# shaofeifei11/SSDR-AL

Measured on AMD Instinct MI355X. Metric: Mpoints/s subsample→KNN→RandLA-Net→FPS-GCN select, S3DIS 40960-pt tiles, higher is better.
Workload: dtype bf16x3: split-bf16 MFMA operands (hi*hi + lo*hi + hi*lo), fp32 accumulate, fp32 activations and non-matrix arithmetic

## Files before the change

include/ssdr_al.h:

```cpp
#ifndef SSDR_AL_H
#define SSDR_AL_H

#include <stddef.h>
#include <stdint.h>

#ifdef __cplusplus
extern "C" {
#endif

#define SSDR_OK               0
#define SSDR_ERR_INVALID      1
#define SSDR_ERR_NO_DEVICE    2
#define SSDR_ERR_HIP          3
#define SSDR_ERR_EMPTY        4
#define SSDR_ERR_UNSUPPORTED  5
#define SSDR_ERR_INTERNAL     6

const char* ssdr_version(void);
const char* ssdr_last_error(void);
int  ssdr_init(int device);
void ssdr_shutdown(void);
int  ssdr_stream_sync(void* stream);
int  ssdr_stream_create(void** out_stream);
int  ssdr_stream_create_priority(void** out_stream, int priority);
int  ssdr_stream_destroy(void* stream);
int  ssdr_main_stream(void** out_stream);
int  ssdr_stream_wait(void* waiter, void* waited);
int  ssdr_event_create(void** ev);
int  ssdr_event_record(void* ev, void* stream);
int  ssdr_stream_wait_event(void* stream, void* ev);
int  ssdr_event_destroy(void* ev);
int ssdr_prof_enable(int on);
const char* ssdr_prof_report(void);
float ssdr_last_gpu_ms(void);

int ssdr_knn(const float* points, size_t npts, size_t dim,
             const float* queries, size_t nqueries, size_t K, int64_t* indices);
int ssdr_knn_batch(const float* batch_data, size_t batch_size, size_t npts, size_t dim,
                   const float* queries, size_t nqueries, size_t K, int64_t* batch_indices);
int ssdr_knn_batch_i32(const float* batch_data, size_t batch_size, size_t npts, size_t dim,
                       const float* queries, size_t nqueries, size_t K, int32_t* batch_indices);
int ssdr_knn_batch_dev(const float* d_batch_data, size_t batch_size, size_t npts, size_t dim,
                       const float* d_queries, size_t nqueries, size_t K, int32_t* d_indices, void* stream);
int ssdr_knn_status(void* stream, int32_t* out4);
int ssdr_knn_status_poll(void* stream, int32_t* out4);

int ssdr_knn_pyramid_dev(const float* d_xyz, size_t batch_size, size_t npts,
                         size_t num_layers, const int32_t* ratios, size_t K,
                         int32_t* const* d_neigh_idx, int32_t* const* d_sub_idx,
                         int32_t* const* d_interp_idx, void* stream);
int ssdr_knn_pyramid(const float* xyz, size_t batch_size, size_t npts,
                     size_t num_layers, const int32_t* ratios, size_t K,
                     int32_t* const* neigh_idx, int32_t* const* sub_idx, int32_t* const* interp_idx);

#define SSDR_ORDER_REFERENCE 0
#define SSDR_ORDER_KEY       1
int ssdr_grid_subsample(const float* points, size_t n,
                        const float* features, size_t fdim,
                        const int32_t* classes, size_t ldim,
                        float sampleDl, int order, size_t* out_m);
int ssdr_grid_subsample_fetch(float* out_points, float* out_features, int32_t* out_classes);
int ssdr_grid_subsample_dev(const float* d_points, size_t n,
                            const float* d_features, size_t fdim,
                            const int32_t* d_classes, size_t ldim,
                            float sampleDl, int order,
                            float* d_out_points, float* d_out_features, int32_t* d_out_classes,
                            int64_t* d_out_m, void* stream);

int ssdr_grid_subsample_batch_dev(const float* d_points, const float* d_features, size_t fdim, const int32_t* d_classes, size_t ldim,
                                  const int64_t* cloud_offsets, size_t num_clouds, float sampleDl,
                                  float* d_out_points, float* d_out_features, int32_t* d_out_classes, int64_t* d_out_m, void* stream);
#define SSDR_SUBSAMPLE_AUTO 0
#define SSDR_SUBSAMPLE_SORT 1
int ssdr_grid_subsample_set_method(int method);
int ssdr_grid_subsample_status(void* stream, int32_t* out_status);

int ssdr_split3_dev(const float* d_xyz, size_t n, size_t max_size, size_t recurse_max_size, size_t merge_max, int32_t* d_part, int32_t* d_order, int64_t* part_offsets,
                    size_t max_parts, size_t* num_parts, void* stream);

int ssdr_tile_select_dev(const float* d_points, const float* d_colors, int color_dim, const int64_t* d_m, size_t n_max,
                         const float* center, size_t num_points, const int32_t* d_perm, const float* d_dup_u, float color_scale,
                         float* d_out_xyz, float* d_out_feat, int32_t* d_out_idx, void* stream);

int ssdr_tile_select_batch_dev(const float* d_points, const float* d_colors, int color_dim, const int64_t* d_m, const int64_t* cloud_offsets,
                               size_t num_clouds, const float* centers, size_t num_points, const int32_t* d_perm, const float* d_dup_u,
                               float color_scale, float* d_out_xyz, float* d_out_feat, int32_t* d_out_idx, const int32_t* d_labels,
                               int32_t* d_out_labels, void* stream);
int ssdr_tile_select_possibility_dev(const float* d_points, const float* d_colors, int color_dim, const int64_t* d_m, size_t n_max,
                                     const float* center, size_t num_points, const int32_t* d_perm, const float* d_dup_u, float color_scale,
                                     float* d_out_xyz, float* d_out_feat, int32_t* d_out_idx,
                                     double* d_possibility, double* d_out_min_possibility, int32_t* d_out_argmin, void* stream);

int ssdr_prune_dev(const float* d_xyz, size_t n, float voxel_size, const uint8_t* d_rgb, const uint8_t* d_labels, int n_labels,
                   const uint32_t* d_objects, int n_objects, float* d_out_xyz, uint8_t* d_out_rgb, uint32_t* d_out_labels,
                   uint32_t* d_out_objects, int64_t* d_out_m, void* stream);
int ssdr_prune_status(void* stream, int32_t* out_status);

int  ssdr_randla_create(int num_layers, const int32_t* d_out, int k_n, int num_classes, int in_dim, void** handle);
int  ssdr_randla_num_layers(void* handle);
int  ssdr_randla_layer_shape(void* handle, int layer, int* in, int* out, int* has_bias);
int  ssdr_randla_set_layer(void* handle, int layer, const float* W, const float* b);
#define SSDR_PREC_F32 0
#define SSDR_PREC_BF16X3 1
#define SSDR_PREC_BF16 2
int  ssdr_randla_set_precision(void* handle, int mode);
int  ssdr_randla_set_formulation(void* handle, int tiles32);
void ssdr_randla_destroy(void* handle);
int  ssdr_randla_infer_dev(void* handle, size_t batch_size, size_t npts, const float* d_features, const float* d_xyz,
                           const int32_t* ratios, int32_t* const* d_neigh_idx, int32_t* const* d_interp_idx,
                           float* d_probs, float* d_feat32, void* stream);
int  ssdr_randla_infer_rows_dev(void* handle, const size_t* level_rows, const float* d_features, const float* d_xyz,
                                int32_t* const* d_neigh_idx, int32_t* const* d_interp_idx, float* d_probs, float* d_feat32, void* stream);

#define SSDR_PREDICT_MAX_ROWS (1 << 23)
int ssdr_predict_layout(const int64_t* cloud_offsets, size_t num_clouds, size_t num_points, size_t num_layers, const int32_t* ratios,
                        int64_t* level_rows);
int ssdr_predict_tile_dev(const float* d_points, const float* d_colors, const int32_t* d_labels, const int64_t* cloud_offsets, size_t num_clouds,
                          const float* centers, size_t num_points, size_t num_layers, const int32_t* ratios, const int32_t* d_perm, const float* d_dup_u,
                          float color_scale, float* d_cm_xyz, int32_t* d_cm_idx, float* d_pk_xyz, float* d_pk_feat, int32_t* d_pk_src,
                          int32_t* d_pk_labels, void* stream);
int ssdr_knn_pyramid_ragged_dev(const float* d_cm_xyz, const int64_t* cloud_offsets, size_t num_clouds, size_t num_points, size_t num_layers,
                                const int32_t* ratios, size_t K, int32_t* d_cm_neigh, int32_t* d_cm_interp, void* stream);
int ssdr_predict_translate_dev(const int64_t* cloud_offsets, size_t num_clouds, size_t num_points, size_t num_layers, const int32_t* ratios, size_t K,
                               const int32_t* d_cm_neigh, const int32_t* d_cm_interp, int32_t* d_pk_neigh, int32_t* d_pk_interp, void* stream);
#define SSDR_READBACK_REFERENCE 0
#define SSDR_READBACK_POINT 1
int ssdr_predict_readback_dev(const int64_t* cloud_offsets, size_t num_clouds, size_t num_points, size_t num_layers, const int32_t* ratios,
                              const int32_t* d_cm_idx, const float* d_pk_probs, size_t num_classes, const float* d_pk_feat32, int mode,
                              float* d_probs, float* d_feat32, void* stream);

#define SSDR_UNC_LC 0
#define SSDR_UNC_ENTROPY 1
#define SSDR_UNC_SB 2
#define SSDR_REGION_MEAN 0
#define SSDR_REGION_SUM_WEIGHT 1
#define SSDR_REGION_WETSU 2
int ssdr_point_uncertainty_dev(const float* d_probs, size_t n, int num_classes, int mode, float* d_unc, int32_t* d_cls, void* stream);
int ssdr_region_stats_dev(const float* d_unc, const int32_t* d_cls, const int32_t* d_sp_off, const int32_t* d_sp_pts, size_t S,
                          int num_classes, int mode, double* d_region_unc, int32_t* d_dom, int32_t* d_dom_cnt, void* stream);
int ssdr_dominant_label_dev(const int32_t* d_labels, const int32_t* d_sp_off, const int32_t* d_sp_pts, size_t S, int num_labels,
                            int32_t* d_label, double* d_purity, void* stream);
int ssdr_clsbal_dev(const int32_t* d_region_class, size_t S, const uint8_t* d_skip, const int32_t* d_selected_class_list, size_t n_selected,
                    double* d_region_unc, void* stream);
int ssdr_class_hist_dev(const int32_t* d_region_class, size_t S, const uint8_t* d_skip, const int32_t* d_selected_class_list, size_t n_selected,
                        int32_t* d_hist64, void* stream);
int ssdr_clsbal_hist_dev(const int32_t* d_region_class, size_t S, const int32_t* d_hist64, size_t total, double* d_region_unc, void* stream);
int ssdr_rank_regions_dev(const double* d_region_unc, size_t S, int32_t* d_sorted_inds, void* stream);
int ssdr_segment_mean_features_dev(const float* d_feat, int feat_dim, const int32_t* d_cls, const int32_t* d_dom,
                                   const int32_t* d_sp_off, const int32_t* d_sp_pts, const int32_t* d_sel, size_t nsel,
                                   float* d_out, void* stream);
int ssdr_mask_regions_dev(const double* d_region_unc, const uint8_t* d_labelled, size_t S, size_t S_padded, double* d_out, void* stream);
int ssdr_gather_rows_dev(const void* d_in, const int32_t* d_idx, size_t n, size_t row_bytes, void* d_out, void* stream);
int ssdr_widen_f32_f64_dev(const float* d_x, size_t n, double* d_y0, double* d_y1, void* stream);
int ssdr_cloud_graph_dev(const float* d_xyz, const int32_t* d_sp_off, const int32_t* d_sp_pts, const int32_t* d_sel, size_t nsel,
                         size_t max_sp_size, int gcn_top, double* d_centres, double* d_cd_dir, double* d_adj, void* stream);
int ssdr_cloud_graph_batch_dev(const float* d_xyz, const int32_t* d_sp_off, const int32_t* d_sp_pts, const int32_t* d_sel,
                               const int32_t* d_coff, const int64_t* d_boff, size_t num_clouds, size_t n_total, size_t n_max,
                               int gcn_top, double* d_centres, double* d_cd_dir, double* d_adj, void* stream);
int ssdr_select_set_chamfer_mode(int mode);
int ssdr_propagate_batch_dev(const double* d_adj, const int32_t* d_coff, const int64_t* d_boff, size_t num_clouds, size_t n_max,
                             const int32_t* d_rows, const double* d_vin, int feat_dim, double* d_vout, double* d_comb, void* stream);
int ssdr_propagate_dev(const double* d_adj, size_t n, const int32_t* d_rows, const double* d_vin, int feat_dim, double* d_vout,
                       double* d_comb, void* stream);
int ssdr_create_adj_dev(const float* d_feat, size_t N, int F, const double* d_centres, const double* d_cd_dir, const int32_t* d_coff, const int64_t* d_boff,
                        size_t num_clouds, size_t n_max, const int32_t* d_rows, float* d_out_v, float* d_out_adj, void* stream);
#define SSDR_GCN_NHID 128
#define SSDR_GCN_NPARAM 4353
#define SSDR_GCN_FUSED_CAP 1024
#define SSDR_GCN_FORM_AUTO 0
#define SSDR_GCN_FORM_GENERAL 1
#define SSDR_GCN_FORM_FUSED 2
#define SSDR_GCN_ST_SINGLETON 32
#define SSDR_GCN_ST_NO_LABELLED 64
#define SSDR_GCN_ST_SUBSTITUTED 128
#define SSDR_GCN_ST_OVERSIZE 256
int ssdr_gcn_block_adj_dev(const float* d_feat, size_t cap_rows, int F, const double* d_centres, const double* d_cd_dir, const int32_t* d_coff, const int64_t* d_boff,
                           size_t num_clouds, size_t n_max, const int32_t* d_rows, const int32_t* d_counts, float* d_out_v, float* d_out_adj, float* d_out_adjT,
                           int32_t* d_rowcloud, int32_t* d_info, void* stream);
int ssdr_gcn_train_dev(const float* d_v, const float* d_adj, const float* d_adjT, const int32_t* d_coff, const int64_t* d_boff, size_t num_clouds, size_t n_max,
                       const int32_t* d_rows, const int32_t* d_rowcloud, const int32_t* d_counts, size_t cap_rows, const float* d_init, float* d_trained, int steps,
                       float p, float lr, float weight_decay, float lamda, uint64_t seed, int form, float* d_loss, int32_t* d_info, void* stream);
int ssdr_gcn_eval_dev(const float* d_v, const float* d_adj, const float* d_adjT, const int32_t* d_coff, const int64_t* d_boff, size_t num_clouds, size_t n_max,
                      const int32_t* d_rows, const int32_t* d_rowcloud, const int32_t* d_counts, size_t cap_rows, const float* d_params, double* d_out, int32_t* d_info,
                      void* stream);
int ssdr_gcn_sampling_dev(const float* d_feat, int feat_dim, const int32_t* d_cls, const int32_t* d_dom, const int32_t* d_lab_cls, const int32_t* d_lab_dom,
                          const float* d_xyz, const int32_t* d_sp_off, const int32_t* d_sp_pts, const int32_t* d_order, size_t S, const uint8_t* d_labelled, const int32_t* d_sp_base, size_t num_clouds,
                          const int32_t* d_lab_off, const int32_t* d_lab_sp, size_t n_lab, size_t batch_size, const float* d_init, int steps, float p, float lr, float weight_decay,
                          float lamda, uint64_t seed, int form, size_t cap_rows, size_t cap_nmax, size_t cap_sq, size_t cap_unl, size_t max_select, int32_t* d_result, void* stream);
int ssdr_gcn_sampling_rows(void* stream, const double** d_rows, size_t* cap_rows, const float** d_params, const float** d_loss, const int32_t** d_info);
int ssdr_gcn_fps_sampling_dev(const float* d_feat, int feat_dim, const int32_t* d_cls, const int32_t* d_dom, const int32_t* d_lab_cls, const int32_t* d_lab_dom,
                              const float* d_xyz, const int32_t* d_sp_off, const int32_t* d_sp_pts, const int32_t* d_order, size_t S, const uint8_t* d_labelled, const int32_t* d_sp_base, size_t num_clouds,
                              const int32_t* d_lab_off, const int32_t* d_lab_sp, size_t n_lab, size_t batch_size, int gcn_number, int gcn_top, int selector, int start,
                              size_t cap_rows, size_t cap_nmax, size_t cap_sq, size_t cap_unl, size_t max_select, int32_t* d_result, void* stream);
int ssdr_gcn_fps_sampling_rows(void* stream, const double** d_rows, size_t* cap_rows);
int ssdr_gcn_fps_sharded_local_dev(const float* d_feat, int feat_dim, const int32_t* d_cls, const int32_t* d_dom, const int32_t* d_lab_cls, const int32_t* d_lab_dom,
                                   const float* d_xyz, const int32_t* d_sp_off, const int32_t* d_sp_pts, const int32_t* d_lab_off, const int32_t* d_lab_sp, size_t n_lab, size_t num_clouds,
                                   const int32_t* d_gorder, size_t Sg, const uint8_t* d_glabelled, const int32_t* d_gbase, int rank, int world, size_t Smax, size_t Bmax,
                                   size_t batch_size, int gcn_number, int gcn_top, size_t cap_rows, size_t cap_nmax, size_t cap_sq, size_t nu_max, size_t nl_max,
                                   double* d_comb_out, int32_t* d_plan, void* stream);
int ssdr_fps_gathered_dev(const double* d_gathered, const int32_t* d_plan, int world, size_t nu_max, size_t cap_rows, int repeat, int start, size_t max_select, double* d_glob,
                          int32_t* d_out, void* stream);
int ssdr_kcenter_gathered_dev(const double* d_gathered, const int32_t* d_plan, int world, size_t nu_max, size_t nl_max, const int32_t* d_nlab_off, size_t n_lab_total,
                              size_t cap_rows, size_t max_select, double* d_glob, int32_t* d_already, int32_t* d_out, void* stream);
int ssdr_select_status(void* stream, int32_t* out_status);
int ssdr_fps_dev(const double* d_feat, size_t n, int feat_dim, int start, size_t count, int32_t* d_out, void* stream);
int ssdr_fps_superpoint_dev(const double* d_centres, const double* d_cd_dir, size_t n, int start, size_t count, int32_t* d_out, void* stream);
int ssdr_edcd_fps_batch_dev(const double* d_centres, double* d_cd_dir, const int32_t* d_coff, const int64_t* d_boff, const int32_t* d_ntop, size_t num_clouds,
                            size_t n_max, size_t max_select, int32_t* d_out, int32_t* d_status, void* stream);
int ssdr_edcd_sampling_dev(const float* d_xyz, const int32_t* d_sp_off, const int32_t* d_sp_pts, const int32_t* d_order, size_t S, const uint8_t* d_labelled,
                           const int32_t* d_sp_base, size_t num_clouds, size_t batch_size, size_t cap_rows, size_t cap_nmax, size_t cap_sq, size_t max_select,
                           int32_t* d_result, void* stream);
int ssdr_edcd_sampling_sharded_dev(const float* d_xyz, const int32_t* d_sp_off, const int32_t* d_sp_pts, size_t num_clouds, const int32_t* d_gorder, size_t Sg,
                                   const uint8_t* d_glabelled, const int32_t* d_gbase, int rank, int world, size_t Smax, size_t Bmax, size_t batch_size,
                                   size_t cap_rows, size_t cap_nmax, size_t cap_sq, size_t max_select, int32_t* d_result, void* stream);
int ssdr_topk_regions_dev(const int32_t* d_order, size_t n, const uint8_t* d_skip, size_t batch_size, size_t lo, size_t hi, int32_t* d_res, int32_t* d_out, void* stream);
#define SSDR_LABEL_DOMINANT 0
#define SSDR_LABEL_NAIL     1
int ssdr_oracle_label_dev(const int32_t* d_gt, const int32_t* d_pred_class, size_t n, const int32_t* d_sp_off, const int32_t* d_sp_pts, size_t S,
                          const int32_t* d_sp_cloud, size_t num_clouds, const int32_t* d_items, const int32_t* d_n_items, size_t max_items,
                          const int32_t* d_cloud_key, size_t max_region, int num_labels, int num_classes, int mode, double threshold, int64_t min_size,
                          int64_t* d_budget, float* d_mask, float* d_label, uint8_t* d_used, uint8_t* d_labeled, int32_t* d_class_out, size_t class_cap,
                          int32_t* d_proc_order, int64_t* d_out, void* stream);
int ssdr_oracle_label_items_dev(const int32_t* d_result, int layout, size_t max_select, const int32_t* d_order, size_t S, const uint8_t* d_skip,
                                const int32_t* d_sp_cloud, size_t num_clouds, int32_t* d_items, size_t max_items, int32_t* d_n_items, int32_t* d_cloud_key,
                                void* stream);
int ssdr_kcenter_dev(const double* d_feat, size_t n, int feat_dim, const int32_t* d_already_selected, size_t n_already, size_t count,
                     int32_t* d_out, void* stream);

int ssdr_chamfer3d_forward_dev(const float* d_xyz1, const float* d_xyz2, size_t batch, size_t n, size_t m,
                               float* d_dist1, float* d_dist2, int32_t* d_idx1, int32_t* d_idx2, void* stream);

int ssdr_vote_smooth_dev(float* d_test_probs, const int32_t* d_point_idx, const float* d_probs, size_t n, int num_classes, double smooth,
                         int32_t* d_owner_scratch, void* stream);
int ssdr_confusion_dev(const float* d_probs, int num_classes, const int32_t* d_proj_idx, const int32_t* d_labels, size_t n, int32_t* d_pred,
                       uint64_t* d_confusion, double* d_iou, void* stream);

int ssdr_dev_alloc(size_t bytes, void** d_ptr);
int ssdr_dev_free(void* d_ptr);
int ssdr_memcpy_h2d(void* d_dst, const void* src, size_t bytes);
int ssdr_memcpy_d2h(void* dst, const void* d_src, size_t bytes);
int ssdr_memcpy_h2d_on(void* d_dst, const void* src, size_t bytes, void* stream);
int ssdr_memcpy_d2h_on(void* dst, const void* d_src, size_t bytes, void* stream);

int ssdr_knn_batch_distance_pick(const float* batch_data, size_t batch_size, size_t npts, size_t dim, float* batch_queries,
                                 size_t nqueries, size_t K, int64_t* batch_indices, uint32_t seed);

int ssdr_knn_graph_dev(const float* d_xyz, size_t n, size_t k_nn1, size_t k_nn2, uint32_t* d_source, uint32_t* d_target,
                       float* d_distances, uint32_t* d_target2, void* stream);
int ssdr_geof_dev(const float* d_xyz, size_t n, const uint32_t* d_target, size_t k_nn, float* d_geof, void* stream);

#ifdef __cplusplus
}
#endif
#endif
```

ssdr-al_amd/csrc/randla.hpp:

```cpp
#pragma once
#include "ssdr_internal.hpp"

namespace ssdr {

struct DenseArgs {
    const float* x1; int k1;
    const float* x2; int k2;
    const int* idx2;
    int m_per_batch;
    int x2_rows_per_batch;
    const float* W; const float* b;
    float* y; int M, N; int act;
    int ldy;
    const float* xyz; size_t xyz_batch_stride; int xyz_rows_per_batch;
    const uint16_t* wt_hi; const uint16_t* wt_lo; int kp;
};

struct LfaArgs {
    const float* xyz; size_t xyz_batch_stride;
    const int* neigh;
    const float* fin;
    const float* w_l1; const float* b_l1;
    const float* w_l2; const float* b_l2;
    const float* w_fc;
    const float* w_fc_t;
    const float* g;
    float* out;
    int n;
    const uint16_t* fc_hi; const uint16_t* fc_lo;
    const uint16_t* l2_hi; const uint16_t* l2_lo; int kp2;
};

struct Lfa32Args {
    const float* xyz; size_t xyz_batch_stride;
    const int* neigh;
    const float* fin;
    const float* g;
    float* out;
    int n;
    const uint16_t* w1p; const float* b1;
    const uint16_t *w2_hi, *w2_lo; const float* b2;
    const uint16_t *fc_hi, *fc_lo;
};

constexpr int PREC_F32 = 0;
constexpr int PREC_BF16X3 = 1;
constexpr int PREC_BF16 = 2;

int launch_dense(const DenseArgs& a, hipStream_t s);
int launch_xyz_fill(const DenseArgs& a, hipStream_t s);
int launch_lfa(int D, const LfaArgs& a, bool second, int B, hipStream_t s);
struct TailArgs {
    const float* x; int M, C;
    const uint16_t *w1h, *w1l; int kp1; const float* b1;
    const uint16_t *w2h, *w2l; int kp2; const float* b2;
    const uint16_t *w3h, *w3l; int kp3; const float* b3;
    float* feat32; float* probs;
    const float* skip; const float* up; const int* idx; int m_per_batch, up_rows_per_batch;
    const uint16_t *wdh, *wdl; int kpd; const float* bd;
};
int launch_tail_bf16(const TailArgs& t, int prec, hipStream_t s);
int launch_dense_bf16(const DenseArgs& a, int prec, hipStream_t s);
int launch_dense_rows2(const DenseArgs& a, const DenseArgs& b, hipStream_t s);
int launch_dense_chain(const DenseArgs& l1, const DenseArgs& l2, int prec, hipStream_t s);
int launch_lfa_bf16(int D, const LfaArgs& a, bool second, int B, int prec, hipStream_t s);
int launch_lfa32(int D, const Lfa32Args& a, bool second, int B, int prec, hipStream_t s);
int launch_gather_max(const float* f, const int* idx, int n_in, int n_out, int idx_rows, int C, float* out, int B, hipStream_t s);
int launch_tail(const float* x, const float* W1, const float* b1, const float* W2, const float* b2, const float* W3, const float* b3,
                int M, int C, float* feat32, float* probs, hipStream_t s);
int launch_head(const float* x, const float* W, const float* b, int M, int C, float* probs, hipStream_t s);

}
```

ssdr-al_amd/csrc/randla_bf16.hip:

```cpp
#include "ssdr_internal.hpp"
#include "randla.hpp"
#include "randla_dev.hpp"
#include <cmath>

namespace ssdr {

__device__ __forceinline__ u32x4 ld128(const void* p) { return *reinterpret_cast<const u32x4*>(p); }
__device__ __forceinline__ void st128(void* p, u32x4 v) { *reinterpret_cast<u32x4*>(p) = v; }

template <int TERMS>
__device__ __forceinline__ f32x4 mma_split(const u32x4 (&a)[2], const u32x4 (&b)[2], f32x4 c) {
    c = mfma_bf16(a[0], b[0], c);
    if (TERMS == 2) { c = mfma_bf16(a[1], b[0], c); c = mfma_bf16(a[0], b[1], c); }
    return c;
}

template <int TM, int KC, int TERMS, bool VEC>
__global__ __launch_bounds__(256) SSDR_WAVES_PER_EU(TM == 128 ? 4 : 5) void dense_bf16_kernel(DenseArgs a) {
    constexpr int KS = KC + 8;
    constexpr int TPR = KC / 8;
    constexpr int RPP = 256 / TPR;
    constexpr int APASS = TM / RPP, BPASS = 64 / RPP;
    static_assert(TM % RPP == 0 && 64 % RPP == 0, "staging passes");
    constexpr int CT = TM == 128 ? 4 : 1;
    __shared__ __attribute__((aligned(16))) uint16_t As[TERMS][TM * KS];
    __shared__ __attribute__((aligned(16))) uint16_t Bs[TERMS][64 * KS];
    const int tid = threadIdx.x, lane = tid & 63, w = tid >> 6;
    int bxr = (int)blockIdx.x, byc = (int)blockIdx.y;
    if (a.idx2 && a.m_per_batch % TM == 0 && a.M % a.m_per_batch == 0 && ((a.M / a.m_per_batch) & 7) == 0) {
        const int gy = (int)gridDim.y, rpb = a.m_per_batch / TM;
        const int lin = byc * (int)gridDim.x + bxr, xcd = lin & 7, j = lin >> 3, rb = j / gy;
        byc = j % gy; bxr = (xcd + 8 * (rb / rpb)) * rpb + rb % rpb;
    }
    const int row0 = bxr * TM, col0 = byc * 64;
    const int K = a.k1 + a.k2;
    const int sr = tid / TPR, sk = (tid % TPR) * 8;
    const float* x1r[APASS]; const float* x2r[APASS];
#pragma unroll
    for (int h = 0; h < APASS; ++h) {
        const int grow = row0 + sr + RPP * h;
        x1r[h] = nullptr; x2r[h] = nullptr;
        if (grow < a.M) {
            x1r[h] = a.x1 + (size_t)grow * a.k1;
            if (a.k2) {
                size_t r2 = (size_t)grow;
                if (a.idx2) r2 = (size_t)(grow / a.m_per_batch) * a.x2_rows_per_batch + (size_t)a.idx2[grow];
                x2r[h] = a.x2 + r2 * a.k2;
            }
        }
    }
    float ra[APASS][8]; u32x4 rb[BPASS][TERMS];
    auto fetch = [&](int kc) {
#pragma unroll
        for (int h = 0; h < APASS; ++h) {
            if (VEC) {
#pragma unroll
                for (int q = 0; q < 2; ++q) {
                    const int gk = kc + sk + 4 * q;
                    float4 v = make_float4(0.f, 0.f, 0.f, 0.f);
                    if (x1r[h] && gk < K) v = (gk < a.k1) ? *reinterpret_cast<const float4*>(x1r[h] + gk) : *reinterpret_cast<const float4*>(x2r[h] + (gk - a.k1));
                    ra[h][4 * q] = v.x; ra[h][4 * q + 1] = v.y; ra[h][4 * q + 2] = v.z; ra[h][4 * q + 3] = v.w;
                }
            } else {
#pragma unroll
                for (int j = 0; j < 8; ++j) {
                    const int gk = kc + sk + j;
                    float v = 0.f;
                    if (x1r[h]) { if (gk < a.k1) v = x1r[h][gk]; else if (gk < K) v = x2r[h][gk - a.k1]; }
                    ra[h][j] = v;
                }
            }
        }
#pragma unroll
        for (int h = 0; h < BPASS; ++h) {
            const int gc = col0 + sr + RPP * h;
#pragma unroll
            for (int t = 0; t < TERMS; ++t) {
                u32x4 v = {0u, 0u, 0u, 0u};
                if (gc < a.N && kc + sk < a.kp) v = ld128((t ? a.wt_lo : a.wt_hi) + (size_t)gc * a.kp + kc + sk);
                rb[h][t] = v;
            }
        }
    };
    auto stash = [&]() {
#pragma unroll
        for (int h = 0; h < APASS; ++h) {
            u32x4 hi, lo;
#pragma unroll
            for (int q = 0; q < 4; ++q) {
                unsigned hq, lq;
                split_bf16(ra[h][2 * q], ra[h][2 * q + 1], hq, lq);
                hi[q] = hq; lo[q] = lq;
            }
            st128(&As[0][(sr + RPP * h) * KS + sk], hi);
            if (TERMS == 2) st128(&As[TERMS - 1][(sr + RPP * h) * KS + sk], lo);
        }
#pragma unroll
        for (int h = 0; h < BPASS; ++h)
#pragma unroll
            for (int t = 0; t < TERMS; ++t) st128(&Bs[t][(sr + RPP * h) * KS + sk], rb[h][t]);
    };
    f32x4 acc[2][CT];
#pragma unroll
    for (int r = 0; r < 2; ++r)
#pragma unroll
        for (int c = 0; c < CT; ++c) acc[r][c] = f32x4{0.f, 0.f, 0.f, 0.f};
    const int rbase = TM == 128 ? w * 32 : 0, cbase = TM == 128 ? 0 : w * 16;
    const int fr = lane & 15, fk = 8 * (lane >> 4);
    fetch(0);
    for (int kc = 0; kc < K; kc += KC) {
        stash();
        __syncthreads();
        if (kc + KC < K) fetch(kc + KC);
#pragma unroll
        for (int ks = 0; ks < KC / 32; ++ks) {
            u32x4 af[2][2], bf[CT][2];
#pragma unroll
            for (int r = 0; r < 2; ++r)
#pragma unroll
                for (int t = 0; t < TERMS; ++t) af[r][t] = ld128(&As[t][(rbase + r * 16 + fr) * KS + ks * 32 + fk]);
#pragma unroll
            for (int c = 0; c < CT; ++c)
#pragma unroll
                for (int t = 0; t < TERMS; ++t) bf[c][t] = ld128(&Bs[t][(cbase + c * 16 + fr) * KS + ks * 32 + fk]);
#pragma unroll
            for (int r = 0; r < 2; ++r)
#pragma unroll
                for (int c = 0; c < CT; ++c) acc[r][c] = mma_split<TERMS>(af[r], bf[c], acc[r][c]);
        }
        __syncthreads();
    }
#pragma unroll
    for (int c = 0; c < CT; ++c) {
        const int col = col0 + cbase + c * 16 + (lane & 15);
        if (col >= a.N) continue;
        const float bias = a.b ? a.b[col] : 0.f;
#pragma unroll
        for (int r = 0; r < 2; ++r)
#pragma unroll
            for (int q = 0; q < 4; ++q) {
                const int row = row0 + rbase + r * 16 + (lane >> 4) * 4 + q;
                if (row < a.M) { float v = acc[r][c][q] + bias; a.y[(size_t)row * (a.ldy ? a.ldy : a.N) + col] = a.act ? lrelu(v) : v; }
            }
    }
}


struct ChainArgs {
    const float* x1; const float* x2; int k2;
    const uint16_t* wa_hi; const uint16_t* wa_lo; int kpa; const float* ba;
    const uint16_t* wb_hi; const uint16_t* wb_lo; int kpb; const float* bb;
    float* y; int M;
};
template <int D, int K2P, int TM, int TERMS>
__global__ __launch_bounds__(256) void dense_chain_kernel(ChainArgs a) {
    constexpr int KS = K2P + 8;
    constexpr int TPR = K2P <= 32 ? 4 : 16;
    constexpr int RPP = 256 / TPR;
    constexpr int WC = TM == 128 ? 1 : 2;
    constexpr int CT1 = (D / 16 + WC - 1) / WC;
    constexpr int CT2 = 4 / WC;
    static_assert(D % 16 == 0 && D <= 64 && K2P % 32 == 0 && TPR * 8 >= K2P && (TM == 128 || TM == 64) && TM % RPP == 0, "shapes");
    __shared__ __attribute__((aligned(16))) uint16_t As[TERMS][TM * KS];
    __shared__ __attribute__((aligned(16))) uint16_t Bs[TERMS][64 * KS];
    const int tid = threadIdx.x, lane = tid & 63, w = tid >> 6;
    const int wr = TM == 128 ? w : (w >> 1), wc = TM == 128 ? 0 : (w & 1);
    const int row0 = (int)blockIdx.x * TM;
    const int sr = tid / TPR, sk = (tid % TPR) * 8;
    const int K = D + a.k2;
    if (sk < K2P) {
        float4 va[TM / RPP][2];
#pragma unroll
        for (int h = 0; h < TM / RPP; ++h) {
            const int grow = row0 + sr + RPP * h;
            va[h][0] = make_float4(0.f, 0.f, 0.f, 0.f); va[h][1] = va[h][0];
            if (grow < a.M) {
                const float* src = sk < D ? a.x1 + (size_t)grow * D + sk : (sk < K ? a.x2 + (size_t)grow * a.k2 + (sk - D) : nullptr);
                if (src) { va[h][0] = *reinterpret_cast<const float4*>(src); va[h][1] = *reinterpret_cast<const float4*>(src + 4); }
            }
        }
#pragma unroll
        for (int h = 0; h < TM / RPP; ++h) {
            const int r = sr + RPP * h;
            const float4 v0 = va[h][0], v1 = va[h][1];
            u32x4 hi, lo; unsigned hq, lq;
            split_bf16(v0.x, v0.y, hq, lq); hi[0] = hq; lo[0] = lq;
            split_bf16(v0.z, v0.w, hq, lq); hi[1] = hq; lo[1] = lq;
            split_bf16(v1.x, v1.y, hq, lq); hi[2] = hq; lo[2] = lq;
            split_bf16(v1.z, v1.w, hq, lq); hi[3] = hq; lo[3] = lq;
            st128(&As[0][r * KS + sk], hi);
            if (TERMS == 2) st128(&As[TERMS - 1][r * KS + sk], lo);
        }
    }
    u32x4 wreg[64 / RPP][TERMS];
    auto load_w = [&](const uint16_t* whi, const uint16_t* wlo, int kp, int col0, int ncols, int kvalid) {
#pragma unroll
        for (int h = 0; h < 64 / RPP; ++h) {
            const int r = sr + RPP * h;
#pragma unroll
            for (int t = 0; t < TERMS; ++t) {
                u32x4 v = {0u, 0u, 0u, 0u};
                if (sk < K2P && col0 + r < ncols && sk < kvalid) v = ld128((t ? wlo : whi) + (size_t)(col0 + r) * kp + sk);
                wreg[h][t] = v;
            }
        }
    };
    auto store_w = [&]() {
        if (sk < K2P) {
#pragma unroll
            for (int h = 0; h < 64 / RPP; ++h)
#pragma unroll
                for (int t = 0; t < TERMS; ++t) st128(&Bs[t][(sr + RPP * h) * KS + sk], wreg[h][t]);
        }
    };
    load_w(a.wa_hi, a.wa_lo, a.kpa, 0, D, D);
    store_w();
    __syncthreads();
    load_w(a.wb_hi, a.wb_lo, a.kpb, 0, 2 * D, K);
    const int fr = lane & 15, fk = 8 * (lane >> 4), rbase = wr * 32;
    {
        f32x4 acc[2][CT1];
#pragma unroll
        for (int r = 0; r < 2; ++r)
#pragma unroll
            for (int c = 0; c < CT1; ++c) acc[r][c] = f32x4{0.f, 0.f, 0.f, 0.f};
        const bool has1 = wc * CT1 * 16 < D;
        if (has1) {
#pragma unroll
            for (int ks = 0; ks < (D + 31) / 32; ++ks) {
                u32x4 af[2][2], bf[CT1][2];
#pragma unroll
                for (int r = 0; r < 2; ++r)
#pragma unroll
                    for (int t = 0; t < TERMS; ++t) af[r][t] = ld128(&As[t][(rbase + r * 16 + fr) * KS + ks * 32 + fk]);
#pragma unroll
                for (int c = 0; c < CT1; ++c)
#pragma unroll
                    for (int t = 0; t < TERMS; ++t) bf[c][t] = ld128(&Bs[t][((wc * CT1 + c) * 16 + fr) * KS + ks * 32 + fk]);
#pragma unroll
                for (int r = 0; r < 2; ++r)
#pragma unroll
                    for (int c = 0; c < CT1; ++c) acc[r][c] = mma_split<TERMS>(af[r], bf[c], acc[r][c]);
            }
        }
        if (WC > 1) __syncthreads();
        if (has1) {
#pragma unroll
            for (int c = 0; c < CT1; ++c) {
                const int col = (wc * CT1 + c) * 16 + (lane & 15);
                const float bias = a.ba ? a.ba[col] : 0.f;
#pragma unroll
                for (int r = 0; r < 2; ++r)
#pragma unroll
                    for (int q = 0; q < 4; ++q) {
                        const int row = rbase + r * 16 + (lane >> 4) * 4 + q;
                        const float v = lrelu(acc[r][c][q] + bias);
                        unsigned hq, lq; split_bf16(v, 0.f, hq, lq);
                        As[0][row * KS + col] = (uint16_t)(hq & 0xffffu);
                        if (TERMS == 2) As[TERMS - 1][row * KS + col] = (uint16_t)(lq & 0xffffu);
                    }
            }
        }
    }
    for (int ct = 0; ct < (2 * D + 63) / 64; ++ct) {
        __syncthreads();
        store_w();
        __syncthreads();
        if (ct + 1 < (2 * D + 63) / 64) load_w(a.wb_hi, a.wb_lo, a.kpb, (ct + 1) * 64, 2 * D, K);
        f32x4 acc[2][CT2];
#pragma unroll
        for (int r = 0; r < 2; ++r)
#pragma unroll
            for (int c = 0; c < CT2; ++c) acc[r][c] = f32x4{0.f, 0.f, 0.f, 0.f};
#pragma unroll
        for (int ks = 0; ks < K2P / 32; ++ks) {
            u32x4 af[2][2], bf[CT2][2];
#pragma unroll
            for (int r = 0; r < 2; ++r)
#pragma unroll
                for (int t = 0; t < TERMS; ++t) af[r][t] = ld128(&As[t][(rbase + r * 16 + fr) * KS + ks * 32 + fk]);
#pragma unroll
            for (int c = 0; c < CT2; ++c)
#pragma unroll
                for (int t = 0; t < TERMS; ++t) bf[c][t] = ld128(&Bs[t][((wc * CT2 + c) * 16 + fr) * KS + ks * 32 + fk]);
#pragma unroll
            for (int r = 0; r < 2; ++r)
#pragma unroll
                for (int c = 0; c < CT2; ++c) acc[r][c] = mma_split<TERMS>(af[r], bf[c], acc[r][c]);
        }
#pragma unroll
        for (int c = 0; c < CT2; ++c) {
            const int col = ct * 64 + (wc * CT2 + c) * 16 + (lane & 15);
            if (col >= 2 * D) continue;
            const float bias = a.bb ? a.bb[col] : 0.f;
#pragma unroll
            for (int r = 0; r < 2; ++r)
#pragma unroll
                for (int q = 0; q < 4; ++q) {
                    const int row = row0 + rbase + r * 16 + (lane >> 4) * 4 + q;
                    if (row < a.M) a.y[(size_t)row * (2 * D) + col] = lrelu(acc[r][c][q] + bias);
                }
        }
    }
}

template <int D> struct LfaBf16Cfg {
    static constexpr int H = D / 2;
    static constexpr int NW = D >= 256 ? 8 : 4;
    static constexpr int NT = NW * 64;
    static constexpr int NCG = D == 64 ? 2 : NW;
    static constexpr int NPG = NW / NCG;
    static constexpr int PTS = D == 64 ? 8 : 4;
    static constexpr int PW = PTS / NPG;
    static constexpr int ROWS = PTS * 16;
    static constexpr int LDX = H + 8;
    static constexpr int NCT1 = H / 16;
    static constexpr int NCH = NCT1 / NCG;
    static_assert(NCT1 % NCG == 0 && PTS % NPG == 0, "tile split");
    static constexpr size_t lds_bytes(int terms) { return (size_t)ROWS * ((size_t)terms * LDX * 2 + 10 * 4 + 4); }
};

#ifndef HIPEMU
typedef __amdgpu_buffer_rsrc_t rsrc_t;
__device__ __forceinline__ rsrc_t make_rsrc(const void* p, unsigned bytes) { return __builtin_amdgcn_make_buffer_rsrc(const_cast<void*>(p), 0, (int)bytes, 0x00020000); }
template <int IMM> __device__ __forceinline__ float buf_load(rsrc_t r, unsigned voff) { return __builtin_bit_cast(float, __builtin_amdgcn_raw_buffer_load_b32(r, (int)voff + IMM, 0, 0)); }
#else
struct rsrc_t { const char* p; };
static inline rsrc_t make_rsrc(const void* p, unsigned) { return rsrc_t{reinterpret_cast<const char*>(p)}; }
template <int IMM> static inline float buf_load(rsrc_t r, unsigned voff) { return *reinterpret_cast<const float*>(r.p + voff + IMM); }
#endif

template <int D, bool SECOND, int TERMS>
__global__ __launch_bounds__(LfaBf16Cfg<D>::NT) SSDR_WAVES_PER_EU((D == 256 && !SECOND) ? 4 : 1) void lfa_bf16_kernel(LfaArgs a) {
    using C = LfaBf16Cfg<D>;
    constexpr int H = C::H, PTS = C::PTS, ROWS = C::ROWS, LDX = C::LDX, NT = C::NT, NCG = C::NCG, PW = C::PW, NCH = C::NCH, NCT1 = C::NCT1;
    SSDR_DYN_SHARED(float, smem);
    uint16_t* X[2];
    X[0] = reinterpret_cast<uint16_t*>(smem);
    X[1] = X[0] + (TERMS == 2 ? (size_t)ROWS * LDX : 0);
    float* REL = reinterpret_cast<float*>(X[0] + (size_t)TERMS * ROWS * LDX);
    int* NBR = reinterpret_cast<int*>(REL + (size_t)ROWS * 10);
    const int tid = threadIdx.x, lane = tid & 63, w = tid >> 6;
    const int lc = lane & 15, lg = lane >> 4;
    const int cg = w % NCG, p0 = (w / NCG) * PW;
    int bx_, b; xcd_tile_map(bx_, b);
    const int pt0 = bx_ * PTS;
    const float* xyz = a.xyz + (size_t)b * a.xyz_batch_stride;
    const int* neigh = a.neigh + (size_t)b * a.n * 16;

    float w1[NCH][3], b1c[NCH]; float4 b1r[NCH];
#pragma unroll
    for (int j = 0; j < NCH; ++j) {
        const int ct = cg * NCH + j;
#pragma unroll
        for (int ks = 0; ks < 3; ++ks) {
            const int k = ks * 4 + lg;
            const float v = a.w_l1[(k < 10 ? k : 9) * H + ct * 16 + lc];
            w1[j][ks] = k < 10 ? v : 0.f;
        }
        b1c[j] = a.b_l1[ct * 16 + lc];
        b1r[j] = *reinterpret_cast<const float4*>(a.b_l1 + ct * 16 + 4 * lg);
    }

    for (int row = tid; row < ROWS; row += NT) {
        const int n = pt0 + (row >> 4);
        float r[10]; int j = 0;
#pragma unroll
        for (int q = 0; q < 10; ++q) r[q] = 0.f;
        if (n < a.n) {
            j = neigh[(size_t)n * 16 + (row & 15)];
            const float px = xyz[3 * (size_t)n], py = xyz[3 * (size_t)n + 1], pz = xyz[3 * (size_t)n + 2];
            const float qx = xyz[3 * (size_t)j], qy = xyz[3 * (size_t)j + 1], qz = xyz[3 * (size_t)j + 2];
            const float dx = px - qx, dy = py - qy, dz = pz - qz;
            r[0] = sqrtf(dx * dx + dy * dy + dz * dz);
            r[1] = dx; r[2] = dy; r[3] = dz; r[4] = px; r[5] = py; r[6] = pz; r[7] = qx; r[8] = qy; r[9] = qz;
        }
#pragma unroll
        for (int q = 0; q < 10; ++q) REL[row * 10 + q] = r[q];
        NBR[row] = j;
    }
    __syncthreads();

    auto store_row4 = [&](int p, int ct, const float (&v)[4]) {
        u32x2 hi, lo; unsigned h, l;
        split_bf16(v[0], v[1], h, l); hi[0] = h; lo[0] = l;
        split_bf16(v[2], v[3], h, l); hi[1] = h; lo[1] = l;
        const int e = (p * 16 + lc) * LDX + ct * 16 + 4 * lg;
        *reinterpret_cast<u32x2*>(&X[0][e]) = hi;
        if (TERMS == 2) *reinterpret_cast<u32x2*>(&X[1][e]) = lo;
    };

    float fx[PW][NCH][4];

#pragma unroll
    for (int p = 0; p < PW; ++p) {
        float rf[3];
#pragma unroll
        for (int ks = 0; ks < 3; ++ks) { const int k = ks * 4 + lg; rf[ks] = (k < 10) ? REL[((p0 + p) * 16 + lc) * 10 + k] : 0.f; }
#pragma unroll
        for (int j = 0; j < NCH; ++j) {
            f32x4 at = f32x4{b1r[j].x, b1r[j].y, b1r[j].z, b1r[j].w};
#pragma unroll
            for (int ks = 0; ks < 3; ++ks) at = mfma16(w1[j][ks], rf[ks], at);
            float v[4];
#pragma unroll
            for (int r = 0; r < 4; ++r) v[r] = lrelu(at[r]);
            store_row4(p0 + p, cg * NCH + j, v);
            if (!SECOND) {
                f32x4 ac = f32x4{b1c[j], b1c[j], b1c[j], b1c[j]};
#pragma unroll
                for (int ks = 0; ks < 3; ++ks) ac = mfma16(rf[ks], w1[j][ks], ac);
#pragma unroll
                for (int r = 0; r < 4; ++r) fx[p][j][r] = lrelu(ac[r]);
            }
        }
    }
    __syncthreads();

    if (SECOND) {
        f32x4 accT[PW][NCH], acc2[PW][NCH];
#pragma unroll
        for (int j = 0; j < NCH; ++j) {
            const int ct = cg * NCH + j;
            const float4 br = *reinterpret_cast<const float4*>(a.b_l2 + ct * 16 + 4 * lg);
            const float bc = a.b_l2[ct * 16 + lc];
#pragma unroll
            for (int p = 0; p < PW; ++p) { accT[p][j] = f32x4{br.x, br.y, br.z, br.w}; acc2[p][j] = f32x4{bc, bc, bc, bc}; }
        }
        for (int kb = 0; kb < H / 32; ++kb) {
            u32x4 xf[PW][2], wf[NCH][2];
#pragma unroll
            for (int j = 0; j < NCH; ++j)
#pragma unroll
                for (int t = 0; t < TERMS; ++t) wf[j][t] = ld128((t ? a.l2_lo : a.l2_hi) + (size_t)((cg * NCH + j) * 16 + lc) * a.kp2 + kb * 32 + 8 * lg);
#pragma unroll
            for (int p = 0; p < PW; ++p)
#pragma unroll
                for (int t = 0; t < TERMS; ++t) xf[p][t] = ld128(&X[t][((p0 + p) * 16 + lc) * LDX + kb * 32 + 8 * lg]);
#pragma unroll
            for (int p = 0; p < PW; ++p)
#pragma unroll
                for (int j = 0; j < NCH; ++j) { accT[p][j] = mma_split<TERMS>(wf[j], xf[p], accT[p][j]); acc2[p][j] = mma_split<TERMS>(xf[p], wf[j], acc2[p][j]); }
        }
        __syncthreads();
#pragma unroll
        for (int p = 0; p < PW; ++p)
#pragma unroll
            for (int j = 0; j < NCH; ++j) {
                float v[4];
#pragma unroll
                for (int r = 0; r < 4; ++r) { v[r] = lrelu(accT[p][j][r]); fx[p][j][r] = lrelu(acc2[p][j][r]); }
                store_row4(p0 + p, cg * NCH + j, v);
            }
        __syncthreads();
    }

    const rsrc_t rG = make_rsrc(a.g + (size_t)b * a.n * D, (unsigned)a.n * D * 4u);
    const rsrc_t rF = make_rsrc(a.fin + (size_t)b * a.n * H, (unsigned)a.n * H * 4u);
    f32x4 acc[PW][2 * NCH];
    float fn[PW][NCH][4];
#pragma unroll
    for (int p = 0; p < PW; ++p) {
        int nb[4];
#pragma unroll
        for (int r = 0; r < 4; ++r) nb[r] = NBR[(p0 + p) * 16 + lg * 4 + r];
#pragma unroll
        for (int r = 0; r < 4; ++r) {
            const unsigned og = (unsigned)nb[r] * (D * 4u) + lc * 4u + cg * NCH * 64u, of = (unsigned)nb[r] * (H * 4u) + lc * 4u + cg * NCH * 64u;
            acc[p][0][r] = buf_load<0>(rG, og); acc[p][NCH][r] = buf_load<H * 4>(rG, og); fn[p][0][r] = buf_load<0>(rF, of);
            if constexpr (NCH == 2) { acc[p][1][r] = buf_load<64>(rG, og); acc[p][NCH + 1][r] = buf_load<H * 4 + 64>(rG, og); fn[p][1][r] = buf_load<64>(rF, of); }
        }
    }
    static_assert(NCH <= 2, "gather immediates are written out for one or two tiles per half");
    for (int kb = 0; kb < H / 32; ++kb) {
        u32x4 af[PW][2], bf[2 * NCH][2];
#pragma unroll
        for (int c = 0; c < 2 * NCH; ++c) {
            const int col = (c < NCH ? cg * NCH + c : NCT1 + cg * NCH + (c - NCH)) * 16 + lc;
#pragma unroll
            for (int t = 0; t < TERMS; ++t) bf[c][t] = ld128((t ? a.fc_lo : a.fc_hi) + (size_t)col * D + H + kb * 32 + 8 * lg);
        }
#pragma unroll
        for (int p = 0; p < PW; ++p)
#pragma unroll
            for (int t = 0; t < TERMS; ++t) af[p][t] = ld128(&X[t][((p0 + p) * 16 + lc) * LDX + kb * 32 + 8 * lg]);
#pragma unroll
        for (int p = 0; p < PW; ++p)
#pragma unroll
            for (int c = 0; c < 2 * NCH; ++c) acc[p][c] = mma_split<TERMS>(af[p], bf[c], acc[p][c]);
    }

    float* out = a.out + (size_t)b * a.n * D;
#pragma unroll
    for (int p = 0; p < PW; ++p) {
        const int n = pt0 + p0 + p;
#pragma unroll
        for (int c = 0; c < 2 * NCH; ++c) {
            const int col = (c < NCH ? cg * NCH + c : NCT1 + cg * NCH + (c - NCH)) * 16 + lc;
            float m = fmaxf(fmaxf(acc[p][c][0], acc[p][c][1]), fmaxf(acc[p][c][2], acc[p][c][3]));
            m = rows_max(m);
            float s = 0.f, v = 0.f;
#pragma unroll
            for (int r = 0; r < 4; ++r) {
                const float e = fast_exp2(acc[p][c][r] - m);
                const float f = c < NCH ? fn[p][c][r] : fx[p][c - NCH][r];
                s += e; v = fmaf(f, e, v);
            }
            s = rows_sum(s); v = rows_sum(v);
            v = v * fast_rcp(s);
            if (lg == 0 && n < a.n) out[(size_t)n * D + col] = v;
        }
    }
}

struct TailPre {
    const float* skip; const float* up; const int* idx; int m_per_batch, up_rows_per_batch;
    const uint16_t *wh, *wl; int kp; const float* b;
};
template <int TERMS, int C, bool PRE>
__global__ __launch_bounds__(256) void tail_bf16_kernel(TailPre pre, const float* __restrict__ x, const uint16_t* __restrict__ w1h, const uint16_t* __restrict__ w1l, int kp1,
                                                        const float* __restrict__ b1, const uint16_t* __restrict__ w2h, const uint16_t* __restrict__ w2l, int kp2,
                                                        const float* __restrict__ b2, const uint16_t* __restrict__ w3h, const uint16_t* __restrict__ w3l, int kp3,
                                                        const float* __restrict__ b3, int M, float* __restrict__ feat32, float* __restrict__ probs) {
    const int lane = threadIdx.x & 63, lc = lane & 15, lg = lane >> 4;
    const int wave = blockIdx.x * 4 + (threadIdx.x >> 6), nwaves = gridDim.x * 4;
    auto ld64x2 = [](const uint16_t* p0, const uint16_t* p1) {
        const u32x2 a = *reinterpret_cast<const u32x2*>(p0), b = *reinterpret_cast<const u32x2*>(p1);
        return u32x4{a[0], a[1], b[0], b[1]};
    };
    constexpr int F_WD = 0, F_W1 = 4, F_W2 = 8, F_W3 = 12, NFRAG = 13;
    __shared__ u32x4 s_w[NFRAG * 2][64];
    float4 BD[2];
    {
        const int wv = threadIdx.x >> 6;
#pragma unroll
        for (int t = 0; t < TERMS; ++t) {
            const uint16_t* p1 = t ? w1l : w1h; const uint16_t* p2 = t ? w2l : w2h; const uint16_t* p3 = t ? w3l : w3h;
            if (PRE && wv == 0) {
                const uint16_t* pd = t ? pre.wl : pre.wh;
#pragma unroll
                for (int kb = 0; kb < 2; ++kb)
#pragma unroll
                    for (int ct = 0; ct < 2; ++ct) s_w[(F_WD + 2 * kb + ct) * 2 + t][lane] = ld128(pd + (size_t)(16 * ct + lc) * pre.kp + 32 * kb + 8 * lg);
            }
            if (wv == 1) {
#pragma unroll
                for (int ct = 0; ct < 4; ++ct)
                    s_w[(F_W1 + ct) * 2 + t][lane] = PRE ? ld64x2(p1 + (size_t)(16 * ct + lc) * kp1 + 4 * lg, p1 + (size_t)(16 * ct + lc) * kp1 + 16 + 4 * lg) : ld128(p1 + (size_t)(16 * ct + lc) * kp1 + 8 * lg);
            }
            if (wv == 2) {
#pragma unroll
                for (int kb = 0; kb < 2; ++kb)
#pragma unroll
                    for (int ct = 0; ct < 2; ++ct) s_w[(F_W2 + 2 * kb + ct) * 2 + t][lane] = ld64x2(p2 + (size_t)(16 * ct + lc) * kp2 + 32 * kb + 4 * lg, p2 + (size_t)(16 * ct + lc) * kp2 + 32 * kb + 16 + 4 * lg);
            }
            if (wv == 3) s_w[F_W3 * 2 + t][lane] = lc < C ? ld64x2(p3 + (size_t)lc * kp3 + 4 * lg, p3 + (size_t)lc * kp3 + 16 + 4 * lg) : u32x4{0u, 0u, 0u, 0u};
        }
        __syncthreads();
    }
    auto wfr = [&](int f, u32x4 (&w)[2]) { w[0] = s_w[f * 2][lane]; w[1] = s_w[f * 2 + (TERMS - 1)][lane]; };
    if (PRE) { BD[0] = *reinterpret_cast<const float4*>(pre.b + 4 * lg); BD[1] = *reinterpret_cast<const float4*>(pre.b + 16 + 4 * lg); }
    float4 B1[4], B2t[2], B3; float B2c[2];
#pragma unroll
    for (int ct = 0; ct < 4; ++ct) B1[ct] = *reinterpret_cast<const float4*>(b1 + 16 * ct + 4 * lg);
#pragma unroll
    for (int ct = 0; ct < 2; ++ct) { B2t[ct] = *reinterpret_cast<const float4*>(b2 + 16 * ct + 4 * lg); B2c[ct] = b2[16 * ct + lc]; }
    {
        float t[4];
#pragma unroll
        for (int r = 0; r < 4; ++r) t[r] = 4 * lg + r < C ? b3[4 * lg + r] : 0.f;
        B3 = make_float4(t[0], t[1], t[2], t[3]);
    }
    auto frag = [](const float (&v)[8], u32x4 (&f)[2]) {
#pragma unroll
        for (int q = 0; q < 4; ++q) { unsigned h, l; split_bf16(v[2 * q], v[2 * q + 1], h, l); f[0][q] = h; f[1][q] = l; }
    };
    const int ntiles = (M + 15) / 16;
    int tpb = 0, nbe = 0;
    if (PRE && pre.m_per_batch % 16 == 0 && M % pre.m_per_batch == 0 && (gridDim.x & 7) == 0) { tpb = pre.m_per_batch / 16; nbe = M / pre.m_per_batch; if (nbe & 7) tpb = 0; }
    const int lw = ((int)blockIdx.x >> 3) * 4 + ((int)threadIdx.x >> 6), lnw = nwaves >> 3, lnt = tpb ? (nbe >> 3) * tpb : 0;
    const int it_first = tpb ? lw : wave, it_end = tpb ? lnt : ntiles, it_step = tpb ? lnw : nwaves;
    auto tile_of = [&](int it) { return tpb ? (((int)blockIdx.x & 7) + 8 * (it / tpb)) * tpb + it % tpb : it; };
    auto row_of = [&](int it) { const int r = tile_of(it) * 16 + lc; return (it < it_end && r < M) ? r : -1; };
    auto load8r = [&](const float* p, int ok, float4 (&v)[2]) {
        v[0] = make_float4(0.f, 0.f, 0.f, 0.f); v[1] = v[0];
        if (ok) { v[0] = *reinterpret_cast<const float4*>(p + 8 * lg); v[1] = *reinterpret_cast<const float4*>(p + 8 * lg + 4); }
    };
    auto unpack8 = [](const float4 (&a)[2], float (&v)[8]) { v[0] = a[0].x; v[1] = a[0].y; v[2] = a[0].z; v[3] = a[0].w; v[4] = a[1].x; v[5] = a[1].y; v[6] = a[1].z; v[7] = a[1].w; };
    float4 n_sk[2], n_up[2];
    int idx_next = 0;
    auto issue_rows = [&](int it, int idx) {
        const int r = row_of(it);
        if (PRE) {
            const int rw = r < 0 ? 0 : r;
            load8r(pre.skip + (size_t)rw * 32, r >= 0, n_sk);
            load8r(pre.up + ((size_t)(rw / pre.m_per_batch) * pre.up_rows_per_batch + (size_t)idx) * 32, r >= 0, n_up);
        } else load8r(x + (size_t)(r < 0 ? 0 : r) * 32, r >= 0, n_sk);
    };
    auto load_idx = [&](int it) { const int r = row_of(it); return (PRE && r >= 0) ? pre.idx[r] : 0; };
    {
        const int i0 = load_idx(it_first);
        idx_next = load_idx(it_first + it_step);
        issue_rows(it_first, i0);
    }
    for (int it = it_first; it < it_end; it += it_step) {
        const int tile = tile_of(it);
        const int row = tile * 16 + lc;
        float c_sk[8], c_up[8];
        unpack8(n_sk, c_sk);
        if (PRE) unpack8(n_up, c_up);
        {
            const int idx2 = load_idx(it + 2 * it_step);
            issue_rows(it + it_step, idx_next);
            idx_next = idx2;
        }
        SSDR_SCHED_FENCE();
        u32x4 xf[2];
        if (PRE) {
            u32x4 sf[2], uf[2]; frag(c_sk, sf); frag(c_up, uf);
            f32x4 d0 = f32x4{BD[0].x, BD[0].y, BD[0].z, BD[0].w}, d1 = f32x4{BD[1].x, BD[1].y, BD[1].z, BD[1].w};
            { u32x4 w[2]; wfr(F_WD + 0, w); d0 = mma_split<TERMS>(w, sf, d0); wfr(F_WD + 2, w); d0 = mma_split<TERMS>(w, uf, d0);
              wfr(F_WD + 1, w); d1 = mma_split<TERMS>(w, sf, d1); wfr(F_WD + 3, w); d1 = mma_split<TERMS>(w, uf, d1); }
            const float v[8] = {lrelu(d0[0]), lrelu(d0[1]), lrelu(d0[2]), lrelu(d0[3]), lrelu(d1[0]), lrelu(d1[1]), lrelu(d1[2]), lrelu(d1[3])};
            frag(v, xf);
        } else frag(c_sk, xf);
        float h1[4][4];
#pragma unroll
        for (int ct = 0; ct < 4; ++ct) {
            f32x4 acc = f32x4{B1[ct].x, B1[ct].y, B1[ct].z, B1[ct].w};
            { u32x4 w[2]; wfr(F_W1 + ct, w); acc = mma_split<TERMS>(w, xf, acc); }
#pragma unroll
            for (int r = 0; r < 4; ++r) h1[ct][r] = lrelu(acc[r]);
        }
        f32x4 at[2] = {f32x4{B2t[0].x, B2t[0].y, B2t[0].z, B2t[0].w}, f32x4{B2t[1].x, B2t[1].y, B2t[1].z, B2t[1].w}};
        f32x4 ac[2] = {f32x4{B2c[0], B2c[0], B2c[0], B2c[0]}, f32x4{B2c[1], B2c[1], B2c[1], B2c[1]}};
#pragma unroll
        for (int kb = 0; kb < 2; ++kb) {
            const float v[8] = {h1[2 * kb][0], h1[2 * kb][1], h1[2 * kb][2], h1[2 * kb][3], h1[2 * kb + 1][0], h1[2 * kb + 1][1], h1[2 * kb + 1][2], h1[2 * kb + 1][3]};
            u32x4 hf[2]; frag(v, hf);
#pragma unroll
            for (int ct = 0; ct < 2; ++ct) { u32x4 w[2]; wfr(F_W2 + 2 * kb + ct, w); at[ct] = mma_split<TERMS>(w, hf, at[ct]); ac[ct] = mma_split<TERMS>(hf, w, ac[ct]); }
        }
#pragma unroll
        for (int ct = 0; ct < 2; ++ct)
#pragma unroll
            for (int r = 0; r < 4; ++r) { const int rr = tile * 16 + 4 * lg + r; if (rr < M) feat32[(size_t)rr * 32 + 16 * ct + lc] = lrelu(ac[ct][r]); }
        const float v2[8] = {lrelu(at[0][0]), lrelu(at[0][1]), lrelu(at[0][2]), lrelu(at[0][3]), lrelu(at[1][0]), lrelu(at[1][1]), lrelu(at[1][2]), lrelu(at[1][3])};
        u32x4 ff[2]; frag(v2, ff);
        f32x4 lg3 = f32x4{B3.x, B3.y, B3.z, B3.w};
        { u32x4 w[2]; wfr(F_W3, w); lg3 = mma_split<TERMS>(w, ff, lg3); }
        float z[4], m = -3.402823466e+38f;
#pragma unroll
        for (int r = 0; r < 4; ++r) { z[r] = 4 * lg + r < C ? lg3[r] : -3.402823466e+38f; m = fmaxf(m, z[r]); }
        m = rows_max(m);
        float e[4], sum = 0.f;
#pragma unroll
        for (int r = 0; r < 4; ++r) { e[r] = 4 * lg + r < C ? expf(z[r] - m) : 0.f; sum += e[r]; }
        sum = rows_sum(sum);
        if (row < M)
#pragma unroll
            for (int r = 0; r < 4; ++r) if (4 * lg + r < C) probs[(size_t)row * C + 4 * lg + r] = e[r] / sum;
    }
}

template <int TM, int KC>
static int launch_dense_bf16_t(const DenseArgs& a, int prec, bool vec, hipStream_t s) {
    dim3 grid((unsigned)((a.M + TM - 1) / TM), (unsigned)((a.N + 63) / 64));
    if (prec == PREC_BF16X3) {
        if (vec) hipLaunchKernelGGL((dense_bf16_kernel<TM, KC, 2, true>), grid, dim3(256), 0, s, a);
        else hipLaunchKernelGGL((dense_bf16_kernel<TM, KC, 2, false>), grid, dim3(256), 0, s, a);
    } else {
        if (vec) hipLaunchKernelGGL((dense_bf16_kernel<TM, KC, 1, true>), grid, dim3(256), 0, s, a);
        else hipLaunchKernelGGL((dense_bf16_kernel<TM, KC, 1, false>), grid, dim3(256), 0, s, a);
    }
    SSDR_HIP(hipGetLastError());
    return SSDR_OK;
}

int launch_dense_bf16(const DenseArgs& a, int prec, hipStream_t s) {
    if (a.M <= 0 || a.N <= 0) return SSDR_OK;
    if (a.N == 8 && a.k2 == 0 && a.k1 <= 16) return launch_dense(a, s);
    if (!a.wt_hi || (prec == PREC_BF16X3 && !a.wt_lo)) { set_error("dense (bf16): the layer has no bf16 weight pieces"); return SSDR_ERR_INVALID; }
    if (a.xyz) SSDR_TRY(launch_xyz_fill(a, s));
    const bool small = a.M <= 16384;
    const double tm = small ? 32.0 : 128.0, kc = small ? 64.0 : 32.0;
    const double exec = 2.0 * std::ceil(a.M / tm) * tm * std::ceil((a.k1 + a.k2) / kc) * kc * std::ceil(a.N / 64.0) * 64.0 * (prec == PREC_BF16X3 ? 3.0 : 1.0);
    ProfScope prof(small ? "dense_bf16_kernel<32,64>" : "dense_bf16_kernel<128,32>", s, 2.0 * (double)a.M * (double)(a.k1 + a.k2) * (double)a.N, exec);
    const bool vec = a.k1 % 4 == 0 && a.k2 % 4 == 0 && ((uintptr_t)a.x1 & 15) == 0 && ((uintptr_t)a.x2 & 15) == 0;
    if (small) return launch_dense_bf16_t<32, 64>(a, prec, vec, s);
    return launch_dense_bf16_t<128, 32>(a, prec, vec, s);
}

int launch_dense_chain(const DenseArgs& l1, const DenseArgs& l2, int prec, hipStream_t s) {
    const int d = l1.k1;
    const bool shapes = l1.k2 == 0 && l1.N == d && l1.act && l2.act && l2.k1 == d && l2.N == 2 * d && l2.x1 == l1.y && l2.M == l1.M && !l2.idx2 && !l1.ldy && !l2.ldy && !l1.xyz && !l2.xyz &&
                        l2.k2 % 8 == 0 && l2.k2 > 0 && l1.wt_hi && l2.wt_hi && (prec != PREC_BF16X3 || (l1.wt_lo && l2.wt_lo)) &&
                        (((uintptr_t)l1.x1 | (uintptr_t)l2.x2) & 15) == 0 && l1.kp % 8 == 0 && l2.kp % 8 == 0;
    if (!shapes || l1.M <= 0) return SSDR_ERR_UNSUPPORTED;
    int k2p = 0;
    if (d == 16 && d + l2.k2 <= 32) k2p = 32; else if (d == 64 && d + l2.k2 <= 96) k2p = 96; else return SSDR_ERR_UNSUPPORTED;
    ChainArgs a{l1.x1, l2.x2, l2.k2, l1.wt_hi, l1.wt_lo, l1.kp, l1.b, l2.wt_hi, l2.wt_lo, l2.kp, l2.b, l2.y, l1.M};
    const double np = prec == PREC_BF16X3 ? 3.0 : 1.0, m128 = std::ceil(l1.M / 128.0) * 128.0;
    ProfScope prof(d == 16 ? "dense_chain_kernel<16>" : "dense_chain_kernel<64>", s, 2.0 * (double)l1.M * ((double)d * d + (double)(d + l2.k2) * 2.0 * d),
                   2.0 * m128 * ((d == 16 ? 32.0 * 16 : 64.0 * 64) + (double)k2p * (d == 16 ? 64.0 : 128.0)) * np);
    const bool t64 = d == 64;
    const dim3 grid((unsigned)((l1.M + (t64 ? 63 : 127)) / (t64 ? 64 : 128)));
#define SSDR_CHAIN(D_, K_, TM_) do { if (prec == PREC_BF16X3) hipLaunchKernelGGL((dense_chain_kernel<D_, K_, TM_, 2>), grid, dim3(256), 0, s, a); else hipLaunchKernelGGL((dense_chain_kernel<D_, K_, TM_, 1>), grid, dim3(256), 0, s, a); } while (0)
    if (d == 16) { if (t64) SSDR_CHAIN(16, 32, 64); else SSDR_CHAIN(16, 32, 128); }
    else { if (t64) SSDR_CHAIN(64, 96, 64); else SSDR_CHAIN(64, 96, 128); }
#undef SSDR_CHAIN
    SSDR_HIP(hipGetLastError());
    return SSDR_OK;
}

int launch_tail_bf16(const TailArgs& t, int prec, hipStream_t s) {
    if (t.M <= 0) return SSDR_OK;
    if ((t.C != 13 && t.C != 8) || (!t.skip && ((uintptr_t)t.x & 15)) || (t.skip && (((uintptr_t)t.skip | (uintptr_t)t.up) & 15)) || !t.w1h || !t.w2h || !t.w3h || (prec == PREC_BF16X3 && (!t.w1l || !t.w2l || !t.w3l))) return SSDR_ERR_UNSUPPORTED;
    const double m16 = std::ceil(t.M / 16.0) * 16.0;
    ProfScope prof("tail_kernel", s, (double)t.M * 4.0 * (32 + 32 + t.C), 2.0 * m16 * ((t.skip ? 64.0 * 32 : 0.0) + 32.0 * 64 + 2.0 * 64 * 32 + 32.0 * 16) * (prec == PREC_BF16X3 ? 3.0 : 1.0));
    const dim3 g((unsigned)std::max(1, std::min((t.M + 63) / 64, ctx().num_cu * 4)));
    TailPre pre{t.skip, t.up, t.idx, t.m_per_batch, t.up_rows_per_batch, t.wdh, t.wdl, t.kpd, t.bd};
#define SSDR_TAIL(TERMS_, C_) do { if (t.skip) hipLaunchKernelGGL((tail_bf16_kernel<TERMS_, C_, true>), g, dim3(256), 0, s, pre, t.x, t.w1h, t.w1l, t.kp1, t.b1, t.w2h, t.w2l, t.kp2, t.b2, t.w3h, t.w3l, t.kp3, t.b3, t.M, t.feat32, t.probs); \
                               else hipLaunchKernelGGL((tail_bf16_kernel<TERMS_, C_, false>), g, dim3(256), 0, s, pre, t.x, t.w1h, t.w1l, t.kp1, t.b1, t.w2h, t.w2l, t.kp2, t.b2, t.w3h, t.w3l, t.kp3, t.b3, t.M, t.feat32, t.probs); } while (0)
    if (prec == PREC_BF16X3) { if (t.C == 13) SSDR_TAIL(2, 13); else SSDR_TAIL(2, 8); }
    else { if (t.C == 13) SSDR_TAIL(1, 13); else SSDR_TAIL(1, 8); }
#undef SSDR_TAIL
    SSDR_HIP(hipGetLastError());
    return SSDR_OK;
}

template <int D> static int launch_lfa_bf16_d(const LfaArgs& a, bool second, int B, int prec, hipStream_t s) {
    using C = LfaBf16Cfg<D>;
    dim3 grid((unsigned)((a.n + C::PTS - 1) / C::PTS), (unsigned)B);
    const int terms = prec == PREC_BF16X3 ? 2 : 1;
    const size_t lds = C::lds_bytes(terms);
    static std::once_flag attr_once;
    hipError_t ae = hipSuccess;
    std::call_once(attr_once, [&] {
        ae = hipFuncSetAttribute(reinterpret_cast<const void*>(&lfa_bf16_kernel<D, true, 2>), hipFuncAttributeMaxDynamicSharedMemorySize, (int)C::lds_bytes(2));
        if (ae == hipSuccess) ae = hipFuncSetAttribute(reinterpret_cast<const void*>(&lfa_bf16_kernel<D, false, 2>), hipFuncAttributeMaxDynamicSharedMemorySize, (int)C::lds_bytes(2));
        if (ae == hipSuccess) ae = hipFuncSetAttribute(reinterpret_cast<const void*>(&lfa_bf16_kernel<D, true, 1>), hipFuncAttributeMaxDynamicSharedMemorySize, (int)C::lds_bytes(1));
        if (ae == hipSuccess) ae = hipFuncSetAttribute(reinterpret_cast<const void*>(&lfa_bf16_kernel<D, false, 1>), hipFuncAttributeMaxDynamicSharedMemorySize, (int)C::lds_bytes(1));
    });
    SSDR_HIP(ae);
    const double rows = (double)B * (double)a.n * 16.0;
    const double np = terms == 2 ? 3.0 : 1.0;
    const double exec = rows * (2.0 * 12 * C::H * (second ? 1.0 : 2.0) + (second ? 2.0 * 2.0 * C::H * C::H * np : 0.0) + 2.0 * C::H * D * np);
    ProfScope prof("lfa_att_kernel", s, rows * (2.0 * 10 * C::H + (second ? 2.0 * C::H * C::H : 0.0) + 2.0 * D * D + 2.0 * D), exec);
    if (terms == 2) {
        if (second) hipLaunchKernelGGL((lfa_bf16_kernel<D, true, 2>), grid, dim3(C::NT), lds, s, a);
        else hipLaunchKernelGGL((lfa_bf16_kernel<D, false, 2>), grid, dim3(C::NT), lds, s, a);
    } else {
        if (second) hipLaunchKernelGGL((lfa_bf16_kernel<D, true, 1>), grid, dim3(C::NT), lds, s, a);
        else hipLaunchKernelGGL((lfa_bf16_kernel<D, false, 1>), grid, dim3(C::NT), lds, s, a);
    }
    SSDR_HIP(hipGetLastError());
    return SSDR_OK;
}

int launch_lfa_bf16(int D, const LfaArgs& a, bool second, int B, int prec, hipStream_t s) {
    if (a.n <= 0 || B <= 0) return SSDR_OK;
    if (!a.g || !a.fc_hi || (second && !a.l2_hi)) { set_error("lfa (bf16): missing G rows or bf16 weight pieces"); return SSDR_ERR_INVALID; }
    switch (D) {
        case 64: return launch_lfa_bf16_d<64>(a, second, B, prec, s);
        case 128: return launch_lfa_bf16_d<128>(a, second, B, prec, s);
        case 256: return launch_lfa_bf16_d<256>(a, second, B, prec, s);
        case 512: return launch_lfa_bf16_d<512>(a, second, B, prec, s);
        default: set_error("d_out=%d has no bf16 LFA kernel (64, 128, 256, 512)", D); return SSDR_ERR_UNSUPPORTED;
    }
}

}
```

ssdr-al_amd/csrc/randla_lfa32.hip:

```cpp
#include "ssdr_internal.hpp"
#include "randla.hpp"
#include "randla_dev.hpp"
#include <cmath>

namespace ssdr {

#ifndef HIPEMU
typedef __amdgpu_buffer_rsrc_t rsrc32_t;
__device__ __forceinline__ rsrc32_t make_rsrc32(const void* p, unsigned bytes) { return __builtin_amdgcn_make_buffer_rsrc(const_cast<void*>(p), 0, (int)bytes, 0x00020000); }
__device__ __forceinline__ float buf_load_s(rsrc32_t r, unsigned voff, unsigned soff) { return __builtin_bit_cast(float, __builtin_amdgcn_raw_buffer_load_b32(r, (int)voff, (int)soff, 0)); }
#else
struct rsrc32_t { const char* p; unsigned bytes; };
static inline rsrc32_t make_rsrc32(const void* p, unsigned bytes) { return rsrc32_t{reinterpret_cast<const char*>(p), bytes}; }
static inline float buf_load_s(rsrc32_t r, unsigned voff, unsigned soff) {
    const unsigned long long o = (unsigned long long)voff + soff;
    return o + 4 <= r.bytes ? *reinterpret_cast<const float*>(r.p + o) : 0.f;
}
#endif

__device__ __forceinline__ u32x4 ld128g(const void* p) { return *reinterpret_cast<const u32x4*>(p); }
__device__ __forceinline__ void st128s(void* p, u32x4 v) { *reinterpret_cast<u32x4*>(p) = v; }

template <int D> struct Lfa32Cfg {
    static constexpr int H = D / 2;
    static constexpr int KS = H / 16;
    static constexpr int HT = H / 32;
    static constexpr int CT = D / 32;
    static constexpr int CCF = D < 8192 / H ? D : 8192 / H;
    static constexpr int CC2 = H < 8192 / H ? H : 8192 / H;
    static constexpr int NF = D / CCF, N2 = H / CC2;
    static constexpr int RS = 2 * H + 16;
    static constexpr int nw(bool second) { return D >= 256 && !second ? 8 : 4; }
    static constexpr int tpw(bool second) { return D == 128 && second ? 4 : 1; }
    static constexpr int SPR = RS / 16;
    static constexpr size_t buf_bytes(int terms) { return ((size_t)terms * CCF * RS + 4095) / 4096 * 4096; }
};

template <int TERMS> __device__ __forceinline__ f32x16 mma32_split(const u32x4 (&a)[TERMS], const u32x4 (&b)[TERMS], f32x16 c) {
    c = mfma32_bf16(a[0], b[0], c);
    if constexpr (TERMS == 2) { c = mfma32_bf16(a[1], b[0], c); c = mfma32_bf16(a[0], b[1], c); }
    return c;
}

template <int TERMS> __device__ __forceinline__ void acc_to_frags(const f32x16& v, u32x4 (&f0)[TERMS], u32x4 (&f1)[TERMS]) {
#pragma unroll
    for (int jj = 0; jj < 4; ++jj) {
        unsigned h, l;
        split_bf16(lrelu(v[2 * jj]), lrelu(v[2 * jj + 1]), h, l); f0[0][jj] = h; if constexpr (TERMS == 2) f0[1][jj] = l;
        split_bf16(lrelu(v[8 + 2 * jj]), lrelu(v[8 + 2 * jj + 1]), h, l); f1[0][jj] = h; if constexpr (TERMS == 2) f1[1][jj] = l;
    }
}

__device__ __forceinline__ f32x16 bias_rows(const float* b, int ch0, int lh) {
    f32x16 v;
#pragma unroll
    for (int g = 0; g < 4; ++g) {
        const float4 t = *reinterpret_cast<const float4*>(b + ch0 + 8 * g + 4 * lh);
        v[4 * g] = t.x; v[4 * g + 1] = t.y; v[4 * g + 2] = t.z; v[4 * g + 3] = t.w;
    }
    return v;
}
__device__ __forceinline__ f32x16 bias_cols(const float* b, int ch0, int lr) {
    const float t = b[ch0 + lr];
    f32x16 v;
#pragma unroll
    for (int q = 0; q < 16; ++q) v[q] = t;
    return v;
}

template <int TERMS> __device__ __forceinline__ u32x4 rel_fragment_x(float px, float py, float pz, float qx, float qy, float qz, int lh) {
    const float dx = px - qx, dy = py - qy, dz = pz - qz;
    const float x[7] = {sqrtf(dx * dx + dy * dy + dz * dz), dx, dy, dz, px, py, pz};
    const unsigned p01 = pack_bf16(x[0], x[1]), p23 = pack_bf16(x[2], x[3]), p45 = pack_bf16(x[4], x[5]);
    u32x4 f;
    if constexpr (TERMS == 2) {
        const float r0 = x[0] - bf16_lo_f32(p01), r1 = x[1] - bf16_hi_f32(p01), r2 = x[2] - bf16_lo_f32(p23), r3 = x[3] - bf16_hi_f32(p23);
        const float r4 = x[4] - bf16_lo_f32(p45), r5 = x[5] - bf16_hi_f32(p45);
        const unsigned p6 = pack_bf16(x[6], r0);
        const float r6 = x[6] - bf16_lo_f32(p6);
        f[0] = lh ? pack_bf16(r1, r2) : p01; f[1] = lh ? pack_bf16(r3, r4) : p23; f[2] = lh ? pack_bf16(r5, r6) : p45; f[3] = lh ? 0u : p6;
    } else {
        f[0] = lh ? 0u : p01; f[1] = lh ? 0u : p23; f[2] = lh ? 0u : p45; f[3] = lh ? 0u : pack_bf16(x[6], 0.f);
    }
    return f;
}
template <int TERMS> __device__ __forceinline__ u32x4 rel_fragment(const float* xyz, int p, int j, int lh) {
    return rel_fragment_x<TERMS>(xyz[3 * (size_t)p], xyz[3 * (size_t)p + 1], xyz[3 * (size_t)p + 2], xyz[3 * (size_t)j], xyz[3 * (size_t)j + 1], xyz[3 * (size_t)j + 2], lh);
}

__device__ __forceinline__ float softmax_wsum(const f32x16& s, const float (&f)[16]) {
    float m = fmaxf(fmaxf(fmaxf(s[0], s[1]), fmaxf(s[2], s[3])), fmaxf(fmaxf(s[4], s[5]), fmaxf(s[6], s[7])));
    m = fmaxf(m, fmaxf(fmaxf(fmaxf(s[8], s[9]), fmaxf(s[10], s[11])), fmaxf(fmaxf(s[12], s[13]), fmaxf(s[14], s[15]))));
    float den = 0.f, num = 0.f;
#pragma unroll
    for (int q = 0; q < 16; ++q) { const float e = fast_exp2(s[q] - m); den += e; num = fmaf(f[q], e, num); }
    return num * fast_rcp(den);
}

template <int D, bool SECOND, int TERMS>
__global__ __launch_bounds__(Lfa32Cfg<D>::nw(SECOND) * 64) SSDR_WAVES_PER_EU((D >= 256 && !SECOND) ? 2 : 1) void lfa32_kernel(Lfa32Args a) {
    using C = Lfa32Cfg<D>;
    constexpr int NW = C::nw(SECOND), NT = NW * 64;
    constexpr int H = C::H, KS = C::KS, HT = C::HT, CT = C::CT, CCF = C::CCF, CC2 = C::CC2, NF = C::NF, N2 = SECOND ? C::N2 : 0, RS = C::RS;
    constexpr int NCH = N2 + NF;
    constexpr int TPW = C::tpw(SECOND);
    static_assert(TPW == 1 || NCH <= 2, "several pairs per wave only where the staged weights stay");
    constexpr size_t BUFB = C::buf_bytes(TERMS);
    constexpr bool OFFREG = H <= 64;
    constexpr bool W1REG = H <= 64;
    __shared__ __attribute__((aligned(16))) char ldsA[BUFB];
    __shared__ __attribute__((aligned(16))) char ldsB[NCH > 1 ? BUFB : 16];
    const int tid = threadIdx.x, lane = tid & 63, w = tid >> 6;
    const int lr = lane & 31, lh = lane >> 5;
    int bx, b; xcd_tile_map(bx, b);
    const int n = a.n;
    const float* xyz = a.xyz + (size_t)b * a.xyz_batch_stride;
    const int* neigh = a.neigh + (size_t)b * n * 16;

    constexpr int MAXP = (TERMS * CCF * (H / 8) + NT - 1) / NT;
    u32x4 stg[MAXP];
    auto stage_load = [&](int i) {
        const bool is2 = SECOND && i < N2;
        const int rows = is2 ? CC2 : CCF, per = rows * (H / 8);
        const size_t base = is2 ? (size_t)i * CC2 * H : (size_t)(i - N2) * CCF * H;
        const uint16_t* hi = (is2 ? a.w2_hi : a.fc_hi) + base; const uint16_t* lo = (is2 ? a.w2_lo : a.fc_lo) + base;
#pragma unroll
        for (int p = 0; p < MAXP; ++p) {
            const int e = tid + NT * p;
            if (e < TERMS * per) { const int t = e >= per ? 1 : 0; stg[p] = ld128g((t ? lo : hi) + (size_t)(e - t * per) * 8); }
        }
    };
    auto stage_store = [&](int i, char* buf) {
        const bool is2 = SECOND && i < N2;
        const int rows = is2 ? CC2 : CCF, per = rows * (H / 8);
#pragma unroll
        for (int p = 0; p < MAXP; ++p) {
            const int e = tid + NT * p;
            if (e < TERMS * per) { const int t = e >= per ? 1 : 0, r = e - t * per; st128s(buf + (size_t)t * rows * RS + (size_t)(r / (H / 8)) * RS + (r % (H / 8)) * 16, stg[p]); }
        }
    };
    stage_load(0);
    u32x4 w1r[W1REG ? HT : 1][TERMS];
    auto w1_frag = [&](int t, int term) { return ld128g(a.w1p + ((size_t)(32 * t + lr) * 2 + term) * 16 + 8 * lh); };
    if constexpr (W1REG) {
#pragma unroll
        for (int t = 0; t < HT; ++t)
#pragma unroll
            for (int term = 0; term < TERMS; ++term) w1r[t][term] = w1_frag(t, term);
    }
    auto w1_get = [&](int t, u32x4 (&f)[TERMS]) {
#pragma unroll
        for (int term = 0; term < TERMS; ++term) { if constexpr (W1REG) f[term] = w1r[t][term]; else f[term] = w1_frag(t, term); }
    };
    const rsrc32_t rG = make_rsrc32(a.g + (size_t)b * n * D, (unsigned)n * D * 4u);
    const rsrc32_t rF = make_rsrc32(a.fin + (size_t)b * n * H, (unsigned)n * H * 4u);

    for (int it = 0; it < TPW; ++it) {
    const int rt = (bx * NW + w) * TPW + it;
    const bool active = 2 * rt < n;
    if (it > 0 && !active) break;

    u32x4 relf = {0u, 0u, 0u, 0u};
    unsigned goff[16], foff[OFFREG ? 16 : 1];
    const int pc = min(2 * rt + lh, n - 1);
    {
        const int pr = min(2 * rt + ((lr >> 2) & 1), n - 1);
        const int j = neigh[(size_t)pr * 16 + (lr & 3) + 4 * (lr >> 3)];
        relf = rel_fragment<TERMS>(xyz, pr, j, lh);
        const int4* nb4 = reinterpret_cast<const int4*>(neigh + (size_t)pc * 16);
#pragma unroll
        for (int g4 = 0; g4 < 4; ++g4) {
            const int4 v = nb4[g4];
            const int nb[4] = {v.x, v.y, v.z, v.w};
#pragma unroll
            for (int r = 0; r < 4; ++r) {
                goff[4 * g4 + r] = (unsigned)nb[r] * (unsigned)(D * 4) + (unsigned)lr * 4u;
                if constexpr (OFFREG) foff[4 * g4 + r] = (unsigned)nb[r] * (unsigned)(H * 4) + (unsigned)lr * 4u;
            }
        }
    }
    auto f_off = [&](int q) -> unsigned { if constexpr (OFFREG) return foff[q]; else return (goff[q] + (unsigned)lr * 4u) >> 1; };

    u32x4 Tf[KS][TERMS];
#pragma unroll
    for (int t = 0; t < HT; ++t) {
        u32x4 wf[TERMS]; w1_get(t, wf);
        f32x16 acc = bias_rows(a.b1, 32 * t, lh);
        acc = mfma32_bf16(wf[0], relf, acc);
        if constexpr (TERMS == 2) acc = mfma32_bf16(wf[1], relf, acc);
        acc_to_frags<TERMS>(acc, Tf[2 * t], Tf[2 * t + 1]);
    }
    auto x1_tile = [&](int t, float (&x)[16]) {
        u32x4 wf[TERMS]; w1_get(t, wf);
        f32x16 acc = bias_cols(a.b1, 32 * t, lr);
        acc = mfma32_bf16(relf, wf[0], acc);
        if constexpr (TERMS == 2) acc = mfma32_bf16(relf, wf[1], acc);
#pragma unroll
        for (int q = 0; q < 16; ++q) x[q] = lrelu(acc[q]);
    };

    if (it == 0) stage_store(0, ldsA);
    float x2[SECOND ? HT : 1][16];
    u32x4 T2f[SECOND ? KS : 1][TERMS];
    auto score_frag = [&](int s) -> const u32x4 (&)[TERMS] { if constexpr (SECOND) return T2f[s]; else return Tf[s]; };

    float gn[16];
#pragma unroll
    for (int q = 0; q < 16; ++q) gn[q] = buf_load_s(rG, goff[q], 0u);

    auto wfrag = [&](const char* img, int rows, int tile, int s, u32x4 (&f)[TERMS]) {
#pragma unroll
        for (int term = 0; term < TERMS; ++term) f[term] = ld128g(img + (size_t)term * rows * RS + (size_t)(32 * tile + lr) * RS + (16 * s + 8 * lh) * 2);
    };

#pragma unroll
    for (int i = 0; i < NCH; ++i) {
        char* buf = (i & 1) ? ldsB : ldsA;
        if (it == 0) {
            __syncthreads();
            if (i + 1 < NCH) stage_load(i + 1);
        }
        if (SECOND && i < N2) {
            if (active) {
#pragma unroll
                for (int tt = 0; tt < CC2 / 32; ++tt) {
                    const int t2 = i * (CC2 / 32) + tt;
                    f32x16 accT = bias_rows(a.b2, 32 * t2, lh), accX = bias_cols(a.b2, 32 * t2, lr);
                    u32x4 wa[TERMS], wb[TERMS];
                    wfrag(buf, CC2, tt, 0, wa);
#pragma unroll
                    for (int s = 0; s < KS; s += 2) {
                        wfrag(buf, CC2, tt, s + 1, wb);
                        SSDR_SCHED_FENCE();
                        accT = mma32_split<TERMS>(wa, Tf[s], accT);
                        accX = mma32_split<TERMS>(Tf[s], wa, accX);
                        SSDR_SCHED_FENCE();
                        if (s + 2 < KS) wfrag(buf, CC2, tt, s + 2, wa);
                        SSDR_SCHED_FENCE();
                        accT = mma32_split<TERMS>(wb, Tf[s + 1], accT);
                        accX = mma32_split<TERMS>(Tf[s + 1], wb, accX);
                        SSDR_SCHED_FENCE();
                    }
                    if constexpr (SECOND) {
#pragma unroll
                        for (int q = 0; q < 16; ++q) x2[t2][q] = lrelu(accX[q]);
                        acc_to_frags<TERMS>(accT, T2f[2 * t2], T2f[2 * t2 + 1]);
                    }
                }
            }
        } else {
            if (active) {
#pragma unroll
                for (int uu = 0; uu < CCF / 32; ++uu) {
                    const int u = (i - N2) * (CCF / 32) + uu;
                    u32x4 wa[TERMS], wb[TERMS];
                    wfrag(buf, CCF, uu, 0, wa);
                    f32x16 acc;
#pragma unroll
                    for (int q = 0; q < 16; ++q) acc[q] = gn[q];
                    if (u + 1 < CT) {
#pragma unroll
                        for (int q = 0; q < 16; ++q) gn[q] = buf_load_s(rG, goff[q], (unsigned)(u + 1) * 128u);
                    }
                    float fv[16];
                    if (u < HT) {
#pragma unroll
                        for (int q = 0; q < 16; ++q) fv[q] = buf_load_s(rF, f_off(q), (unsigned)u * 128u);
                    }
                    static_assert(KS % 2 == 0, "k steps in pairs");
                    SSDR_SCHED_FENCE();
#pragma unroll
                    for (int s = 0; s < KS; s += 2) {
                        wfrag(buf, CCF, uu, s + 1, wb);
                        SSDR_SCHED_FENCE();
                        acc = mma32_split<TERMS>(score_frag(s), wa, acc);
                        SSDR_SCHED_FENCE();
                        if (s + 2 < KS) wfrag(buf, CCF, uu, s + 2, wa);
                        SSDR_SCHED_FENCE();
                        acc = mma32_split<TERMS>(score_frag(s + 1), wb, acc);
                        SSDR_SCHED_FENCE();
                    }
                    if (u >= HT) {
                        if constexpr (SECOND) {
#pragma unroll
                            for (int q = 0; q < 16; ++q) fv[q] = x2[u - HT][q];
                        } else x1_tile(u - HT, fv);
                    }
                    const float v = softmax_wsum(acc, fv);
                    if (2 * rt + lh < n) a.out[((size_t)b * n + (size_t)(2 * rt + lh)) * D + 32 * u + lr] = v;
                }
            }
        }
        if (it == 0 && i + 1 < NCH) stage_store(i + 1, (i & 1) ? ldsA : ldsB);
    }
    }
}

template <int D> struct Lfa32ResCfg {
    static constexpr int H = D / 2, RS = 2 * H + 16;
    static constexpr int NW = 4;
    static constexpr int RPW = 8;
    static constexpr int FRS = H * 4 + 16;
    static constexpr size_t w_bytes(int terms, bool second) { return (size_t)terms * ((second ? H : 0) + 2 * D) * RS; }
    static constexpr size_t lds_bytes(int terms, bool second) { return w_bytes(terms, second) + (size_t)NW * 32 * FRS; }
};

template <int D, bool SECOND, int TERMS>
__global__ __launch_bounds__(Lfa32ResCfg<D>::NW * 64) void lfa32_res_kernel(Lfa32Args a) {
    using C = Lfa32ResCfg<D>;
    constexpr int H = C::H, KS = H / 16, HT = H / 32, CT = D / 32, RS = C::RS, RPW = C::RPW, NW = C::NW, FRS = C::FRS;
    SSDR_DYN_SHARED(float, smem);
    char* lds = reinterpret_cast<char*>(smem);
    char* const img2 = lds;
    char* const imgp = lds + (SECOND ? (size_t)TERMS * H * RS : 0);
    char* const imgn = imgp + (size_t)TERMS * D * RS;
    const int tid = threadIdx.x, lane = tid & 63, w = tid >> 6;
    char* const fimg = lds + C::w_bytes(TERMS, SECOND) + (size_t)w * 32 * FRS;
    const int lr = lane & 31, lh = lane >> 5;
    int bx, b; xcd_tile_map(bx, b);
    const int n = a.n;
    const float* xyz = a.xyz + (size_t)b * a.xyz_batch_stride;
    const int* neigh = a.neigh + (size_t)b * n * 16;
    const float* finb = a.fin + (size_t)b * n * H;
    {
        constexpr int P8 = H / 8, N2P = SECOND ? TERMS * H * P8 : 0, NFP = TERMS * 2 * D * P8;
        for (int e = tid; e < N2P + NFP; e += NW * 64) {
            const bool is2 = e < N2P;
            const int r = is2 ? e : e - N2P, rows = is2 ? H : 2 * D, per = rows * P8, t = r >= per ? 1 : 0, q = r - t * per;
            const uint16_t* src = (is2 ? (t ? a.w2_lo : a.w2_hi) : (t ? a.fc_lo : a.fc_hi)) + (size_t)q * 8;
            const int row = q / P8;
            char* dst = is2 ? img2 + (size_t)t * H * RS + (size_t)row * RS : (row < D ? imgp + (size_t)t * D * RS + (size_t)row * RS : imgn + (size_t)t * D * RS + (size_t)(row - D) * RS);
            st128s(dst + (q % P8) * 16, ld128g(src));
        }
    }
    u32x4 w1r[HT][TERMS];
#pragma unroll
    for (int t = 0; t < HT; ++t)
#pragma unroll
        for (int term = 0; term < TERMS; ++term) w1r[t][term] = ld128g(a.w1p + ((size_t)(32 * t + lr) * 2 + term) * 16 + 8 * lh);
    const int nbrrow = (lr & 3) + 4 * (lr >> 3), prow = (lr >> 2) & 1;
    __syncthreads();

    const int rt0 = ((int)bx * NW + w) * RPW;
    for (int it = 0; it < RPW; ++it) {
        const int rt = rt0 + it;
        if (2 * rt >= n) break;
        const int pr = min(2 * rt + prow, n - 1);
        const int j = neigh[(size_t)pr * 16 + nbrrow];
        const float* fj = finb + (size_t)j * H + 8 * lh;
        float4 fa[KS][2];
#pragma unroll
        for (int s2 = 0; s2 < KS; ++s2) { fa[s2][0] = *reinterpret_cast<const float4*>(fj + 16 * s2); fa[s2][1] = *reinterpret_cast<const float4*>(fj + 16 * s2 + 4); }
        const u32x4 relf = rel_fragment<TERMS>(xyz, pr, j, lh);
        u32x4 fnf[KS][TERMS];
        wave_sync();
#pragma unroll
        for (int s2 = 0; s2 < KS; ++s2) {
            float4* dst = reinterpret_cast<float4*>(fimg + (size_t)lr * FRS + (16 * s2 + 8 * lh) * 4);
            dst[0] = fa[s2][0]; dst[1] = fa[s2][1];
            const float f[8] = {fa[s2][0].x, fa[s2][0].y, fa[s2][0].z, fa[s2][0].w, fa[s2][1].x, fa[s2][1].y, fa[s2][1].z, fa[s2][1].w};
#pragma unroll
            for (int k2 = 0; k2 < 4; ++k2) { unsigned hh, ll; split_bf16(f[2 * k2], f[2 * k2 + 1], hh, ll); fnf[s2][0][k2] = hh; if constexpr (TERMS == 2) fnf[s2][1][k2] = ll; }
        }
        wave_sync();
        u32x4 Tf[KS][TERMS];
#pragma unroll
        for (int t = 0; t < HT; ++t) {
            f32x16 acc = bias_rows(a.b1, 32 * t, lh);
            acc = mfma32_bf16(w1r[t][0], relf, acc);
            if constexpr (TERMS == 2) acc = mfma32_bf16(w1r[t][1], relf, acc);
            acc_to_frags<TERMS>(acc, Tf[2 * t], Tf[2 * t + 1]);
        }
        float x2[SECOND ? HT : 1][16];
        if constexpr (SECOND) {
            u32x4 T2f[KS][TERMS];
#pragma unroll
            for (int t2 = 0; t2 < HT; ++t2) {
                f32x16 accT = bias_rows(a.b2, 32 * t2, lh), accX = bias_cols(a.b2, 32 * t2, lr);
                u32x4 wa[TERMS], wb[TERMS];
                auto w2f = [&](int s2, u32x4 (&f)[TERMS]) {
#pragma unroll
                    for (int term = 0; term < TERMS; ++term) f[term] = ld128g(img2 + (size_t)term * H * RS + (size_t)(32 * t2 + lr) * RS + (16 * s2 + 8 * lh) * 2);
                };
                w2f(0, wa);
#pragma unroll
                for (int s2 = 0; s2 < KS; s2 += 2) {
                    w2f(s2 + 1, wb);
                    accT = mma32_split<TERMS>(wa, Tf[s2], accT);
                    accX = mma32_split<TERMS>(Tf[s2], wa, accX);
                    if (s2 + 2 < KS) w2f(s2 + 2, wa);
                    accT = mma32_split<TERMS>(wb, Tf[s2 + 1], accT);
                    accX = mma32_split<TERMS>(Tf[s2 + 1], wb, accX);
                }
#pragma unroll
                for (int q = 0; q < 16; ++q) x2[t2][q] = lrelu(accX[q]);
                acc_to_frags<TERMS>(accT, T2f[2 * t2], T2f[2 * t2 + 1]);
            }
#pragma unroll
            for (int s2 = 0; s2 < KS; ++s2)
#pragma unroll
                for (int term = 0; term < TERMS; ++term) Tf[s2][term] = T2f[s2][term];
        }
#pragma unroll
        for (int u = 0; u < CT; ++u) {
            f32x16 acc;
#pragma unroll
            for (int q = 0; q < 16; ++q) acc[q] = 0.f;
            float fv[16];
            if (u < HT) {
#pragma unroll
                for (int q = 0; q < 16; ++q) fv[q] = *reinterpret_cast<const float*>(fimg + (size_t)((q & 3) + 8 * (q >> 2) + 4 * lh) * FRS + (32 * u + lr) * 4);
            }
            u32x4 wa[2][TERMS], wb[2][TERMS];
            auto wsf = [&](int s2, u32x4 (&f)[2][TERMS]) {
#pragma unroll
                for (int term = 0; term < TERMS; ++term) {
                    f[0][term] = ld128g(imgn + (size_t)term * D * RS + (size_t)(32 * u + lr) * RS + (16 * s2 + 8 * lh) * 2);
                    f[1][term] = ld128g(imgp + (size_t)term * D * RS + (size_t)(32 * u + lr) * RS + (16 * s2 + 8 * lh) * 2);
                }
            };
            wsf(0, wa);
#pragma unroll
            for (int s2 = 0; s2 < KS; s2 += 2) {
                wsf(s2 + 1, wb);
                acc = mma32_split<TERMS>(fnf[s2], wa[0], acc);
                acc = mma32_split<TERMS>(Tf[s2], wa[1], acc);
                if (s2 + 2 < KS) wsf(s2 + 2, wa);
                acc = mma32_split<TERMS>(fnf[s2 + 1], wb[0], acc);
                acc = mma32_split<TERMS>(Tf[s2 + 1], wb[1], acc);
            }
            if (u < HT) {
            } else if constexpr (SECOND) {
#pragma unroll
                for (int q = 0; q < 16; ++q) fv[q] = x2[u - HT][q];
            } else {
                f32x16 ax = bias_cols(a.b1, 32 * (u - HT), lr);
                ax = mfma32_bf16(relf, w1r[u - HT][0], ax);
                if constexpr (TERMS == 2) ax = mfma32_bf16(relf, w1r[u - HT][1], ax);
#pragma unroll
                for (int q = 0; q < 16; ++q) fv[q] = lrelu(ax[q]);
            }
            const float v = softmax_wsum(acc, fv);
            if (2 * rt + lh < n) a.out[((size_t)b * n + (size_t)(2 * rt + lh)) * D + 32 * u + lr] = v;
        }
    }
}

constexpr int L0_TPW = 8;
constexpr int L0_IMG = 64 * 32 + 32, L0_ZERO = 1024, L0_WAVE = L0_IMG + L0_ZERO;

template <bool SECOND, int TERMS>
__global__ __launch_bounds__(256) void lfa32_l0_kernel(Lfa32Args a) {
    __shared__ __attribute__((aligned(16))) char l0lds[4 * L0_WAVE];
    const int tid = threadIdx.x, lane = tid & 63, w = tid >> 6;
    const int lr = lane & 31, lh = lane >> 5, cc = lr & 15, sg = lr >> 4;
    int bx, b; xcd_tile_map(bx, b);
    const int n = a.n;
    const int* neigh = a.neigh + (size_t)b * n * 16;
    const float* tabb = a.fin + (size_t)b * n * 16;
    char* const img = l0lds + w * L0_WAVE;
    for (int i = lane; i < L0_ZERO / 4; i += 64) reinterpret_cast<float*>(img + L0_IMG)[i] = 0.f;
    auto tab = [&](const uint16_t* t, int f) { return ld128g(t + ((size_t)f * 64 + lane) * 8); };
    u32x4 locT[TERMS], locX[TERMS], w2T[SECOND ? TERMS : 1], w2X[SECOND ? TERMS : 1], fcB[TERMS], fcN[TERMS];
#pragma unroll
    for (int t = 0; t < TERMS; ++t) {
        locT[t] = tab(a.w1p, t); locX[t] = tab(a.w1p, 2 + t);
        fcB[t] = tab(t ? a.fc_lo : a.fc_hi, 0); fcN[t] = tab(t ? a.fc_lo : a.fc_hi, 1);
        if constexpr (SECOND) { w2T[t] = tab(t ? a.w2_lo : a.w2_hi, 0); w2X[t] = tab(t ? a.w2_lo : a.w2_hi, 1); }
    }
    u32x4 onesA = {0u, 0u, 0u, 0u}, biasB = {0u, 0u, 0u, 0u};
    float b2r[8];
    if constexpr (SECOND) {
        if (lh == 0) { onesA[0] = 0x3f803f80u; if (cc >= 8) { const float bv = a.b2[cc - 8]; unsigned h, l; split_bf16(bv, 0.f, h, l); biasB[0] = (h & 0xffffu) | (TERMS == 2 ? (l << 16) : 0u); } }
#pragma unroll
        for (int q = 0; q < 8; ++q) b2r[q] = a.b2[q];
    }
    const float slope = cc < 8 ? 1.f : 0.2f;
    float* out = a.out + (size_t)b * n * 16;
    const int g0 = ((int)bx * 4 + w) * L0_TPW;
    const int nbrrow = (lr & 3) + 4 * (lr >> 3), prow = 2 * lh + ((lr >> 2) & 1), pcol = 2 * sg + lh;
    char* const wrow = img + lane * 32 + lh * 32;
    const char* const rbase = cc < 8 ? img + (32 * (pcol >> 1) + 4 * (pcol & 1)) * 32 + (pcol >> 1) * 32 + cc * 4 : img + L0_IMG;
    for (int it = 0; it < L0_TPW; ++it) {
        const int t = g0 + it;
        if (4 * t >= n) break;
        const int pr = min(4 * t + prow, n - 1);
        const int j = neigh[(size_t)pr * 16 + nbrrow];
        const float4 pp = *reinterpret_cast<const float4*>(tabb + (size_t)pr * 16);
        const float4* rowj = reinterpret_cast<const float4*>(tabb + (size_t)j * 16);
        const float4 qq = rowj[0], fa0 = rowj[1], fa1 = rowj[2];
        wave_sync();
        reinterpret_cast<float4*>(wrow)[0] = fa0; reinterpret_cast<float4*>(wrow)[1] = fa1;
        u32x4 rel[TERMS], fnA[TERMS];
        {
            const float dx = pp.x - qq.x, dy = pp.y - qq.y, dz = pp.z - qq.z;
            const float v[8] = {sqrtf(dx * dx + dy * dy + dz * dz), dx, dy, dz, pp.x, pp.y, pp.z, 1.f};
            const float f[8] = {fa0.x, fa0.y, fa0.z, fa0.w, fa1.x, fa1.y, fa1.z, fa1.w};
#pragma unroll
            for (int k2 = 0; k2 < 4; ++k2) {
                unsigned h, l;
                split_bf16(v[2 * k2], v[2 * k2 + 1], h, l); rel[0][k2] = h; if constexpr (TERMS == 2) rel[1][k2] = l;
                split_bf16(f[2 * k2], f[2 * k2 + 1], h, l); fnA[0][k2] = h; if constexpr (TERMS == 2) fnA[1][k2] = l;
            }
        }
        wave_sync();
        f32x16 accX;
#pragma unroll
        for (int q = 0; q < 16; ++q) accX[q] = *reinterpret_cast<const float*>(rbase + ((q & 3) + 8 * (q >> 2)) * 32);
        f32x16 accS, accT;
#pragma unroll
        for (int q = 0; q < 16; ++q) { accS[q] = 0.f; accT[q] = 0.f; }
        accS = mma32_split<TERMS>(fnA, fcN, accS);
        accT = mma32_split<TERMS>(locT, rel, accT);
        u32x4 Tf[TERMS];
        auto to_frag = [&](const f32x16& v, u32x4 (&f)[TERMS]) {
#pragma unroll
            for (int jj = 0; jj < 4; ++jj) { unsigned h, l; split_bf16(lrelu(v[2 * jj]), lrelu(v[2 * jj + 1]), h, l); f[0][jj] = h; if constexpr (TERMS == 2) f[1][jj] = l; }
        };
        to_frag(accT, Tf);
        if constexpr (SECOND) {
            f32x16 acc2;
#pragma unroll
            for (int q = 0; q < 16; ++q) acc2[q] = q < 8 ? b2r[q] : 0.f;
            acc2 = mma32_split<TERMS>(w2T, Tf, acc2);
            accX = mfma32_bf16(onesA, biasB, accX);
            accX = mma32_split<TERMS>(Tf, w2X, accX);
            to_frag(acc2, Tf);
        } else {
            accX = mma32_split<TERMS>(rel, locX, accX);
        }
        float fv[16];
#pragma unroll
        for (int q = 0; q < 16; ++q) fv[q] = fmaxf(accX[q], accX[q] * slope);
        accS = mma32_split<TERMS>(Tf, fcB, accS);
        const float v = softmax_wsum(accS, fv);
        const int pcu = 4 * t + pcol;
        if (pcu < n) out[(size_t)pcu * 16 + cc] = v;
    }
}

static int launch_lfa32_l0(const Lfa32Args& a, bool second, int B, int prec, hipStream_t s) {
    dim3 grid((unsigned)((a.n + 16 * L0_TPW - 1) / (16 * L0_TPW)), (unsigned)B);
    const int terms = prec == PREC_BF16X3 ? 2 : 1;
    const double rows = (double)B * (double)a.n * 16.0, np = terms == 2 ? 3.0 : 1.0;
    const double exec = (double)B * std::ceil(a.n / 4.0) * 2.0 * 32 * 32 * 16 * (np * (second ? 5.0 : 4.0) + (second ? 1.0 : 0.0));
    ProfScope prof("lfa32_l0_kernel", s, rows * (2.0 * 10 * 8 + (second ? 2.0 * 8 * 8 : 0.0) + 2.0 * 16 * 16 + 2.0 * 16), exec);
    if (terms == 2) {
        if (second) hipLaunchKernelGGL((lfa32_l0_kernel<true, 2>), grid, dim3(256), 0, s, a);
        else hipLaunchKernelGGL((lfa32_l0_kernel<false, 2>), grid, dim3(256), 0, s, a);
    } else {
        if (second) hipLaunchKernelGGL((lfa32_l0_kernel<true, 1>), grid, dim3(256), 0, s, a);
        else hipLaunchKernelGGL((lfa32_l0_kernel<false, 1>), grid, dim3(256), 0, s, a);
    }
    SSDR_HIP(hipGetLastError());
    return SSDR_OK;
}

template <int D> static int launch_lfa32_d(const Lfa32Args& a, bool second, int B, int prec, hipStream_t s) {
    using C = Lfa32Cfg<D>;
    const int nw = C::nw(second);
    dim3 grid((unsigned)((a.n + 2 * nw * C::tpw(second) - 1) / (2 * nw * C::tpw(second))), (unsigned)B);
    const int terms = prec == PREC_BF16X3 ? 2 : 1;
    const double rows = (double)B * (double)a.n * 16.0;
    const double np = terms == 2 ? 3.0 : 1.0;
    const double exec = rows * (2.0 * 2.0 * 16 * C::H * terms + (second ? 2.0 * 2.0 * C::H * C::H * np : 0.0) + 2.0 * C::H * D * np);
    ProfScope prof(D == 128 ? "lfa32_kernel<128>" : D == 256 ? "lfa32_kernel<256>" : "lfa32_kernel<512>", s, rows * (2.0 * 10 * C::H + (second ? 2.0 * C::H * C::H : 0.0) + 2.0 * D * D + 2.0 * D), exec);
    if (terms == 2) {
        if (second) hipLaunchKernelGGL((lfa32_kernel<D, true, 2>), grid, dim3(nw * 64), 0, s, a);
        else hipLaunchKernelGGL((lfa32_kernel<D, false, 2>), grid, dim3(nw * 64), 0, s, a);
    } else {
        if (second) hipLaunchKernelGGL((lfa32_kernel<D, true, 1>), grid, dim3(nw * 64), 0, s, a);
        else hipLaunchKernelGGL((lfa32_kernel<D, false, 1>), grid, dim3(nw * 64), 0, s, a);
    }
    SSDR_HIP(hipGetLastError());
    return SSDR_OK;
}

template <int D> static int launch_lfa32_res(const Lfa32Args& a, bool second, int B, int prec, hipStream_t s) {
    using C = Lfa32ResCfg<D>;
    dim3 grid((unsigned)((a.n + 2 * C::NW * C::RPW - 1) / (2 * C::NW * C::RPW)), (unsigned)B);
    const int terms = prec == PREC_BF16X3 ? 2 : 1;
    const size_t lds = C::lds_bytes(terms, second);
    static std::once_flag attr_once;
    hipError_t ae = hipSuccess;
    std::call_once(attr_once, [&] {
        ae = hipFuncSetAttribute(reinterpret_cast<const void*>(&lfa32_res_kernel<D, true, 2>), hipFuncAttributeMaxDynamicSharedMemorySize, (int)C::lds_bytes(2, true));
        if (ae == hipSuccess) ae = hipFuncSetAttribute(reinterpret_cast<const void*>(&lfa32_res_kernel<D, false, 2>), hipFuncAttributeMaxDynamicSharedMemorySize, (int)C::lds_bytes(2, false));
        if (ae == hipSuccess) ae = hipFuncSetAttribute(reinterpret_cast<const void*>(&lfa32_res_kernel<D, true, 1>), hipFuncAttributeMaxDynamicSharedMemorySize, (int)C::lds_bytes(1, true));
        if (ae == hipSuccess) ae = hipFuncSetAttribute(reinterpret_cast<const void*>(&lfa32_res_kernel<D, false, 1>), hipFuncAttributeMaxDynamicSharedMemorySize, (int)C::lds_bytes(1, false));
    });
    SSDR_HIP(ae);
    const double rows = (double)B * (double)a.n * 16.0, np = terms == 2 ? 3.0 : 1.0;
    const double exec = rows * (2.0 * 2.0 * 16 * C::H * terms + (second ? 2.0 * 2.0 * C::H * C::H * np : 0.0) + 2.0 * D * D * np);
    ProfScope prof("lfa32_res_kernel<64>", s, rows * (2.0 * 10 * C::H + (second ? 2.0 * C::H * C::H : 0.0) + 2.0 * D * D + 2.0 * D), exec);
    const dim3 blk(C::NW * 64);
    if (terms == 2) {
        if (second) hipLaunchKernelGGL((lfa32_res_kernel<D, true, 2>), grid, blk, lds, s, a);
        else hipLaunchKernelGGL((lfa32_res_kernel<D, false, 2>), grid, blk, lds, s, a);
    } else {
        if (second) hipLaunchKernelGGL((lfa32_res_kernel<D, true, 1>), grid, blk, lds, s, a);
        else hipLaunchKernelGGL((lfa32_res_kernel<D, false, 1>), grid, blk, lds, s, a);
    }
    SSDR_HIP(hipGetLastError());
    return SSDR_OK;
}

int launch_lfa32(int D, const Lfa32Args& a, bool second, int B, int prec, hipStream_t s) {
    if (a.n <= 0 || B <= 0) return SSDR_OK;
    if ((!a.g && D > 64) || !a.fc_hi || !a.w1p || (second && !a.w2_hi)) { set_error("lfa32: missing G rows or permuted weight pieces"); return SSDR_ERR_INVALID; }
    switch (D) {
        case 16: return launch_lfa32_l0(a, second, B, prec, s);
        case 64: return launch_lfa32_res<64>(a, second, B, prec, s);
        case 128: return launch_lfa32_d<128>(a, second, B, prec, s);
        case 256: return launch_lfa32_d<256>(a, second, B, prec, s);
        case 512: return launch_lfa32_d<512>(a, second, B, prec, s);
        default: return SSDR_ERR_UNSUPPORTED;
    }
}

}
```

ssdr-al_amd/csrc/randla_model.hip:

```cpp
#include "ssdr_internal.hpp"
#include "randla.hpp"
#include <cstring>

namespace ssdr {
namespace {

struct Layer {
    int in = 0, out = 0; bool has_b = true; DevBuf W, b, Wt; bool set = false;
    DevBuf Wh, Wl; int kp = 0;
    DevBuf Ph, Pl, P1;
};

struct Model {
    int L = 5, K = 16, C = 13, in_dim = 6;
    int prec = PREC_F32;
    int tiles32 = 1;
    int d_out[8] = {16, 64, 128, 256, 512, 0, 0, 0};
    std::vector<Layer> layers;
    std::vector<DevBuf> ws;
};

int n_layers(const Model& m) { return 1 + 8 * m.L + 1 + m.L + 3; }

void shapes(Model& m) {
    m.layers.clear(); m.layers.resize(n_layers(m));
    auto set = [&](int i, int in, int out, bool b) { m.layers[i].in = in; m.layers[i].out = out; m.layers[i].has_b = b; };
    set(0, m.in_dim, 8, true);
    int d_in = 8;
    std::vector<int> enc_ch; enc_ch.push_back(2 * m.d_out[0]);
    for (int i = 0; i < m.L; ++i) {
        const int d = m.d_out[i], h = d / 2, base = 1 + 8 * i;
        set(base + 0, d_in, h, true); set(base + 1, 10, h, true); set(base + 2, d, d, false); set(base + 3, d, h, true);
        set(base + 4, h, h, true); set(base + 5, d, d, false); set(base + 6, d, d, true); set(base + 7, d + d_in, 2 * d, true);
        d_in = 2 * d; enc_ch.push_back(2 * d);
    }
    int idx = 1 + 8 * m.L;
    set(idx++, d_in, d_in, true);
    int feat = d_in;
    for (int j = 0; j < m.L; ++j) { const int skip = enc_ch[enc_ch.size() - j - 2]; set(idx++, skip + feat, skip, true); feat = skip; }
    set(idx++, feat, 64, true); set(idx++, 64, 32, true); set(idx++, 32, m.C, true);
}

DenseArgs dense(const float* x1, int k1, const Layer& ly, float* y, int M, int act) {
    DenseArgs a{}; a.x1 = x1; a.k1 = k1; a.x2 = nullptr; a.k2 = 0; a.idx2 = nullptr; a.m_per_batch = 1; a.x2_rows_per_batch = 0;
    a.W = ly.W.as<float>(); a.b = ly.has_b ? ly.b.as<float>() : nullptr; a.y = y; a.M = M; a.N = ly.out; a.act = act;
    a.wt_hi = ly.Wh.as<uint16_t>(); a.wt_lo = ly.Wl.as<uint16_t>(); a.kp = ly.kp;
    return a;
}

uint16_t bf16_rn(float f) { uint32_t u; memcpy(&u, &f, 4); return (uint16_t)((u + 0x7fffu + ((u >> 16) & 1u)) >> 16); }
float bf16_f32(uint16_t h) { uint32_t u = (uint32_t)h << 16; float f; memcpy(&f, &u, 4); return f; }

int kperm_src(int pos) { const int h = pos >> 3, j = pos & 7; return 8 * (j >> 2) + 4 * h + (j & 3); }

int permuted_pieces(Layer& ly, const float* W, int k0, int K, double scale, bool with_natural = false) {
    std::vector<uint16_t> hi((size_t)ly.out * K * (with_natural ? 2 : 1)), lo(hi.size());
    for (int x = 0; x < ly.out; ++x)
        for (int kb = 0; kb < K; kb += 16)
            for (int pos = 0; pos < 16; ++pos) {
                const float v = (float)((double)W[(size_t)(k0 + kb + kperm_src(pos)) * ly.out + x] * scale);
                const uint16_t h = bf16_rn(v);
                hi[(size_t)x * K + kb + pos] = h; lo[(size_t)x * K + kb + pos] = bf16_rn(v - bf16_f32(h));
            }
    if (with_natural)
        for (int x = 0; x < ly.out; ++x)
            for (int k = 0; k < K; ++k) {
                const float v = (float)((double)W[(size_t)k * ly.out + x] * scale);
                const uint16_t h = bf16_rn(v);
                hi[(size_t)(ly.out + x) * K + k] = h; lo[(size_t)(ly.out + x) * K + k] = bf16_rn(v - bf16_f32(h));
            }
    SSDR_TRY(ly.Ph.reserve(2 * hi.size())); SSDR_TRY(ly.Pl.reserve(2 * lo.size()));
    SSDR_HIP(hipMemcpy(ly.Ph.p, hi.data(), 2 * hi.size(), hipMemcpyHostToDevice));
    SSDR_HIP(hipMemcpy(ly.Pl.p, lo.data(), 2 * lo.size(), hipMemcpyHostToDevice));
    return SSDR_OK;
}

int locse_fragments(Layer& ly, const float* W) {
    std::vector<uint16_t> f((size_t)ly.out * 32, 0);
    for (int c = 0; c < ly.out; ++c) {
        double w7[7];
        w7[0] = W[c];
        for (int a = 0; a < 3; ++a) { w7[1 + a] = (double)W[(size_t)(1 + a) * ly.out + c] - (double)W[(size_t)(7 + a) * ly.out + c]; w7[4 + a] = (double)W[(size_t)(4 + a) * ly.out + c] + (double)W[(size_t)(7 + a) * ly.out + c]; }
        for (int i = 0; i < 7; ++i) {
            const float v = (float)w7[i];
            const uint16_t h = bf16_rn(v), l = bf16_rn(v - bf16_f32(h));
            const int s0 = i, s1 = i == 0 ? 7 : 7 + i;
            f[(size_t)c * 32 + s0] = h; f[(size_t)c * 32 + s1] = h;
            f[(size_t)c * 32 + 16 + s0] = l; f[(size_t)c * 32 + 16 + s1] = l;
        }
    }
    SSDR_TRY(ly.P1.reserve(2 * f.size()));
    SSDR_HIP(hipMemcpy(ly.P1.p, f.data(), 2 * f.size(), hipMemcpyHostToDevice));
    return SSDR_OK;
}

template <class F> void level0_fragment(std::vector<uint16_t>& hi, std::vector<uint16_t>& lo, bool transposed, bool pos_only, F&& weight ) {
    for (int l = 0; l < 64; ++l) {
        const int r = l & 31, hh = l >> 5;
        int pair, ch; bool used;
        if (transposed) { pair = (r >> 2) & 1; ch = (r & 3) + 4 * (r >> 3); used = r < 16; }
        else { pair = r >> 4; ch = r & 15; used = !pos_only || ch >= 8; if (pos_only) ch -= 8; }
        for (int j = 0; j < 8; ++j) {
            uint16_t h = 0, lw = 0;
            if (used && pair == hh) { const float v = weight(j, ch); h = bf16_rn(v); lw = bf16_rn(v - bf16_f32(h)); }
            hi.push_back(h); lo.push_back(lw);
        }
    }
}
int upload16(DevBuf& d, const std::vector<uint16_t>& v) {
    SSDR_TRY(d.reserve(2 * v.size()));
    SSDR_HIP(hipMemcpy(d.p, v.data(), 2 * v.size(), hipMemcpyHostToDevice));
    return SSDR_OK;
}
int level0_tables(Layer& ly, int role, const float* W, const float* b) {
    std::vector<uint16_t> hi, lo;
    if (role == 1) {
        auto w8 = [&](int j, int c) -> float {
            if (j == 0) return W[c];
            if (j < 4) return (float)((double)W[(size_t)j * 8 + c] - (double)W[(size_t)(6 + j) * 8 + c]);
            if (j < 7) return (float)((double)W[(size_t)j * 8 + c] + (double)W[(size_t)(3 + j) * 8 + c]);
            return b[c];
        };
        std::vector<uint16_t> th, tl, xh, xl;
        level0_fragment(th, tl, true, false, w8); level0_fragment(xh, xl, false, true, w8);
        std::vector<uint16_t> all; all.insert(all.end(), th.begin(), th.end()); all.insert(all.end(), tl.begin(), tl.end());
        all.insert(all.end(), xh.begin(), xh.end()); all.insert(all.end(), xl.begin(), xl.end());
        return upload16(ly.P1, all);
    }
    if (role == 4) {
        auto w = [&](int j, int c) -> float { return W[(size_t)j * 8 + c]; };
        std::vector<uint16_t> xh, xl;
        level0_fragment(hi, lo, true, false, w); level0_fragment(xh, xl, false, true, w);
        hi.insert(hi.end(), xh.begin(), xh.end()); lo.insert(lo.end(), xl.begin(), xl.end());
    } else {
        for (int half = 1; half >= 0; --half) {
            auto w = [&](int j, int c) -> float { return (float)((double)W[(size_t)(8 * half + j) * 16 + c] * 1.4426950408889634); };
            level0_fragment(hi, lo, false, false, w);
        }
    }
    SSDR_TRY(upload16(ly.Ph, hi));
    return upload16(ly.Pl, lo);
}

int run_dense(const Model& m, const DenseArgs& a, hipStream_t s) { return m.prec == PREC_F32 ? launch_dense(a, s) : launch_dense_bf16(a, m.prec, s); }

}
}

using namespace ssdr;

extern "C" {

int ssdr_randla_create(int num_layers, const int32_t* d_out, int k_n, int num_classes, int in_dim, void** handle) {
    if (!handle || !d_out || num_layers < 1 || num_layers > 8) { set_error("randla_create: bad arguments"); return SSDR_ERR_INVALID; }
    if (k_n != 16) { set_error("randla: k_n=%d is not supported (16)", k_n); return SSDR_ERR_UNSUPPORTED; }
    if (num_classes < 1 || num_classes > 32) { set_error("randla: num_classes must be in [1,32]"); return SSDR_ERR_UNSUPPORTED; }
    if (in_dim < 1) { set_error("randla: in_dim=%d: the input features need at least one channel", in_dim); return SSDR_ERR_UNSUPPORTED; }
    for (int i = 0; i < num_layers; ++i)
        if (d_out[i] != 16 && d_out[i] != 64 && d_out[i] != 128 && d_out[i] != 256 && d_out[i] != 512) { set_error("randla: d_out[%d]=%d is not supported", i, d_out[i]); return SSDR_ERR_UNSUPPORTED; }
    Model* m = new Model();
    m->L = num_layers; m->K = k_n; m->C = num_classes; m->in_dim = in_dim;
    for (int i = 0; i < num_layers; ++i) m->d_out[i] = d_out[i];
    shapes(*m);
    *handle = m;
    return SSDR_OK;
}

int ssdr_randla_num_layers(void* handle) { return handle ? n_layers(*static_cast<Model*>(handle)) : 0; }

int ssdr_randla_layer_shape(void* handle, int layer, int* in, int* out, int* has_bias) {
    Model* m = static_cast<Model*>(handle);
    if (!m || layer < 0 || layer >= n_layers(*m)) { set_error("randla_layer_shape: bad layer"); return SSDR_ERR_INVALID; }
    if (in) *in = m->layers[layer].in;
    if (out) *out = m->layers[layer].out;
    if (has_bias) *has_bias = m->layers[layer].has_b;
    return SSDR_OK;
}

int ssdr_randla_set_layer(void* handle, int layer, const float* W, const float* b) {
    Model* m = static_cast<Model*>(handle);
    if (!m || layer < 0 || layer >= n_layers(*m) || !W) { set_error("randla_set_layer: bad arguments"); return SSDR_ERR_INVALID; }
    SSDR_TRY(ensure_init());
    Layer& ly = m->layers[layer];
    if (ly.has_b && !b) { set_error("randla_set_layer: layer %d needs a bias", layer); return SSDR_ERR_INVALID; }
    SSDR_TRY(ly.W.reserve(sizeof(float) * (size_t)ly.in * ly.out));
    SSDR_HIP(hipMemcpy(ly.W.p, W, sizeof(float) * (size_t)ly.in * ly.out, hipMemcpyHostToDevice));
    if (ly.has_b) { SSDR_TRY(ly.b.reserve(sizeof(float) * ly.out)); SSDR_HIP(hipMemcpy(ly.b.p, b, sizeof(float) * ly.out, hipMemcpyHostToDevice)); }
    if (!ly.has_b && ly.in == ly.out) {
        std::vector<float> t((size_t)ly.in * ly.out);
        for (int k = 0; k < ly.in; ++k) for (int c = 0; c < ly.out; ++c) t[(size_t)c * ly.in + k] = W[(size_t)k * ly.out + c];
        SSDR_TRY(ly.Wt.reserve(sizeof(float) * t.size()));
        SSDR_HIP(hipMemcpy(ly.Wt.p, t.data(), sizeof(float) * t.size(), hipMemcpyHostToDevice));
    }
    {
        ly.kp = (ly.in + 63) / 64 * 64;
        std::vector<uint16_t> hi((size_t)ly.out * ly.kp, 0), lo((size_t)ly.out * ly.kp, 0);
        const double scale = (!ly.has_b && ly.in == ly.out) ? 1.4426950408889634 : 1.0;
        for (int k = 0; k < ly.in; ++k)
            for (int c = 0; c < ly.out; ++c) {
                const float v = (float)((double)W[(size_t)k * ly.out + c] * scale);
                const uint16_t h = bf16_rn(v);
                hi[(size_t)c * ly.kp + k] = h; lo[(size_t)c * ly.kp + k] = bf16_rn(v - bf16_f32(h));
            }
        SSDR_TRY(ly.Wh.reserve(2 * hi.size())); SSDR_TRY(ly.Wl.reserve(2 * lo.size()));
        SSDR_HIP(hipMemcpy(ly.Wh.p, hi.data(), 2 * hi.size(), hipMemcpyHostToDevice));
        SSDR_HIP(hipMemcpy(ly.Wl.p, lo.data(), 2 * lo.size(), hipMemcpyHostToDevice));
    }
    if (layer >= 1 && layer < 1 + 8 * m->L) {
        const int r = (layer - 1) % 8;
        if (m->d_out[(layer - 1) / 8] == 16 && (r == 1 || r == 2 || r == 4 || r == 5)) SSDR_TRY(level0_tables(ly, r == 5 ? 2 : r, W, b));
        else if (r == 1 && ly.in == 10) SSDR_TRY(locse_fragments(ly, W));
        else if (r == 4 && ly.in % 16 == 0) SSDR_TRY(permuted_pieces(ly, W, 0, ly.in, 1.0));
        else if ((r == 2 || r == 5) && ly.in % 32 == 0) SSDR_TRY(permuted_pieces(ly, W, ly.in / 2, ly.in / 2, 1.4426950408889634, true));
    }
    ly.set = true;
    return SSDR_OK;
}

int ssdr_randla_set_precision(void* handle, int mode) {
    Model* m = static_cast<Model*>(handle);
    if (!m || (mode != PREC_F32 && mode != PREC_BF16X3 && mode != PREC_BF16)) { set_error("randla_set_precision: mode must be 0 (f32), 1 (split bf16) or 2 (bf16)"); return SSDR_ERR_INVALID; }
    m->prec = mode;
    return SSDR_OK;
}

int ssdr_randla_set_formulation(void* handle, int tiles32) {
    Model* m = static_cast<Model*>(handle);
    if (!m) { set_error("randla_set_formulation: bad handle"); return SSDR_ERR_INVALID; }
    m->tiles32 = tiles32 ? 1 : 0;
    return SSDR_OK;
}

void ssdr_randla_destroy(void* handle) {
    Model* m = static_cast<Model*>(handle);
    if (!m) return;
    for (auto& l : m->layers) { l.W.release(); l.b.release(); l.Wt.release(); l.Wh.release(); l.Wl.release(); l.Ph.release(); l.Pl.release(); l.P1.release(); }
    for (auto& w : m->ws) w.release();
    delete m;
}

}

namespace ssdr {
namespace {

int infer_levels(Model* m, size_t B, size_t n0, const std::vector<int>& N, const float* d_features, const float* d_xyz,
                 int32_t* const* d_neigh_idx, int32_t* const* d_interp_idx, float* d_probs, float* d_feat32, hipStream_t s) {
    const int L = m->L, Bi = (int)B;

    size_t need = 0;
    auto idxs = [&](int level, int which) { return level * 6 + which; };
    if (m->ws.size() < (size_t)(6 * L + 7)) m->ws.resize(6 * L + 7);
    auto buf = [&](int slot, size_t floats) -> float* { if (m->ws[slot].reserve(floats * 4) != SSDR_OK) return nullptr; (void)need; return m->ws[slot].as<float>(); };

    float* f0 = buf(6 * L + 0, B * N[0] * 8); if (!f0) return SSDR_ERR_HIP;
    const DenseArgs a_fc0 = dense(d_features, m->in_dim, m->layers[0], f0, Bi * N[0], 1);
    if (L < 1) { set_error("randla_infer: no encoder level"); return SSDR_ERR_INVALID; }
    const float* f = f0; int d_in = 8;
    std::vector<const float*> enc; std::vector<int> enc_ch, enc_n;
    for (int i = 0; i < L; ++i) {
        const int d = m->d_out[i], h = d / 2, base = 1 + 8 * i, n = N[i];
        const size_t rows = B * (size_t)n;
        float* f_pc = buf(idxs(i, 0), rows * h); float* agg = buf(idxs(i, 1), rows * d); float* aggm = buf(idxs(i, 2), rows * d);
        float* out = buf(idxs(i, 3), rows * 2 * d); float* samp = buf(idxs(i, 4), B * (size_t)N[i + 1] * 2 * d);
        if (!f_pc || !agg || !aggm || !out || !samp) return SSDR_ERR_HIP;
        const bool use32 = m->prec != PREC_F32 && m->tiles32 != 0;
        float* tab0 = nullptr;
        if (use32 && d == 16) { tab0 = buf(6 * L + 5, rows * 16); if (!tab0) return SSDR_ERR_HIP; }
        {
            DenseArgs a1 = dense(f, d_in, m->layers[base + 0], tab0 ? tab0 + 4 : f_pc, (int)rows, 1);
            if (tab0) { a1.ldy = 16; a1.xyz = d_xyz; a1.xyz_batch_stride = n0 * 3; a1.xyz_rows_per_batch = n; }
            if (i == 0) {
                const int fused = launch_dense_rows2(a_fc0, a1, s);
                if (fused == SSDR_ERR_UNSUPPORTED) { SSDR_TRY(run_dense(*m, a_fc0, s)); SSDR_TRY(run_dense(*m, a1, s)); }
                else SSDR_TRY(fused);
            } else SSDR_TRY(run_dense(*m, a1, s));
        }
        LfaArgs la{}; la.xyz = d_xyz; la.xyz_batch_stride = n0 * 3; la.neigh = d_neigh_idx[i]; la.n = n;
        la.w_l1 = m->layers[base + 1].W.as<float>(); la.b_l1 = m->layers[base + 1].b.as<float>();
        la.w_l2 = m->layers[base + 4].W.as<float>(); la.b_l2 = m->layers[base + 4].b.as<float>();
        la.fin = f_pc; la.w_fc = m->layers[base + 2].W.as<float>(); la.w_fc_t = m->layers[base + 2].Wt.as<float>(); la.out = agg;
        la.fc_hi = m->layers[base + 2].Wh.as<uint16_t>(); la.fc_lo = m->layers[base + 2].Wl.as<uint16_t>();
        la.l2_hi = m->layers[base + 4].Wh.as<uint16_t>(); la.l2_lo = m->layers[base + 4].Wl.as<uint16_t>(); la.kp2 = m->layers[base + 4].kp;
        const bool lfa16 = m->prec != PREC_F32 && d >= 64;
        float* gbuf = nullptr;
        if (d >= 64 && !(use32 && d <= 64)) {
            gbuf = buf(idxs(i, 5), rows * d); if (!gbuf) return SSDR_ERR_HIP;
            DenseArgs ga{}; ga.x1 = f_pc; ga.k1 = h; ga.W = la.w_fc; ga.b = nullptr; ga.y = gbuf; ga.M = (int)rows; ga.N = d; ga.act = 0; ga.m_per_batch = 1;
            ga.wt_hi = la.fc_hi; ga.wt_lo = la.fc_lo; ga.kp = m->layers[base + 2].kp;
            SSDR_TRY(run_dense(*m, ga, s));
        }
        la.g = gbuf;
        Lfa32Args l32{}; l32.xyz = d_xyz; l32.xyz_batch_stride = n0 * 3; l32.neigh = d_neigh_idx[i]; l32.n = n; l32.g = gbuf; l32.out = agg;
        l32.w1p = m->layers[base + 1].P1.as<uint16_t>(); l32.b1 = la.b_l1;
        l32.w2_hi = m->layers[base + 4].Ph.as<uint16_t>(); l32.w2_lo = m->layers[base + 4].Pl.as<uint16_t>(); l32.b2 = la.b_l2;
        auto run_lfa = [&](bool second, const float* fin, const Layer& fc) -> int {
            if (use32) {
                l32.fin = fin; l32.fc_hi = fc.Ph.as<uint16_t>(); l32.fc_lo = fc.Pl.as<uint16_t>();
                const int rc = launch_lfa32(d, l32, second, Bi, m->prec, s);
                if (rc != SSDR_ERR_UNSUPPORTED) return rc;
                if (tab0 || !gbuf) { set_error("randla: the 32 x 32-tile attention kernel refused d = %d and the level's buffers were laid out for it", d); return SSDR_ERR_INTERNAL; }
            }
            return lfa16 ? launch_lfa_bf16(d, la, second, Bi, m->prec, s) : launch_lfa(d, la, second, Bi, s);
        };
        SSDR_TRY(run_lfa(false, tab0 ? tab0 : f_pc, m->layers[base + 2]));
        {
            DenseArgs a3 = dense(agg, d, m->layers[base + 3], tab0 ? tab0 + 4 : aggm, (int)rows, 1);
            if (tab0) a3.ldy = 16;
            SSDR_TRY(run_dense(*m, a3, s));
        }
        la.fin = aggm; la.w_fc = m->layers[base + 5].W.as<float>(); la.w_fc_t = m->layers[base + 5].Wt.as<float>(); la.out = agg;
        la.fc_hi = m->layers[base + 5].Wh.as<uint16_t>(); la.fc_lo = m->layers[base + 5].Wl.as<uint16_t>();
        if (gbuf) {
            DenseArgs ga{}; ga.x1 = aggm; ga.k1 = h; ga.W = la.w_fc; ga.b = nullptr; ga.y = gbuf; ga.M = (int)rows; ga.N = d; ga.act = 0; ga.m_per_batch = 1;
            ga.wt_hi = la.fc_hi; ga.wt_lo = la.fc_lo; ga.kp = m->layers[base + 5].kp;
            SSDR_TRY(run_dense(*m, ga, s));
        }
        SSDR_TRY(run_lfa(true, tab0 ? tab0 : aggm, m->layers[base + 5]));
        DenseArgs a6 = dense(agg, d, m->layers[base + 6], aggm, (int)rows, 1);
        DenseArgs r = dense(aggm, d, m->layers[base + 7], out, (int)rows, 1);
        r.x2 = f; r.k2 = d_in;
        int chained = m->prec != PREC_F32 ? launch_dense_chain(a6, r, m->prec, s) : SSDR_ERR_UNSUPPORTED;
        if (chained == SSDR_ERR_UNSUPPORTED) { SSDR_TRY(run_dense(*m, a6, s)); SSDR_TRY(run_dense(*m, r, s)); }
        else SSDR_TRY(chained);
        SSDR_TRY(launch_gather_max(out, d_neigh_idx[i], n, N[i + 1], n, 2 * d, samp, Bi, s));
        if (i == 0) { enc.push_back(out); enc_ch.push_back(2 * d); enc_n.push_back(n); }
        enc.push_back(samp); enc_ch.push_back(2 * d); enc_n.push_back(N[i + 1]);
        f = samp; d_in = 2 * d;
    }
    int li = 1 + 8 * L;
    float* dec = buf(6 * L + 1, B * (size_t)N[L] * d_in); if (!dec) return SSDR_ERR_HIP;
    SSDR_TRY(run_dense(*m, dense(enc.back(), d_in, m->layers[li++], dec, Bi * N[L], 1), s));
    const float* feat = dec; int feat_c = d_in, feat_n = N[L];
    const Layer& l1 = m->layers[li + L]; const Layer& l2 = m->layers[li + L + 1]; const Layer& fc = m->layers[li + L + 2];
    const bool tail16 = m->prec != PREC_F32 && l1.in == 32 && l1.out == 64 && l2.out == 32 && l1.has_b && l2.has_b && fc.has_b && (m->C == 13 || m->C == 8);
    TailArgs t{};
    for (int j = 0; j < L; ++j) {
        const int e = (int)enc.size() - j - 2;
        const int skip_c = enc_ch[e], n = enc_n[e];
        const Layer& ld = m->layers[li];
        if (j == L - 1 && tail16 && skip_c == 32 && feat_c == 32 && ld.has_b) {
            t.skip = enc[e]; t.up = feat; t.idx = d_interp_idx[L - 1 - j]; t.m_per_batch = n; t.up_rows_per_batch = feat_n;
            t.wdh = ld.Wh.as<uint16_t>(); t.wdl = ld.Wl.as<uint16_t>(); t.kpd = ld.kp; t.bd = ld.b.as<float>();
            ++li; feat = nullptr; feat_c = skip_c; feat_n = n;
            break;
        }
        float* y = buf(6 * L + 2 + (j & 1), B * (size_t)n * skip_c); if (!y) return SSDR_ERR_HIP;
        DenseArgs a = dense(enc[e], skip_c, m->layers[li++], y, Bi * n, 1);
        a.x2 = feat; a.k2 = feat_c; a.idx2 = d_interp_idx[L - 1 - j]; a.m_per_batch = n; a.x2_rows_per_batch = feat_n;
        SSDR_TRY(run_dense(*m, a, s));
        feat = y; feat_c = skip_c; feat_n = n;
    }
    int fused = SSDR_ERR_UNSUPPORTED;
    if (tail16 && feat_c == 32) {
        t.x = feat; t.M = Bi * N[0]; t.C = m->C;
        t.w1h = l1.Wh.as<uint16_t>(); t.w1l = l1.Wl.as<uint16_t>(); t.kp1 = l1.kp; t.b1 = l1.b.as<float>();
        t.w2h = l2.Wh.as<uint16_t>(); t.w2l = l2.Wl.as<uint16_t>(); t.kp2 = l2.kp; t.b2 = l2.b.as<float>();
        t.w3h = fc.Wh.as<uint16_t>(); t.w3l = fc.Wl.as<uint16_t>(); t.kp3 = fc.kp; t.b3 = fc.b.as<float>();
        t.feat32 = d_feat32; t.probs = d_probs;
        fused = launch_tail_bf16(t, m->prec, s);
        if (fused == SSDR_ERR_UNSUPPORTED && t.skip) { set_error("randla: the fused decoder + tail kernel refused its arguments"); return SSDR_ERR_INTERNAL; }
    }
    if (fused == SSDR_ERR_UNSUPPORTED && feat_c == 32 && l1.out == 64 && l2.out == 32 && l1.has_b && l2.has_b)
        fused = launch_tail(feat, l1.W.as<float>(), l1.b.as<float>(), l2.W.as<float>(), l2.b.as<float>(), fc.W.as<float>(), fc.b.as<float>(),
                            Bi * N[0], m->C, d_feat32, d_probs, s);
    if (fused == SSDR_ERR_UNSUPPORTED) {
        float* f1 = buf(6 * L + 4, B * (size_t)N[0] * 64); if (!f1) return SSDR_ERR_HIP;
        SSDR_TRY(run_dense(*m, dense(feat, feat_c, l1, f1, Bi * N[0], 1), s));
        SSDR_TRY(run_dense(*m, dense(f1, 64, l2, d_feat32, Bi * N[0], 1), s));
        SSDR_TRY(launch_head(d_feat32, fc.W.as<float>(), fc.b.as<float>(), Bi * N[0], m->C, d_probs, s));
    } else SSDR_TRY(fused);
    return SSDR_OK;
}

}
}

extern "C" {

int ssdr_randla_infer_dev(void* handle, size_t B, size_t n0, const float* d_features, const float* d_xyz,
                          const int32_t* ratios, int32_t* const* d_neigh_idx, int32_t* const* d_interp_idx,
                          float* d_probs, float* d_feat32, void* stream) {
    Model* m = static_cast<Model*>(handle);
    if (!m || !d_features || !d_xyz || !ratios || !d_neigh_idx || !d_interp_idx || !d_probs || !d_feat32 || B == 0 || n0 == 0) { set_error("randla_infer: bad arguments"); return SSDR_ERR_INVALID; }
    for (auto& l : m->layers) if (!l.set) { set_error("randla_infer: not every layer has weights"); return SSDR_ERR_INVALID; }
    SSDR_TRY(ensure_init());
    hipStream_t s = pick_stream(stream);
    const int L = m->L;
    std::vector<int> N(L + 1); N[0] = (int)n0;
    for (int i = 0; i < L; ++i) { if (ratios[i] <= 0) { set_error("ratio must be positive"); return SSDR_ERR_INVALID; } N[i + 1] = N[i] / ratios[i]; }
    if (N[L] <= 0) { set_error("randla_infer: tile too small for the pyramid"); return SSDR_ERR_INVALID; }
    return infer_levels(m, B, n0, N, d_features, d_xyz, d_neigh_idx, d_interp_idx, d_probs, d_feat32, s);
}

int ssdr_randla_infer_rows_dev(void* handle, const size_t* level_rows, const float* d_features, const float* d_xyz,
                               int32_t* const* d_neigh_idx, int32_t* const* d_interp_idx, float* d_probs, float* d_feat32, void* stream) {
    Model* m = static_cast<Model*>(handle);
    if (!m || !level_rows || !d_features || !d_xyz || !d_neigh_idx || !d_interp_idx || !d_probs || !d_feat32) { set_error("randla_infer_rows: bad arguments"); return SSDR_ERR_INVALID; }
    for (auto& l : m->layers) if (!l.set) { set_error("randla_infer_rows: not every layer has weights"); return SSDR_ERR_INVALID; }
    const int L = m->L;
    if (level_rows[0] > SSDR_PREDICT_MAX_ROWS) { set_error("randla_infer_rows: %zu level-0 rows (cap %d = 2^23: int32 element offsets)", level_rows[0], SSDR_PREDICT_MAX_ROWS); return SSDR_ERR_UNSUPPORTED; }
    std::vector<int> N(L + 1);
    for (int i = 0; i <= L; ++i) {
        if (level_rows[i] == 0 || (i > 0 && level_rows[i] > level_rows[i - 1])) {
            set_error("randla_infer_rows: level table must be positive and non-increasing (level %d: %zu rows, level above: %zu)", i, level_rows[i], i > 0 ? level_rows[i - 1] : 0);
            return SSDR_ERR_INVALID;
        }
        N[i] = (int)level_rows[i];
    }
    SSDR_TRY(ensure_init());
    return infer_levels(m, 1, level_rows[0], N, d_features, d_xyz, d_neigh_idx, d_interp_idx, d_probs, d_feat32, pick_stream(stream));
}

}
```

ssdr-al_amd/ssdr_al/_lib.py:

```python
import ctypes as C
import os

import numpy as np

_PKG = os.path.dirname(os.path.dirname(os.path.abspath(__file__)))
DEFAULT_PATH = os.path.join(_PKG, "libssdr_al.so")

SSDR_OK = 0
ORDER_REFERENCE, ORDER_KEY = 0, 1

_lib = None
_forced_path = None
_libs = {}


class SsdrError(RuntimeError):
    def __init__(self, status, msg):
        super().__init__("libssdr_al status %d: %s" % (status, msg))
        self.status = status


def lib_path():
    return _forced_path or os.environ.get("SSDR_AL_LIBRARY", DEFAULT_PATH)


def use(path):
    global _lib, _forced_path
    _forced_path = path
    _lib = None


def lib():
    global _lib
    if _lib is None:
        path = lib_path()
        if path in _libs:
            _lib = _libs[path]
            return _lib
        if not os.path.exists(path):
            raise SsdrError(-1, "%s not found: build it with `python -c 'import __graft_entry__ as g; g.build()'` "
                                "(hipcc --offload-arch=gfx950); there is no CPU fallback" % path)
        L = C.CDLL(path)
        vp, sz, f32, i32 = C.c_void_p, C.c_size_t, C.c_float, C.c_int
        L.ssdr_version.restype = C.c_char_p
        L.ssdr_last_error.restype = C.c_char_p
        L.ssdr_last_gpu_ms.restype = C.c_float
        L.ssdr_init.argtypes = [i32]
        L.ssdr_stream_sync.argtypes = [vp]
        L.ssdr_stream_create.argtypes = [C.POINTER(vp)]
        L.ssdr_stream_create_priority.argtypes = [C.POINTER(vp), i32]
        L.ssdr_stream_destroy.argtypes = [vp]
        L.ssdr_stream_wait.argtypes = [vp, vp]
        L.ssdr_knn.argtypes = [vp, sz, sz, vp, sz, sz, vp]
        L.ssdr_knn_batch.argtypes = [vp, sz, sz, sz, vp, sz, sz, vp]
        L.ssdr_knn_batch_i32.argtypes = [vp, sz, sz, sz, vp, sz, sz, vp]
        L.ssdr_knn_batch_dev.argtypes = [vp, sz, sz, sz, vp, sz, sz, vp, vp]
        L.ssdr_knn_status.argtypes = [vp, vp]
        L.ssdr_knn_pyramid.argtypes = [vp, sz, sz, sz, vp, sz, vp, vp, vp]
        L.ssdr_knn_pyramid_dev.argtypes = [vp, sz, sz, sz, vp, sz, vp, vp, vp, vp]
        L.ssdr_grid_subsample.argtypes = [vp, sz, vp, sz, vp, sz, f32, i32, C.POINTER(sz)]
        L.ssdr_grid_subsample_fetch.argtypes = [vp, vp, vp]
        L.ssdr_grid_subsample_dev.argtypes = [vp, sz, vp, sz, vp, sz, f32, i32, vp, vp, vp, vp, vp]
        L.ssdr_randla_create.argtypes = [i32, vp, i32, i32, i32, C.POINTER(vp)]
        L.ssdr_randla_num_layers.argtypes = [vp]
        L.ssdr_randla_layer_shape.argtypes = [vp, i32, C.POINTER(i32), C.POINTER(i32), C.POINTER(i32)]
        L.ssdr_randla_set_layer.argtypes = [vp, i32, vp, vp]
        L.ssdr_randla_set_precision.argtypes = [vp, i32]
        L.ssdr_select_status.argtypes = [vp, C.POINTER(i32)]
        L.ssdr_randla_set_formulation.argtypes = [vp, i32]
        L.ssdr_randla_destroy.argtypes = [vp]
        L.ssdr_randla_destroy.restype = None
        L.ssdr_randla_infer_dev.argtypes = [vp, sz, sz, vp, vp, vp, vp, vp, vp, vp, vp]
        f64 = C.c_double
        L.ssdr_point_uncertainty_dev.argtypes = [vp, sz, i32, i32, vp, vp, vp]
        L.ssdr_region_stats_dev.argtypes = [vp, vp, vp, vp, sz, i32, i32, vp, vp, vp, vp]
        L.ssdr_dominant_label_dev.argtypes = [vp, vp, vp, sz, i32, vp, vp, vp]
        L.ssdr_clsbal_dev.argtypes = [vp, sz, vp, vp, sz, vp, vp]
        L.ssdr_class_hist_dev.argtypes = [vp, sz, vp, vp, sz, vp, vp]
        L.ssdr_clsbal_hist_dev.argtypes = [vp, sz, vp, sz, vp, vp]
        L.ssdr_rank_regions_dev.argtypes = [vp, sz, vp, vp]
        L.ssdr_segment_mean_features_dev.argtypes = [vp, i32, vp, vp, vp, vp, vp, sz, vp, vp]
        L.ssdr_widen_f32_f64_dev.argtypes = [vp, sz, vp, vp, vp]
        L.ssdr_knn_batch_distance_pick.argtypes = [vp, sz, sz, sz, vp, sz, sz, vp, C.c_uint32]
        L.ssdr_knn_graph_dev.argtypes = [vp, sz, sz, sz, vp, vp, vp, vp, vp]
        L.ssdr_geof_dev.argtypes = [vp, sz, vp, sz, vp, vp]
        L.ssdr_cloud_graph_dev.argtypes = [vp, vp, vp, vp, sz, sz, i32, vp, vp, vp, vp]
        L.ssdr_propagate_dev.argtypes = [vp, sz, vp, vp, i32, vp, vp, vp]
        L.ssdr_cloud_graph_batch_dev.argtypes = [vp, vp, vp, vp, vp, vp, sz, sz, sz, i32, vp, vp, vp, vp]
        L.ssdr_propagate_batch_dev.argtypes = [vp, vp, vp, sz, sz, vp, vp, i32, vp, vp, vp]
        L.ssdr_fps_dev.argtypes = [vp, sz, i32, i32, sz, vp, vp]
        L.ssdr_create_adj_dev.argtypes = [vp, sz, i32, vp, vp, vp, vp, sz, sz, vp, vp, vp, vp]
        L.ssdr_gcn_fps_sampling_dev.argtypes = [vp, i32, vp, vp, vp, vp, vp, vp, vp, vp, sz, vp, vp, sz, vp, vp, sz, sz, i32, i32, i32, i32, sz, sz, sz, sz, sz, vp, vp]
        L.ssdr_fps_superpoint_dev.argtypes = [vp, vp, sz, i32, sz, vp, vp]
        L.ssdr_edcd_fps_batch_dev.argtypes = [vp, vp, vp, vp, vp, sz, sz, sz, vp, vp, vp]
        L.ssdr_edcd_sampling_dev.argtypes = [vp, vp, vp, vp, sz, vp, vp, sz, sz, sz, sz, sz, sz, vp, vp]
        L.ssdr_edcd_sampling_sharded_dev.argtypes = [vp, vp, vp, sz, vp, sz, vp, vp, i32, i32, sz, sz, sz, sz, sz, sz, sz, vp, vp]
        L.ssdr_topk_regions_dev.argtypes = [vp, sz, vp, sz, sz, sz, vp, vp, vp]
        L.ssdr_oracle_label_dev.argtypes = [vp, vp, sz, vp, vp, sz, vp, sz, vp, vp, sz, vp, sz, i32, i32, i32, f64, C.c_int64, vp, vp, vp, vp, vp, vp, sz, vp, vp, vp]
        L.ssdr_oracle_label_items_dev.argtypes = [vp, i32, sz, vp, sz, vp, vp, sz, vp, sz, vp, vp, vp]
        L.ssdr_gcn_fps_sharded_local_dev.argtypes = [vp, i32, vp, vp, vp, vp, vp, vp, vp, vp, vp, sz, sz, vp, sz, vp, vp, i32, i32, sz, sz, sz, i32, i32, sz, sz, sz, sz, sz, vp, vp, vp]
        L.ssdr_event_create.argtypes = [C.POINTER(vp)]; L.ssdr_event_record.argtypes = [vp, vp]; L.ssdr_stream_wait_event.argtypes = [vp, vp]; L.ssdr_event_destroy.argtypes = [vp]
        L.ssdr_select_set_chamfer_mode.argtypes = [i32]
        L.ssdr_gcn_fps_sampling_rows.argtypes = [vp, C.POINTER(vp), C.POINTER(sz)]
        u64 = C.c_uint64
        L.ssdr_gcn_block_adj_dev.argtypes = [vp, sz, i32, vp, vp, vp, vp, sz, sz, vp, vp, vp, vp, vp, vp, vp, vp]
        L.ssdr_gcn_train_dev.argtypes = [vp, vp, vp, vp, vp, sz, sz, vp, vp, vp, sz, vp, vp, i32, f32, f32, f32, f32, u64, i32, vp, vp, vp]
        L.ssdr_gcn_eval_dev.argtypes = [vp, vp, vp, vp, vp, sz, sz, vp, vp, vp, sz, vp, vp, vp, vp]
        L.ssdr_gcn_sampling_dev.argtypes = [vp, i32, vp, vp, vp, vp, vp, vp, vp, vp, sz, vp, vp, sz, vp, vp, sz, sz, vp, i32, f32, f32, f32, f32, u64, i32, sz, sz, sz, sz, sz, vp, vp]
        L.ssdr_gcn_sampling_rows.argtypes = [vp, C.POINTER(vp), C.POINTER(sz), C.POINTER(vp), C.POINTER(vp), C.POINTER(vp)]
        L.ssdr_kcenter_gathered_dev.argtypes = [vp, vp, i32, sz, sz, vp, sz, sz, sz, vp, vp, vp, vp]
        L.ssdr_fps_gathered_dev.argtypes = [vp, vp, i32, sz, sz, i32, i32, sz, vp, vp, vp]
        L.ssdr_kcenter_dev.argtypes = [vp, sz, i32, vp, sz, sz, vp, vp]
        L.ssdr_tile_select_dev.argtypes = [vp, vp, i32, vp, sz, vp, sz, vp, vp, f32, vp, vp, vp, vp]
        L.ssdr_grid_subsample_batch_dev.argtypes = [vp, vp, sz, vp, sz, vp, sz, f32, vp, vp, vp, vp, vp]
        L.ssdr_tile_select_batch_dev.argtypes = [vp, vp, i32, vp, vp, sz, vp, sz, vp, vp, f32, vp, vp, vp, vp, vp, vp]
        L.ssdr_tile_select_possibility_dev.argtypes = [vp, vp, i32, vp, sz, vp, sz, vp, vp, f32, vp, vp, vp, vp, vp, vp, vp]
        L.ssdr_split3_dev.argtypes = [vp, sz, sz, sz, sz, vp, vp, vp, sz, C.POINTER(sz), vp]
        L.ssdr_chamfer3d_forward_dev.argtypes = [vp, vp, sz, sz, sz, vp, vp, vp, vp, vp]
        L.ssdr_vote_smooth_dev.argtypes = [vp, vp, vp, sz, i32, f64, vp, vp]
        L.ssdr_confusion_dev.argtypes = [vp, i32, vp, vp, sz, vp, vp, vp, vp]
        L.ssdr_main_stream.argtypes = [C.POINTER(vp)]
        L.ssdr_mask_regions_dev.argtypes = [vp, vp, sz, sz, vp, vp]
        L.ssdr_gather_rows_dev.argtypes = [vp, vp, sz, sz, vp, vp]
        L.ssdr_prune_dev.argtypes = [vp, sz, f32, vp, vp, i32, vp, i32, vp, vp, vp, vp, vp, vp]
        L.ssdr_prune_status.argtypes = [vp, vp]
        L.ssdr_prof_enable.argtypes = [i32]
        L.ssdr_prof_report.restype = C.c_char_p
        L.ssdr_dev_alloc.argtypes = [sz, C.POINTER(vp)]
        L.ssdr_dev_free.argtypes = [vp]
        L.ssdr_memcpy_h2d.argtypes = [vp, vp, sz]
        L.ssdr_memcpy_d2h.argtypes = [vp, vp, sz]
        L.ssdr_memcpy_h2d_on.argtypes = [vp, vp, sz, vp]
        L.ssdr_memcpy_d2h_on.argtypes = [vp, vp, sz, vp]
        L.ssdr_knn_status_poll.argtypes = [vp, vp]
        L.ssdr_grid_subsample_status.argtypes = [vp, vp]
        L.ssdr_grid_subsample_set_method.argtypes = [i32]
        L.ssdr_randla_infer_rows_dev.argtypes = [vp, vp, vp, vp, vp, vp, vp, vp, vp]
        L.ssdr_predict_layout.argtypes = [vp, sz, sz, sz, vp, vp]
        L.ssdr_predict_tile_dev.argtypes = [vp, vp, vp, vp, sz, vp, sz, sz, vp, vp, vp, f32, vp, vp, vp, vp, vp, vp, vp]
        L.ssdr_knn_pyramid_ragged_dev.argtypes = [vp, vp, sz, sz, sz, vp, sz, vp, vp, vp]
        L.ssdr_predict_translate_dev.argtypes = [vp, sz, sz, sz, vp, sz, vp, vp, vp, vp, vp]
        L.ssdr_predict_readback_dev.argtypes = [vp, sz, sz, sz, vp, vp, vp, sz, vp, i32, vp, vp, vp]
        _lib = _libs[path] = L
    return _lib


def check(status):
    if status != SSDR_OK:
        raise SsdrError(status, lib().ssdr_last_error().decode())


def ptr(a):
    return None if a is None else a.ctypes.data_as(C.c_void_p)


def last_gpu_ms():
    return float(lib().ssdr_last_gpu_ms())


_pool = {}


def _size_class(nbytes):
    c = 256
    while c < nbytes:
        c *= 2
    return c


class DevArray:

    def __init__(self, shape, dtype):
        self.shape = tuple(int(s) for s in shape)
        self.dtype = np.dtype(dtype)
        self.nbytes = int(np.prod(self.shape)) * self.dtype.itemsize
        self._cls = _size_class(max(self.nbytes, 1))
        self._owner_lib = lib()
        free = _pool.get((id(self._owner_lib), self._cls))
        if free:
            self.ptr = free.pop()
        else:
            p = C.c_void_p()
            check(lib().ssdr_dev_alloc(self._cls, C.byref(p)))
            self.ptr = p.value

    @classmethod
    def from_host(cls, a, stream=None):
        a = np.ascontiguousarray(a)
        d = cls(a.shape, a.dtype)
        if stream is None:
            check(lib().ssdr_memcpy_h2d(d.ptr, ptr(a), d.nbytes))
        else:
            check(lib().ssdr_memcpy_h2d_on(d.ptr, ptr(a), d.nbytes, stream))
        return d

    @property
    def __cuda_array_interface__(self):
        return {"shape": self.shape, "typestr": self.dtype.str, "data": (int(self.ptr), False), "version": 2, "strides": None}

    def host_view(self):
        buf = (C.c_char * self.nbytes).from_address(int(self.ptr))
        return np.frombuffer(buf, self.dtype).reshape(self.shape)

    def to_host(self, stream=None):
        out = np.empty(self.shape, self.dtype)
        if stream is None:
            check(lib().ssdr_memcpy_d2h(ptr(out), self.ptr, self.nbytes))
        else:
            check(lib().ssdr_memcpy_d2h_on(ptr(out), self.ptr, self.nbytes, stream))
        return out

    def __del__(self):
        try:
            if self.ptr:
                free = _pool.setdefault((id(self._owner_lib), self._cls), [])
                if len(free) < 64 and self._cls <= (1 << 26):
                    free.append(self.ptr)
                else:
                    self._owner_lib.ssdr_dev_free(self.ptr)
                self.ptr = None
        except Exception:
            pass


def sync(stream=None):
    check(lib().ssdr_stream_sync(stream))
```

ssdr-al_amd/ssdr_al/randlanet.py:

```python
import ctypes as C

import numpy as np

from . import _lib
from .helper_tool import ConfigS3DIS

BN_EPS = 1e-6


def _fold(ent):
    w = np.asarray(ent["W"], np.float64)
    if ent.get("transposed"):
        w = w.T
    b = np.zeros(w.shape[1]) if ent.get("b") is None else np.asarray(ent["b"], np.float64)
    if ent.get("bn") is not None:
        g, beta, mu, var = [np.asarray(a, np.float64) for a in ent["bn"]]
        s = g / np.sqrt(var + BN_EPS)
        w = w * s[None, :]
        b = (b - mu) * s + beta
    return w, b


class Network:

    def __init__(self, config=ConfigS3DIS, in_dim=6):
        self.config = config
        self.in_dim = in_dim
        self._h = C.c_void_p()
        d = np.asarray(config.d_out, np.int32)
        _lib.check(_lib.lib().ssdr_randla_create(config.num_layers, _lib.ptr(d), config.k_n, config.num_classes, in_dim,
                                                 C.byref(self._h)))
        self._lib = _lib.lib()
        self.precision = "f32"

    def __del__(self):
        try:
            if self._h:
                self._lib.ssdr_randla_destroy(self._h)
                self._h = None
        except Exception:
            pass

    PRECISIONS = {"f32": 0, "bf16x3": 1, "bf16": 2}

    def set_precision(self, mode):
        _lib.check(_lib.lib().ssdr_randla_set_precision(self._h, self.PRECISIONS[mode]))
        self.precision = mode
        return self

    def set_formulation(self, tiles32=True):
        _lib.check(_lib.lib().ssdr_randla_set_formulation(self._h, 1 if tiles32 else 0))
        return self

    def layer_table(self, weights):
        L = self.config.num_layers
        out = [_fold(weights["fc0"])]
        for i in range(L):
            p = "Encoder_layer_%d" % i
            out.append(_fold(weights[p + "mlp1"]))
            out.append(_fold(weights[p + "LFAmlp1"]))
            out.append((np.asarray(weights[p + "LFAatt_pooling_1fc"]["W"], np.float64), None))
            out.append(_fold(weights[p + "LFAatt_pooling_1mlp"]))
            out.append(_fold(weights[p + "LFAmlp2"]))
            out.append((np.asarray(weights[p + "LFAatt_pooling_2fc"]["W"], np.float64), None))
            out.append(_fold(weights[p + "LFAatt_pooling_2mlp"]))
            w2, b2 = _fold(weights[p + "mlp2"])
            ws, bs = _fold(weights[p + "shortcut"])
            out.append((np.concatenate([w2, ws], 0), b2 + bs))
        out.append(_fold(weights["decoder_0"]))
        for j in range(L):
            out.append(_fold(weights["Decoder_layer_%d" % j]))
        out += [_fold(weights["fc1"]), _fold(weights["fc2"]), _fold(weights["fc"])]
        return out

    def load(self, weights):
        table = self.layer_table(weights)
        L = _lib.lib()
        assert L.ssdr_randla_num_layers(self._h) == len(table)
        for i, (w, b) in enumerate(table):
            cin, cout, hb = C.c_int(), C.c_int(), C.c_int()
            _lib.check(L.ssdr_randla_layer_shape(self._h, i, C.byref(cin), C.byref(cout), C.byref(hb)))
            assert w.shape == (cin.value, cout.value), "layer %d: %s vs (%d,%d)" % (i, w.shape, cin.value, cout.value)
            w32 = np.ascontiguousarray(w, np.float32)
            b32 = None if b is None else np.ascontiguousarray(b, np.float32)
            _lib.check(L.ssdr_randla_set_layer(self._h, i, _lib.ptr(w32), _lib.ptr(b32)))
        return self

    def infer_dev(self, B, N, d_features, d_xyz, d_neigh, d_interp, d_probs, d_feat, stream=None):
        L = self.config.num_layers
        arr = C.c_void_p * L
        r = np.asarray(self.config.sub_sampling_ratio, np.int32)
        _lib.check(_lib.lib().ssdr_randla_infer_dev(self._h, B, N, d_features, d_xyz, _lib.ptr(r), arr(*d_neigh), arr(*d_interp),
                                                    d_probs, d_feat, stream))

    def infer(self, features, xyz):
        cfg = self.config
        features = np.ascontiguousarray(features, np.float32)
        xyz = np.ascontiguousarray(xyz, np.float32)
        B, N = xyz.shape[0], xyz.shape[1]
        L, K = cfg.num_layers, cfg.k_n
        sizes = [N]
        for r in cfg.sub_sampling_ratio:
            sizes.append(sizes[-1] // r)
        d_xyz = _lib.DevArray.from_host(xyz)
        d_feat_in = _lib.DevArray.from_host(features)
        neigh = [_lib.DevArray((B, sizes[i], K), np.int32) for i in range(L)]
        interp = [_lib.DevArray((B, sizes[i], 1), np.int32) for i in range(L)]
        arr = C.c_void_p * L
        r = np.asarray(cfg.sub_sampling_ratio, np.int32)
        _lib.check(_lib.lib().ssdr_knn_pyramid_dev(d_xyz.ptr, B, N, L, _lib.ptr(r), K, arr(*[a.ptr for a in neigh]), None,
                                                   arr(*[a.ptr for a in interp]), None))
        probs = _lib.DevArray((B * N, cfg.num_classes), np.float32)
        feat = _lib.DevArray((B * N, 32), np.float32)
        self.infer_dev(B, N, d_feat_in.ptr, d_xyz.ptr, [a.ptr for a in neigh], [a.ptr for a in interp], probs.ptr, feat.ptr)
        _lib.sync()
        return probs.to_host(), feat.to_host()
```

Baseline: 203.2.

## Fuse layer-0 attention-pool MLP and dense chain into LFA32 kernel

Adds a fused variant of the first-encoder-layer LFA32 kernel. The first pass also applies the 16→8 attention-pooling MLP and writes a second tile table, and the second pass runs the mlp2+shortcut dense chain on the pooled result in LDS and writes the block output directly. This removes two dense-kernel launches and the round-trips of the agg/aggm intermediates through global memory for layer 0. The cost is much more LDS and register use in the l0 kernel, which may lower occupancy. A new fusion mode (off/auto/always) defaults to auto, which enables the path for more than 16384 rows.

Result: no change. 204.5, median of 6 (+0.6%).

```diff
diff --git a/include/ssdr_al.h b/include/ssdr_al.h
--- a/include/ssdr_al.h
+++ b/include/ssdr_al.h
@@ -105,6 +105,7 @@
 #define SSDR_PREC_BF16 2
 int  ssdr_randla_set_precision(void* handle, int mode);
 int  ssdr_randla_set_formulation(void* handle, int tiles32);
+int  ssdr_randla_set_fusion(void* handle, int mode);
 void ssdr_randla_destroy(void* handle);
 int  ssdr_randla_infer_dev(void* handle, size_t batch_size, size_t npts, const float* d_features, const float* d_xyz,
                            const int32_t* ratios, int32_t* const* d_neigh_idx, int32_t* const* d_interp_idx,
diff --git a/ssdr-al_amd/csrc/randla.hpp b/ssdr-al_amd/csrc/randla.hpp
--- a/ssdr-al_amd/csrc/randla.hpp
+++ b/ssdr-al_amd/csrc/randla.hpp
@@ -43,6 +43,14 @@
     const uint16_t *fc_hi, *fc_lo;
 };
 
+struct L0FuseArgs {
+    const float* w; const float* b; float* tab2;
+    const float* x2;
+    const uint16_t *wa_hi, *wa_lo; int kpa; const float* ba;
+    const uint16_t *wb_hi, *wb_lo; int kpb; const float* bb;
+    float* y;
+};
+
 constexpr int PREC_F32 = 0;
 constexpr int PREC_BF16X3 = 1;
 constexpr int PREC_BF16 = 2;
@@ -65,6 +73,8 @@
 int launch_dense_chain(const DenseArgs& l1, const DenseArgs& l2, int prec, hipStream_t s);
 int launch_lfa_bf16(int D, const LfaArgs& a, bool second, int B, int prec, hipStream_t s);
 int launch_lfa32(int D, const Lfa32Args& a, bool second, int B, int prec, hipStream_t s);
+bool dense_chain_accepts(const DenseArgs& l1, const DenseArgs& l2, int prec);
+int launch_lfa32_l0_fused(const Lfa32Args& a, const L0FuseArgs& f, bool second, int B, int prec, hipStream_t s);
 int launch_gather_max(const float* f, const int* idx, int n_in, int n_out, int idx_rows, int C, float* out, int B, hipStream_t s);
 int launch_tail(const float* x, const float* W1, const float* b1, const float* W2, const float* b2, const float* W3, const float* b3,
                 int M, int C, float* feat32, float* probs, hipStream_t s);
diff --git a/ssdr-al_amd/csrc/randla_bf16.hip b/ssdr-al_amd/csrc/randla_bf16.hip
--- a/ssdr-al_amd/csrc/randla_bf16.hip
+++ b/ssdr-al_amd/csrc/randla_bf16.hip
@@ -1,19 +1,10 @@
 #include "ssdr_internal.hpp"
 #include "randla.hpp"
 #include "randla_dev.hpp"
+#include "randla_chain.hpp"
 #include <cmath>
 
 namespace ssdr {
-
-__device__ __forceinline__ u32x4 ld128(const void* p) { return *reinterpret_cast<const u32x4*>(p); }
-__device__ __forceinline__ void st128(void* p, u32x4 v) { *reinterpret_cast<u32x4*>(p) = v; }
-
-template <int TERMS>
-__device__ __forceinline__ f32x4 mma_split(const u32x4 (&a)[2], const u32x4 (&b)[2], f32x4 c) {
-    c = mfma_bf16(a[0], b[0], c);
-    if (TERMS == 2) { c = mfma_bf16(a[1], b[0], c); c = mfma_bf16(a[0], b[1], c); }
-    return c;
-}
 
 template <int TM, int KC, int TERMS, bool VEC>
 __global__ __launch_bounds__(256) SSDR_WAVES_PER_EU(TM == 128 ? 4 : 5) void dense_bf16_kernel(DenseArgs a) {
@@ -217,7 +208,8 @@
     store_w();
     __syncthreads();
     load_w(a.wb_hi, a.wb_lo, a.kpb, 0, 2 * D, K);
-    const int fr = lane & 15, fk = 8 * (lane >> 4), rbase = wr * 32;
+    const int rbase = wr * 32;
+    uint16_t* const Aw[2] = {&As[0][rbase * KS], &As[TERMS - 1][rbase * KS]};
     {
         f32x4 acc[2][CT1];
 #pragma unroll
@@ -225,82 +217,20 @@
 #pragma unroll
             for (int c = 0; c < CT1; ++c) acc[r][c] = f32x4{0.f, 0.f, 0.f, 0.f};
         const bool has1 = wc * CT1 * 16 < D;
-        if (has1) {
-#pragma unroll
-            for (int ks = 0; ks < (D + 31) / 32; ++ks) {
-                u32x4 af[2][2], bf[CT1][2];
-#pragma unroll
-                for (int r = 0; r < 2; ++r)
-#pragma unroll
-                    for (int t = 0; t < TERMS; ++t) af[r][t] = ld128(&As[t][(rbase + r * 16 + fr) * KS + ks * 32 + fk]);
-#pragma unroll
-                for (int c = 0; c < CT1; ++c)
-#pragma unroll
-                    for (int t = 0; t < TERMS; ++t) bf[c][t] = ld128(&Bs[t][((wc * CT1 + c) * 16 + fr) * KS + ks * 32 + fk]);
-#pragma unroll
-                for (int r = 0; r < 2; ++r)
-#pragma unroll
-                    for (int c = 0; c < CT1; ++c) acc[r][c] = mma_split<TERMS>(af[r], bf[c], acc[r][c]);
-            }
-        }
+        const uint16_t* const B1[2] = {&Bs[0][wc * CT1 * 16 * KS], &Bs[TERMS - 1][wc * CT1 * 16 * KS]};
+        if (has1) chain_first_mma<D, KS, TERMS, CT1>(Aw, B1, lane, acc);
         if (WC > 1) __syncthreads();
-        if (has1) {
-#pragma unroll
-            for (int c = 0; c < CT1; ++c) {
-                const int col = (wc * CT1 + c) * 16 + (lane & 15);
-                const float bias = a.ba ? a.ba[col] : 0.f;
-#pragma unroll
-                for (int r = 0; r < 2; ++r)
-#pragma unroll
-                    for (int q = 0; q < 4; ++q) {
-                        const int row = rbase + r * 16 + (lane >> 4) * 4 + q;
-                        const float v = lrelu(acc[r][c][q] + bias);
-                        unsigned hq, lq; split_bf16(v, 0.f, hq, lq);
-                        As[0][row * KS + col] = (uint16_t)(hq & 0xffffu);
-                        if (TERMS == 2) As[TERMS - 1][row * KS + col] = (uint16_t)(lq & 0xffffu);
-                    }
-            }
-        }
-    }
+        if (has1) chain_first_store<KS, TERMS, CT1>(Aw, a.ba, wc * CT1 * 16, lane, acc);
+    }
+    const uint16_t* const B2[2] = {&Bs[0][wc * CT2 * 16 * KS], &Bs[TERMS - 1][wc * CT2 * 16 * KS]};
     for (int ct = 0; ct < (2 * D + 63) / 64; ++ct) {
         __syncthreads();
         store_w();
         __syncthreads();
         if (ct + 1 < (2 * D + 63) / 64) load_w(a.wb_hi, a.wb_lo, a.kpb, (ct + 1) * 64, 2 * D, K);
         f32x4 acc[2][CT2];
-#pragma unroll
-        for (int r = 0; r < 2; ++r)
-#pragma unroll
-            for (int c = 0; c < CT2; ++c) acc[r][c] = f32x4{0.f, 0.f, 0.f, 0.f};
-#pragma unroll
-        for (int ks = 0; ks < K2P / 32; ++ks) {
-            u32x4 af[2][2], bf[CT2][2];
-#pragma unroll
-            for (int r = 0; r < 2; ++r)
-#pragma unroll
-                for (int t = 0; t < TERMS; ++t) af[r][t] = ld128(&As[t][(rbase + r * 16 + fr) * KS + ks * 32 + fk]);
-#pragma unroll
-            for (int c = 0; c < CT2; ++c)
-#pragma unroll
-                for (int t = 0; t < TERMS; ++t) bf[c][t] = ld128(&Bs[t][((wc * CT2 + c) * 16 + fr) * KS + ks * 32 + fk]);
-#pragma unroll
-            for (int r = 0; r < 2; ++r)
-#pragma unroll
-                for (int c = 0; c < CT2; ++c) acc[r][c] = mma_split<TERMS>(af[r], bf[c], acc[r][c]);
-        }
-#pragma unroll
-        for (int c = 0; c < CT2; ++c) {
-            const int col = ct * 64 + (wc * CT2 + c) * 16 + (lane & 15);
-            if (col >= 2 * D) continue;
-            const float bias = a.bb ? a.bb[col] : 0.f;
-#pragma unroll
-            for (int r = 0; r < 2; ++r)
-#pragma unroll
-                for (int q = 0; q < 4; ++q) {
-                    const int row = row0 + rbase + r * 16 + (lane >> 4) * 4 + q;
-                    if (row < a.M) a.y[(size_t)row * (2 * D) + col] = lrelu(acc[r][c][q] + bias);
-                }
-        }
+        chain_second_mma<K2P, KS, TERMS, CT2>(Aw, B2, lane, acc);
+        chain_second_store<CT2>(acc, a.bb, ct * 64 + wc * CT2 * 16, 2 * D, a.y + (size_t)(row0 + rbase) * (2 * D), 2 * D, a.M - (row0 + rbase), lane);
     }
 }
 
@@ -691,14 +621,21 @@
     return launch_dense_bf16_t<128, 32>(a, prec, vec, s);
 }
 
-int launch_dense_chain(const DenseArgs& l1, const DenseArgs& l2, int prec, hipStream_t s) {
+static int chain_k2p(const DenseArgs& l1, const DenseArgs& l2, int prec) {
     const int d = l1.k1;
     const bool shapes = l1.k2 == 0 && l1.N == d && l1.act && l2.act && l2.k1 == d && l2.N == 2 * d && l2.x1 == l1.y && l2.M == l1.M && !l2.idx2 && !l1.ldy && !l2.ldy && !l1.xyz && !l2.xyz &&
                         l2.k2 % 8 == 0 && l2.k2 > 0 && l1.wt_hi && l2.wt_hi && (prec != PREC_BF16X3 || (l1.wt_lo && l2.wt_lo)) &&
                         (((uintptr_t)l1.x1 | (uintptr_t)l2.x2) & 15) == 0 && l1.kp % 8 == 0 && l2.kp % 8 == 0;
-    if (!shapes || l1.M <= 0) return SSDR_ERR_UNSUPPORTED;
-    int k2p = 0;
-    if (d == 16 && d + l2.k2 <= 32) k2p = 32; else if (d == 64 && d + l2.k2 <= 96) k2p = 96; else return SSDR_ERR_UNSUPPORTED;
+    if (!shapes || l1.M <= 0) return 0;
+    if (d == 16 && d + l2.k2 <= 32) return 32;
+    if (d == 64 && d + l2.k2 <= 96) return 96;
+    return 0;
+}
+bool dense_chain_accepts(const DenseArgs& l1, const DenseArgs& l2, int prec) { return chain_k2p(l1, l2, prec) != 0; }
+
+int launch_dense_chain(const DenseArgs& l1, const DenseArgs& l2, int prec, hipStream_t s) {
+    const int d = l1.k1, k2p = chain_k2p(l1, l2, prec);
+    if (!k2p) return SSDR_ERR_UNSUPPORTED;
     ChainArgs a{l1.x1, l2.x2, l2.k2, l1.wt_hi, l1.wt_lo, l1.kp, l1.b, l2.wt_hi, l2.wt_lo, l2.kp, l2.b, l2.y, l1.M};
     const double np = prec == PREC_BF16X3 ? 3.0 : 1.0, m128 = std::ceil(l1.M / 128.0) * 128.0;
     ProfScope prof(d == 16 ? "dense_chain_kernel<16>" : "dense_chain_kernel<64>", s, 2.0 * (double)l1.M * ((double)d * d + (double)(d + l2.k2) * 2.0 * d),
diff --git a/ssdr-al_amd/csrc/randla_chain.hpp b/ssdr-al_amd/csrc/randla_chain.hpp
--- /dev/null
+++ b/ssdr-al_amd/csrc/randla_chain.hpp
@@ -0,0 +1,99 @@
+#pragma once
+#include "randla_dev.hpp"
+
+namespace ssdr {
+
+__device__ __forceinline__ u32x4 ld128(const void* p) { return *reinterpret_cast<const u32x4*>(p); }
+__device__ __forceinline__ void st128(void* p, u32x4 v) { *reinterpret_cast<u32x4*>(p) = v; }
+
+template <int TERMS>
+__device__ __forceinline__ f32x4 mma_split(const u32x4 (&a)[2], const u32x4 (&b)[2], f32x4 c) {
+    c = mfma_bf16(a[0], b[0], c);
+    if (TERMS == 2) { c = mfma_bf16(a[1], b[0], c); c = mfma_bf16(a[0], b[1], c); }
+    return c;
+}
+
+
+template <int K1, int KS, int TERMS, int CT1>
+__device__ __forceinline__ void chain_first_mma(uint16_t* const (&A)[2], const uint16_t* const (&B)[2], int lane, f32x4 (&acc)[2][CT1]) {
+    const int fr = lane & 15, fk = 8 * (lane >> 4);
+#pragma unroll
+    for (int ks = 0; ks < (K1 + 31) / 32; ++ks) {
+        u32x4 af[2][2], bf[CT1][2];
+#pragma unroll
+        for (int r = 0; r < 2; ++r)
+#pragma unroll
+            for (int t = 0; t < TERMS; ++t) af[r][t] = ld128(&A[t][(r * 16 + fr) * KS + ks * 32 + fk]);
+#pragma unroll
+        for (int c = 0; c < CT1; ++c)
+#pragma unroll
+            for (int t = 0; t < TERMS; ++t) bf[c][t] = ld128(&B[t][(c * 16 + fr) * KS + ks * 32 + fk]);
+#pragma unroll
+        for (int r = 0; r < 2; ++r)
+#pragma unroll
+            for (int c = 0; c < CT1; ++c) acc[r][c] = mma_split<TERMS>(af[r], bf[c], acc[r][c]);
+    }
+}
+
+template <int KS, int TERMS, int CT1>
+__device__ __forceinline__ void chain_first_store(uint16_t* const (&A)[2], const float* ba, int col0, int lane, const f32x4 (&acc)[2][CT1]) {
+#pragma unroll
+    for (int c = 0; c < CT1; ++c) {
+        const int col = col0 + c * 16 + (lane & 15);
+        const float bias = ba ? ba[col] : 0.f;
+#pragma unroll
+        for (int r = 0; r < 2; ++r)
+#pragma unroll
+            for (int q = 0; q < 4; ++q) {
+                const int row = r * 16 + (lane >> 4) * 4 + q;
+                const float v = lrelu(acc[r][c][q] + bias);
+                unsigned hq, lq; split_bf16(v, 0.f, hq, lq);
+                A[0][row * KS + col] = (uint16_t)(hq & 0xffffu);
+                if (TERMS == 2) A[TERMS - 1][row * KS + col] = (uint16_t)(lq & 0xffffu);
+            }
+    }
+}
+
+template <int K2P, int KS, int TERMS, int CT2>
+__device__ __forceinline__ void chain_second_mma(uint16_t* const (&A)[2], const uint16_t* const (&B)[2], int lane, f32x4 (&acc)[2][CT2]) {
+    const int fr = lane & 15, fk = 8 * (lane >> 4);
+#pragma unroll
+    for (int r = 0; r < 2; ++r)
+#pragma unroll
+        for (int c = 0; c < CT2; ++c) acc[r][c] = f32x4{0.f, 0.f, 0.f, 0.f};
+#pragma unroll
+    for (int ks = 0; ks < K2P / 32; ++ks) {
+        u32x4 af[2][2], bf[CT2][2];
+#pragma unroll
+        for (int r = 0; r < 2; ++r)
+#pragma unroll
+            for (int t = 0; t < TERMS; ++t) af[r][t] = ld128(&A[t][(r * 16 + fr) * KS + ks * 32 + fk]);
+#pragma unroll
+        for (int c = 0; c < CT2; ++c)
+#pragma unroll
+            for (int t = 0; t < TERMS; ++t) bf[c][t] = ld128(&B[t][(c * 16 + fr) * KS + ks * 32 + fk]);
+#pragma unroll
+        for (int r = 0; r < 2; ++r)
+#pragma unroll
+            for (int c = 0; c < CT2; ++c) acc[r][c] = mma_split<TERMS>(af[r], bf[c], acc[r][c]);
+    }
+}
+
+template <int CT2>
+__device__ __forceinline__ void chain_second_store(const f32x4 (&acc)[2][CT2], const float* bb, int col0, int ncols, float* y, int ldy, int rows, int lane) {
+#pragma unroll
+    for (int c = 0; c < CT2; ++c) {
+        const int col = col0 + c * 16 + (lane & 15);
+        if (col >= ncols) continue;
+        const float bias = bb ? bb[col] : 0.f;
+#pragma unroll
+        for (int r = 0; r < 2; ++r)
+#pragma unroll
+            for (int q = 0; q < 4; ++q) {
+                const int row = r * 16 + (lane >> 4) * 4 + q;
+                if (row < rows) y[(size_t)row * ldy + col] = lrelu(acc[r][c][q] + bias);
+            }
+    }
+}
+
+}
diff --git a/ssdr-al_amd/csrc/randla_lfa32.hip b/ssdr-al_amd/csrc/randla_lfa32.hip
--- a/ssdr-al_amd/csrc/randla_lfa32.hip
+++ b/ssdr-al_amd/csrc/randla_lfa32.hip
@@ -1,6 +1,7 @@
 #include "ssdr_internal.hpp"
 #include "randla.hpp"
 #include "randla_dev.hpp"
+#include "randla_chain.hpp"
 #include <cmath>
 
 namespace ssdr {
@@ -448,10 +449,20 @@
 
 constexpr int L0_TPW = 8;
 constexpr int L0_IMG = 64 * 32 + 32, L0_ZERO = 1024, L0_WAVE = L0_IMG + L0_ZERO;
-
-template <bool SECOND, int TERMS>
-__global__ __launch_bounds__(256) void lfa32_l0_kernel(Lfa32Args a) {
+constexpr int L0_PRS = 20;
+constexpr int L0_CKS = 32 + 8;
+constexpr int L0_YS = 32 + 4;
+
+template <bool SECOND, int TERMS, bool FUSED>
+__global__ __launch_bounds__(256) void lfa32_l0_kernel(Lfa32Args a, L0FuseArgs fz) {
     __shared__ __attribute__((aligned(16))) char l0lds[4 * L0_WAVE];
+    constexpr bool F1 = FUSED && !SECOND, F2 = FUSED && SECOND;
+    __shared__ __attribute__((aligned(16))) float l0pool[F1 ? 4 * 32 * L0_PRS : 4];
+    __shared__ float l0w[F1 ? 16 * 8 + 8 : 1];
+    constexpr int L0_AW = TERMS * 32 * L0_CKS * 2 > 32 * L0_YS * 4 ? TERMS * 32 * L0_CKS * 2 : 32 * L0_YS * 4;
+    __shared__ __attribute__((aligned(16))) char l0A[F2 ? 4 * L0_AW : 16];
+    __shared__ __attribute__((aligned(16))) uint16_t l0Wa[TERMS][F2 ? 16 * L0_CKS : 8], l0Wb[TERMS][F2 ? 32 * L0_CKS : 8];
+    __shared__ float l0bias[F2 ? 16 + 32 : 1];
     const int tid = threadIdx.x, lane = tid & 63, w = tid >> 6;
     const int lr = lane & 31, lh = lane >> 5, cc = lr & 15, sg = lr >> 4;
     int bx, b; xcd_tile_map(bx, b);
@@ -481,6 +492,48 @@
     const int nbrrow = (lr & 3) + 4 * (lr >> 3), prow = 2 * lh + ((lr >> 2) & 1), pcol = 2 * sg + lh;
     char* const wrow = img + lane * 32 + lh * 32;
     const char* const rbase = cc < 8 ? img + (32 * (pcol >> 1) + 4 * (pcol & 1)) * 32 + (pcol >> 1) * 32 + cc * 4 : img + L0_IMG;
+    const int p0 = 4 * g0;
+    float* const pool = l0pool + (F1 ? w * 32 * L0_PRS : 0);
+    uint16_t* const Aimg = reinterpret_cast<uint16_t*>(l0A + (F2 ? w * L0_AW : 0));
+    uint16_t* const Aw[2] = {Aimg, Aimg + (F2 ? (TERMS - 1) * 32 * L0_CKS : 0)};
+    constexpr int NSTG = F2 ? (TERMS * 48 * 4 + 255) / 256 : 1;
+    u32x4 stg[NSTG]; float wst = 0.f; float4 x2v = make_float4(0.f, 0.f, 0.f, 0.f);
+    if constexpr (F1) { if (tid < 16 * 8) wst = fz.w[tid]; else if (tid < 16 * 8 + 8 && fz.b) wst = fz.b[tid - 16 * 8]; }
+    if constexpr (F2) {
+#pragma unroll
+        for (int p = 0; p < NSTG; ++p) {
+            const int e = tid + 256 * p, t = e / (48 * 4), q = e - t * (48 * 4), row = q >> 2, sk = (q & 3) * 8;
+            stg[p] = u32x4{0u, 0u, 0u, 0u};
+            if (e < TERMS * 48 * 4) {
+                if (row < 16) { if (sk < 16) stg[p] = ld128((t ? fz.wa_lo : fz.wa_hi) + (size_t)row * fz.kpa + sk); }
+                else if (sk < 24) stg[p] = ld128((t ? fz.wb_lo : fz.wb_hi) + (size_t)(row - 16) * fz.kpb + sk);
+            }
+        }
+        if (tid < 16) wst = fz.ba ? fz.ba[tid] : 0.f; else if (tid < 48) wst = fz.bb ? fz.bb[tid - 16] : 0.f;
+        if (p0 + (lane >> 1) < n) x2v = *reinterpret_cast<const float4*>(fz.x2 + ((size_t)b * n + (size_t)(p0 + (lane >> 1))) * 8 + 4 * (lane & 1));
+    }
+    auto stage_store = [&]() {
+        if constexpr (F1) { if (tid < 16 * 8 + 8) l0w[tid] = wst; }
+        if constexpr (F2) {
+#pragma unroll
+            for (int p = 0; p < NSTG; ++p) {
+                const int e = tid + 256 * p, t = e / (48 * 4), q = e - t * (48 * 4), row = q >> 2, sk = (q & 3) * 8;
+                if (e < TERMS * 48 * 4) { if (row < 16) st128(&l0Wa[t][row * L0_CKS + sk], stg[p]); else st128(&l0Wb[t][(row - 16) * L0_CKS + sk], stg[p]); }
+            }
+            if (tid < 48) l0bias[tid] = wst;
+            u32x2 hi, lo; unsigned hq, lq;
+            split_bf16(x2v.x, x2v.y, hq, lq); hi[0] = hq; lo[0] = lq;
+            split_bf16(x2v.z, x2v.w, hq, lq); hi[1] = hq; lo[1] = lq;
+            *reinterpret_cast<u32x2*>(&Aw[0][(lane >> 1) * L0_CKS + 16 + 4 * (lane & 1)]) = hi;
+            if (TERMS == 2) *reinterpret_cast<u32x2*>(&Aw[TERMS - 1][(lane >> 1) * L0_CKS + 16 + 4 * (lane & 1)]) = lo;
+            if (lane < 32) {
+                const u32x4 z = {0u, 0u, 0u, 0u};
+#pragma unroll
+                for (int t = 0; t < TERMS; ++t) st128(&Aw[t][lane * L0_CKS + 24], z);
+            }
+        }
+        if constexpr (FUSED) __syncthreads();
+    };
     for (int it = 0; it < L0_TPW; ++it) {
         const int t = g0 + it;
         if (4 * t >= n) break;
@@ -534,26 +587,93 @@
         for (int q = 0; q < 16; ++q) fv[q] = fmaxf(accX[q], accX[q] * slope);
         accS = mma32_split<TERMS>(Tf, fcB, accS);
         const float v = softmax_wsum(accS, fv);
-        const int pcu = 4 * t + pcol;
-        if (pcu < n) out[(size_t)pcu * 16 + cc] = v;
-    }
-}
-
-static int launch_lfa32_l0(const Lfa32Args& a, bool second, int B, int prec, hipStream_t s) {
+        if constexpr (F1) pool[(4 * it + pcol) * L0_PRS + cc] = v;
+        else if constexpr (F2) {
+            unsigned hq, lq; split_bf16(v, 0.f, hq, lq);
+            Aw[0][(4 * it + pcol) * L0_CKS + cc] = (uint16_t)(hq & 0xffffu);
+            if (TERMS == 2) Aw[TERMS - 1][(4 * it + pcol) * L0_CKS + cc] = (uint16_t)(lq & 0xffffu);
+        } else {
+            const int pcu = 4 * t + pcol;
+            if (pcu < n) out[(size_t)pcu * 16 + cc] = v;
+        }
+        if constexpr (FUSED) { if (it == 0) stage_store(); }
+    }
+    if (p0 >= n) { stage_store(); return; }
+    if constexpr (F1) {
+        wave_sync();
+        const int pt = p0 + lr;
+        if (pt < n) {
+            float x[16];
+#pragma unroll
+            for (int q = 0; q < 4; ++q) { const float4 t4 = reinterpret_cast<const float4*>(pool + lr * L0_PRS)[q]; x[4 * q] = t4.x; x[4 * q + 1] = t4.y; x[4 * q + 2] = t4.z; x[4 * q + 3] = t4.w; }
+            float acc[4];
+#pragma unroll
+            for (int j = 0; j < 4; ++j) acc[j] = l0w[16 * 8 + 4 * lh + j];
+#pragma unroll
+            for (int k = 0; k < 16; ++k)
+#pragma unroll
+                for (int j = 0; j < 4; ++j) acc[j] = fmaf(x[k], l0w[k * 8 + 4 * lh + j], acc[j]);
+            float4* row = reinterpret_cast<float4*>(fz.tab2 + ((size_t)b * n + (size_t)pt) * 16);
+            if (lh == 0) row[0] = *reinterpret_cast<const float4*>(tabb + (size_t)pt * 16);
+            row[1 + lh] = make_float4(lrelu(acc[0]), lrelu(acc[1]), lrelu(acc[2]), lrelu(acc[3]));
+        }
+    }
+    if constexpr (F2) {
+        wave_sync();
+        const uint16_t* const Ba[2] = {l0Wa[0], l0Wa[TERMS - 1]};
+        const uint16_t* const Bb[2] = {l0Wb[0], l0Wb[TERMS - 1]};
+        f32x4 acc1[2][1] = {{f32x4{0.f, 0.f, 0.f, 0.f}}, {f32x4{0.f, 0.f, 0.f, 0.f}}};
+        chain_first_mma<16, L0_CKS, TERMS, 1>(Aw, Ba, lane, acc1);
+        wave_sync();
+        chain_first_store<L0_CKS, TERMS, 1>(Aw, l0bias, 0, lane, acc1);
+        wave_sync();
+        f32x4 acc2[2][2];
+        chain_second_mma<32, L0_CKS, TERMS, 2>(Aw, Bb, lane, acc2);
+        wave_sync();
+        float* const ytile = reinterpret_cast<float*>(Aimg);
+        chain_second_store<2>(acc2, l0bias + 16, 0, 32, ytile, L0_YS, 32, lane);
+        wave_sync();
+        float* const y = fz.y + ((size_t)b * n + (size_t)p0) * 32;
+#pragma unroll
+        for (int j = 0; j < 4; ++j) {
+            const int row = 8 * j + (lane >> 3);
+            const float4 v4 = *reinterpret_cast<const float4*>(ytile + row * L0_YS + 4 * (lane & 7));
+            if (p0 + row < n) *reinterpret_cast<float4*>(y + (size_t)row * 32 + 4 * (lane & 7)) = v4;
+        }
+    }
+}
+
+static int launch_lfa32_l0(const Lfa32Args& a, const L0FuseArgs* fuse, bool second, int B, int prec, hipStream_t s) {
     dim3 grid((unsigned)((a.n + 16 * L0_TPW - 1) / (16 * L0_TPW)), (unsigned)B);
     const int terms = prec == PREC_BF16X3 ? 2 : 1;
-    const double rows = (double)B * (double)a.n * 16.0, np = terms == 2 ? 3.0 : 1.0;
-    const double exec = (double)B * std::ceil(a.n / 4.0) * 2.0 * 32 * 32 * 16 * (np * (second ? 5.0 : 4.0) + (second ? 1.0 : 0.0));
-    ProfScope prof("lfa32_l0_kernel", s, rows * (2.0 * 10 * 8 + (second ? 2.0 * 8 * 8 : 0.0) + 2.0 * 16 * 16 + 2.0 * 16), exec);
-    if (terms == 2) {
-        if (second) hipLaunchKernelGGL((lfa32_l0_kernel<true, 2>), grid, dim3(256), 0, s, a);
-        else hipLaunchKernelGGL((lfa32_l0_kernel<false, 2>), grid, dim3(256), 0, s, a);
-    } else {
-        if (second) hipLaunchKernelGGL((lfa32_l0_kernel<true, 1>), grid, dim3(256), 0, s, a);
-        else hipLaunchKernelGGL((lfa32_l0_kernel<false, 1>), grid, dim3(256), 0, s, a);
-    }
+    const double rows = (double)B * (double)a.n * 16.0, np = terms == 2 ? 3.0 : 1.0, pts = (double)B * (double)a.n;
+    double exec = (double)B * std::ceil(a.n / 4.0) * 2.0 * 32 * 32 * 16 * (np * (second ? 5.0 : 4.0) + (second ? 1.0 : 0.0));
+    double flops = rows * (2.0 * 10 * 8 + (second ? 2.0 * 8 * 8 : 0.0) + 2.0 * 16 * 16 + 2.0 * 16);
+    if (fuse) {
+        flops += pts * (second ? 2.0 * (16 * 16 + 24 * 32) : 2.0 * 16 * 8);
+        if (second) exec += (double)B * std::ceil(a.n / 32.0) * 32.0 * 2.0 * 32 * (16 + 32) * np;
+    }
+    ProfScope prof("lfa32_l0_kernel", s, flops, exec);
+    const L0FuseArgs fz = fuse ? *fuse : L0FuseArgs{};
+#define SSDR_L0(SECOND_, TERMS_) do { if (fuse) hipLaunchKernelGGL((lfa32_l0_kernel<SECOND_, TERMS_, true>), grid, dim3(256), 0, s, a, fz); \
+                                      else hipLaunchKernelGGL((lfa32_l0_kernel<SECOND_, TERMS_, false>), grid, dim3(256), 0, s, a, fz); } while (0)
+    if (terms == 2) { if (second) SSDR_L0(true, 2); else SSDR_L0(false, 2); }
+    else { if (second) SSDR_L0(true, 1); else SSDR_L0(false, 1); }
+#undef SSDR_L0
     SSDR_HIP(hipGetLastError());
     return SSDR_OK;
+}
+
+int launch_lfa32_l0_fused(const Lfa32Args& a, const L0FuseArgs& f, bool second, int B, int prec, hipStream_t s) {
+    if (a.n <= 0 || B <= 0) return SSDR_OK;
+    if (!a.fin || !a.fc_hi || !a.w1p || (second && !a.w2_hi)) return SSDR_ERR_UNSUPPORTED;
+    if (!second) {
+        if (!f.w || !f.tab2 || (((uintptr_t)f.tab2 | (uintptr_t)a.fin) & 15)) return SSDR_ERR_UNSUPPORTED;
+    } else {
+        if (!f.x2 || !f.y || !f.wa_hi || !f.wb_hi || (prec == PREC_BF16X3 && (!f.wa_lo || !f.wb_lo)) || f.kpa % 8 || f.kpb % 8 || f.kpa < 16 || f.kpb < 24 ||
+            (((uintptr_t)f.x2 | (uintptr_t)f.y | (uintptr_t)f.wa_hi | (uintptr_t)f.wa_lo | (uintptr_t)f.wb_hi | (uintptr_t)f.wb_lo) & 15)) return SSDR_ERR_UNSUPPORTED;
+    }
+    return launch_lfa32_l0(a, &f, second, B, prec, s);
 }
 
 template <int D> static int launch_lfa32_d(const Lfa32Args& a, bool second, int B, int prec, hipStream_t s) {
@@ -609,7 +729,7 @@
     if (a.n <= 0 || B <= 0) return SSDR_OK;
     if ((!a.g && D > 64) || !a.fc_hi || !a.w1p || (second && !a.w2_hi)) { set_error("lfa32: missing G rows or permuted weight pieces"); return SSDR_ERR_INVALID; }
     switch (D) {
-        case 16: return launch_lfa32_l0(a, second, B, prec, s);
+        case 16: return launch_lfa32_l0(a, nullptr, second, B, prec, s);
         case 64: return launch_lfa32_res<64>(a, second, B, prec, s);
         case 128: return launch_lfa32_d<128>(a, second, B, prec, s);
         case 256: return launch_lfa32_d<256>(a, second, B, prec, s);
diff --git a/ssdr-al_amd/csrc/randla_model.hip b/ssdr-al_amd/csrc/randla_model.hip
--- a/ssdr-al_amd/csrc/randla_model.hip
+++ b/ssdr-al_amd/csrc/randla_model.hip
@@ -15,6 +15,7 @@
     int L = 5, K = 16, C = 13, in_dim = 6;
     int prec = PREC_F32;
     int tiles32 = 1;
+    int fusion = 1;
     int d_out[8] = {16, 64, 128, 256, 512, 0, 0, 0};
     std::vector<Layer> layers;
     std::vector<DevBuf> ws;
@@ -231,6 +232,13 @@
     return SSDR_OK;
 }
 
+int ssdr_randla_set_fusion(void* handle, int mode) {
+    Model* m = static_cast<Model*>(handle);
+    if (!m || mode < 0 || mode > 2) { set_error("randla_set_fusion: mode must be 0 (off), 1 (auto) or 2 (always)"); return SSDR_ERR_INVALID; }
+    m->fusion = mode;
+    return SSDR_OK;
+}
+
 void ssdr_randla_destroy(void* handle) {
     Model* m = static_cast<Model*>(handle);
     if (!m) return;
@@ -261,12 +269,20 @@
     for (int i = 0; i < L; ++i) {
         const int d = m->d_out[i], h = d / 2, base = 1 + 8 * i, n = N[i];
         const size_t rows = B * (size_t)n;
-        float* f_pc = buf(idxs(i, 0), rows * h); float* agg = buf(idxs(i, 1), rows * d); float* aggm = buf(idxs(i, 2), rows * d);
+        float* f_pc = buf(idxs(i, 0), rows * h);
         float* out = buf(idxs(i, 3), rows * 2 * d); float* samp = buf(idxs(i, 4), B * (size_t)N[i + 1] * 2 * d);
-        if (!f_pc || !agg || !aggm || !out || !samp) return SSDR_ERR_HIP;
+        if (!f_pc || !out || !samp) return SSDR_ERR_HIP;
         const bool use32 = m->prec != PREC_F32 && m->tiles32 != 0;
         float* tab0 = nullptr;
         if (use32 && d == 16) { tab0 = buf(6 * L + 5, rows * 16); if (!tab0) return SSDR_ERR_HIP; }
+        const bool fuse = tab0 && m->fusion != 0 && (m->fusion == 2 || rows > 16384);
+        float* agg = nullptr; float* aggm = nullptr;
+        auto pooled = [&]() -> bool {
+            if (!agg) agg = buf(idxs(i, 1), rows * d);
+            if (!aggm) aggm = buf(idxs(i, 2), rows * d);
+            return agg && aggm;
+        };
+        if (!fuse && !pooled()) return SSDR_ERR_HIP;
         {
             DenseArgs a1 = dense(f, d_in, m->layers[base + 0], tab0 ? tab0 + 4 : f_pc, (int)rows, 1);
             if (tab0) { a1.ldy = 16; a1.xyz = d_xyz; a1.xyz_batch_stride = n0 * 3; a1.xyz_rows_per_batch = n; }
@@ -303,26 +319,53 @@
             }
             return lfa16 ? launch_lfa_bf16(d, la, second, Bi, m->prec, s) : launch_lfa(d, la, second, Bi, s);
         };
-        SSDR_TRY(run_lfa(false, tab0 ? tab0 : f_pc, m->layers[base + 2]));
-        {
+        auto run_lfa_fused = [&](bool second, const float* fin, const Layer& fc, const L0FuseArgs& fz) -> int {
+            l32.fin = fin; l32.fc_hi = fc.Ph.as<uint16_t>(); l32.fc_lo = fc.Pl.as<uint16_t>();
+            return launch_lfa32_l0_fused(l32, fz, second, Bi, m->prec, s);
+        };
+        const float* tab_second = tab0;
+        int fused1 = SSDR_ERR_UNSUPPORTED;
+        if (fuse && m->layers[base + 3].in == 16 && m->layers[base + 3].out == 8) {
+            float* tab2 = buf(6 * L + 6, rows * 16); if (!tab2) return SSDR_ERR_HIP;
+            L0FuseArgs fz{}; fz.w = m->layers[base + 3].W.as<float>(); fz.b = m->layers[base + 3].b.as<float>(); fz.tab2 = tab2;
+            fused1 = run_lfa_fused(false, tab0, m->layers[base + 2], fz);
+            if (fused1 != SSDR_ERR_UNSUPPORTED) { SSDR_TRY(fused1); tab_second = tab2; }
+        }
+        if (fused1 == SSDR_ERR_UNSUPPORTED) {
+            if (!pooled()) return SSDR_ERR_HIP;
+            la.out = agg; l32.out = agg;
+            SSDR_TRY(run_lfa(false, tab0 ? tab0 : f_pc, m->layers[base + 2]));
             DenseArgs a3 = dense(agg, d, m->layers[base + 3], tab0 ? tab0 + 4 : aggm, (int)rows, 1);
             if (tab0) a3.ldy = 16;
             SSDR_TRY(run_dense(*m, a3, s));
         }
-        la.fin = aggm; la.w_fc = m->layers[base + 5].W.as<float>(); la.w_fc_t = m->layers[base + 5].Wt.as<float>(); la.out = agg;
+        la.w_fc = m->layers[base + 5].W.as<float>(); la.w_fc_t = m->layers[base + 5].Wt.as<float>();
         la.fc_hi = m->layers[base + 5].Wh.as<uint16_t>(); la.fc_lo = m->layers[base + 5].Wl.as<uint16_t>();
         if (gbuf) {
             DenseArgs ga{}; ga.x1 = aggm; ga.k1 = h; ga.W = la.w_fc; ga.b = nullptr; ga.y = gbuf; ga.M = (int)rows; ga.N = d; ga.act = 0; ga.m_per_batch = 1;
             ga.wt_hi = la.fc_hi; ga.wt_lo = la.fc_lo; ga.kp = m->layers[base + 5].kp;
             SSDR_TRY(run_dense(*m, ga, s));
         }
-        SSDR_TRY(run_lfa(true, tab0 ? tab0 : aggm, m->layers[base + 5]));
         DenseArgs a6 = dense(agg, d, m->layers[base + 6], aggm, (int)rows, 1);
         DenseArgs r = dense(aggm, d, m->layers[base + 7], out, (int)rows, 1);
         r.x2 = f; r.k2 = d_in;
-        int chained = m->prec != PREC_F32 ? launch_dense_chain(a6, r, m->prec, s) : SSDR_ERR_UNSUPPORTED;
-        if (chained == SSDR_ERR_UNSUPPORTED) { SSDR_TRY(run_dense(*m, a6, s)); SSDR_TRY(run_dense(*m, r, s)); }
-        else SSDR_TRY(chained);
+        int fused2 = SSDR_ERR_UNSUPPORTED;
+        if (fuse && d_in == 8 && dense_chain_accepts(a6, r, m->prec)) {
+            L0FuseArgs fz{}; fz.x2 = r.x2; fz.wa_hi = a6.wt_hi; fz.wa_lo = a6.wt_lo; fz.kpa = a6.kp; fz.ba = a6.b;
+            fz.wb_hi = r.wt_hi; fz.wb_lo = r.wt_lo; fz.kpb = r.kp; fz.bb = r.b; fz.y = out;
+            fused2 = run_lfa_fused(true, tab_second, m->layers[base + 5], fz);
+            if (fused2 != SSDR_ERR_UNSUPPORTED) SSDR_TRY(fused2);
+        }
+        if (fused2 == SSDR_ERR_UNSUPPORTED) {
+            if (!pooled()) return SSDR_ERR_HIP;
+            la.fin = aggm; la.out = agg; l32.out = agg;
+            a6 = dense(agg, d, m->layers[base + 6], aggm, (int)rows, 1);
+            r = dense(aggm, d, m->layers[base + 7], out, (int)rows, 1); r.x2 = f; r.k2 = d_in;
+            SSDR_TRY(run_lfa(true, tab0 ? tab_second : aggm, m->layers[base + 5]));
+            int chained = m->prec != PREC_F32 ? launch_dense_chain(a6, r, m->prec, s) : SSDR_ERR_UNSUPPORTED;
+            if (chained == SSDR_ERR_UNSUPPORTED) { SSDR_TRY(run_dense(*m, a6, s)); SSDR_TRY(run_dense(*m, r, s)); }
+            else SSDR_TRY(chained);
+        }
         SSDR_TRY(launch_gather_max(out, d_neigh_idx[i], n, N[i + 1], n, 2 * d, samp, Bi, s));
         if (i == 0) { enc.push_back(out); enc_ch.push_back(2 * d); enc_n.push_back(n); }
         enc.push_back(samp); enc_ch.push_back(2 * d); enc_n.push_back(N[i + 1]);
diff --git a/ssdr-al_amd/ssdr_al/_lib.py b/ssdr-al_amd/ssdr_al/_lib.py
--- a/ssdr-al_amd/ssdr_al/_lib.py
+++ b/ssdr-al_amd/ssdr_al/_lib.py
@@ -68,6 +68,7 @@
         L.ssdr_randla_set_precision.argtypes = [vp, i32]
         L.ssdr_select_status.argtypes = [vp, C.POINTER(i32)]
         L.ssdr_randla_set_formulation.argtypes = [vp, i32]
+        L.ssdr_randla_set_fusion.argtypes = [vp, i32]
         L.ssdr_randla_destroy.argtypes = [vp]
         L.ssdr_randla_destroy.restype = None
         L.ssdr_randla_infer_dev.argtypes = [vp, sz, sz, vp, vp, vp, vp, vp, vp, vp, vp]
diff --git a/ssdr-al_amd/ssdr_al/randlanet.py b/ssdr-al_amd/ssdr_al/randlanet.py
--- a/ssdr-al_amd/ssdr_al/randlanet.py
+++ b/ssdr-al_amd/ssdr_al/randlanet.py
@@ -50,6 +50,12 @@
 
     def set_formulation(self, tiles32=True):
         _lib.check(_lib.lib().ssdr_randla_set_formulation(self._h, 1 if tiles32 else 0))
+        return self
+
+    FUSION = {"off": 0, "auto": 1, "always": 2}
+
+    def set_fusion(self, mode="auto"):
+        _lib.check(_lib.lib().ssdr_randla_set_fusion(self._h, self.FUSION.get(mode, mode)))
         return self
 
     def layer_table(self, weights):
```
